# LeoIV/polyaxon

Measured on AMD Instinct MI355X. Metric: HPO trials/hour (whole node) + wall-clock-to-target, ResNet-50 Hyperband sweep, higher is better.
Workload: dtype bf16

## Files before the change

### polyaxon_amd/csrc/bn_kernels.hip

```cpp
#include <hip/hip_runtime.h>

#include "handoff.h"
#include <stdint.h>

#define PLX_API extern "C" __attribute__((visibility("default")))

namespace {

constexpr int kBlock = 256;

struct alignas(16) bf16x8 {
  uint16_t v[8];
};

__device__ __forceinline__ float bf2f(uint16_t b) { return __uint_as_float(((uint32_t)b) << 16); }

__device__ __forceinline__ uint16_t f2bf(float f) {
  return __builtin_bit_cast(uint16_t, (__bf16)f);
}

__device__ __forceinline__ void load8(const bf16x8* p, float* f) {
  const bf16x8 v = *p;
#pragma unroll
  for (int k = 0; k < 8; ++k) f[k] = bf2f(v.v[k]);
}

__device__ __forceinline__ void store8(bf16x8* p, const float* f) {
  bf16x8 v;
#pragma unroll
  for (int k = 0; k < 8; ++k) v.v[k] = f2bf(f[k]);
  *p = v;
}

__global__ __launch_bounds__(kBlock) void bn_stats_kernel(const bf16x8* __restrict__ x, int64_t M, int G, int Gb,
                                                          int64_t rows_per_block, float* __restrict__ psum,
                                                          float* __restrict__ psq) {
  __shared__ float s_sum[kBlock * 8];
  __shared__ float s_sq[kBlock * 8];
  const int tid = threadIdx.x;
  const int cg_local = tid % Gb, rlane = tid / Gb, R = kBlock / Gb;
  const int cg = blockIdx.y * Gb + cg_local;
  const int C = G * 8;
  float shift[8], s[8], q[8];
  load8(x + cg, shift);
#pragma unroll
  for (int k = 0; k < 8; ++k) s[k] = q[k] = 0.f;
  const int64_t r0 = (int64_t)blockIdx.x * rows_per_block;
  int64_t r1 = r0 + rows_per_block;
  if (r1 > M) r1 = M;
#pragma unroll 4
  for (int64_t r = r0 + rlane; r < r1; r += R) {
    float v[8];
    load8(x + r * G + cg, v);
#pragma unroll
    for (int k = 0; k < 8; ++k) {
      const float d = v[k] - shift[k];
      s[k] += d;
      q[k] = fmaf(d, d, q[k]);
    }
  }
#pragma unroll
  for (int k = 0; k < 8; ++k) {
    s_sum[tid * 8 + k] = s[k];
    s_sq[tid * 8 + k] = q[k];
  }
  __syncthreads();
  if (rlane == 0) {
    for (int j = 1; j < R; ++j) {
      const int o = (j * Gb + cg_local) * 8;
#pragma unroll
      for (int k = 0; k < 8; ++k) {
        s[k] += s_sum[o + k];
        q[k] += s_sq[o + k];
      }
    }
    float* ps = psum + (int64_t)blockIdx.x * C + cg * 8;
    float* pq = psq + (int64_t)blockIdx.x * C + cg * 8;
#pragma unroll
    for (int k = 0; k < 8; ++k) {
      ps[k] = s[k];
      pq[k] = q[k];
    }
  }
}

constexpr int kRowsPerSplit = 64;

template <int NT>
__device__ __forceinline__ float l1_rows(const float* __restrict__ src, int b0, int b1, int C, int c, int lane) {
  constexpr int G = NT / 64, U = kRowsPerSplit / G;
  float x[U];
#pragma unroll
  for (int u = 0; u < U; ++u) {
    const int b = b0 + lane + u * G;
    x[u] = b < b1 ? src[(int64_t)b * C + c] : 0.f;
  }
  float a = 0.f;
#pragma unroll
  for (int u = 0; u < U; ++u) a += x[u];
  return a;
}

template <int NT>
__global__ __launch_bounds__(NT) void bn_partial_reduce_kernel(const float* __restrict__ part, int nblk, int C,
                                                               float* __restrict__ out, int S) {
  constexpr int G = NT / 64;
  __shared__ float sh[NT];
  const int c = blockIdx.x * 64 + (threadIdx.x & 63);
  const int lane = threadIdx.x >> 6;
  const int s = blockIdx.y, which = blockIdx.z;
  const int b0 = s * kRowsPerSplit;
  const int b1 = b0 + kRowsPerSplit < nblk ? b0 + kRowsPerSplit : nblk;
  sh[threadIdx.x] = c < C ? l1_rows<NT>(part + (int64_t)which * nblk * C, b0, b1, C, c, lane) : 0.f;
  __syncthreads();
  if (lane == 0 && c < C) {
    float r = 0.f;
#pragma unroll
    for (int g = 0; g < G; ++g) r += sh[threadIdx.x + 64 * g];
    out[((int64_t)which * S + s) * C + c] = r;
  }
}

template <int NT = 256, bool ATOMIC = false>
__device__ __forceinline__ bool fin_sum2(const float* __restrict__ pa, const float* __restrict__ pb, int nblk, int C,
                                         double& A, double& B) {
  constexpr int G = NT / 64;
  __shared__ double sh[2][G][64];
  const int lc = threadIdx.x & 63, sp = threadIdx.x >> 6;
  const int c = blockIdx.x * 64 + lc;
  double a0 = 0.0, b0 = 0.0;
  if (c < C) {
    for (int b = sp; b < nblk; b += 8 * G) {
      float x[8], y[8];
#pragma unroll
      for (int u = 0; u < 8; ++u) {
        const int r = b + u * G;
        if (ATOMIC) {
          x[u] = r < nblk ? __hip_atomic_load(pa + (int64_t)r * C + c, __ATOMIC_RELAXED, __HIP_MEMORY_SCOPE_AGENT) : 0.f;
          y[u] = r < nblk ? __hip_atomic_load(pb + (int64_t)r * C + c, __ATOMIC_RELAXED, __HIP_MEMORY_SCOPE_AGENT) : 0.f;
        } else {
          x[u] = r < nblk ? pa[(int64_t)r * C + c] : 0.f;
          y[u] = r < nblk ? pb[(int64_t)r * C + c] : 0.f;
        }
      }
#pragma unroll
      for (int u = 0; u < 8; ++u) { a0 += x[u]; b0 += y[u]; }
    }
  }
  sh[0][sp][lc] = a0;
  sh[1][sp][lc] = b0;
  __syncthreads();
  if (sp != 0 || c >= C) return false;
  double sa = 0.0, sb = 0.0;
#pragma unroll
  for (int g = 0; g < G; ++g) { sa += sh[0][g][lc]; sb += sh[1][g][lc]; }
  A = sa;
  B = sb;
  return true;
}

struct FwdFin {
  const uint16_t* x_row0;
  int C;
  int64_t M;
  const float* gamma;
  const float* beta;
  float eps, momentum;
  float* running_mean;
  float* running_var;
  float* save_mean;
  float* save_invstd;
  float* scale;
  float* bias;
};

struct BwdFin {
  int C;
  int64_t M;
  const float* gamma;
  const float* mean;
  const float* invstd;
  float* dgamma;
  float* dbeta;
  float* coef;
  int accumulate;
};

template <int NT, bool ATOMIC = false>
__device__ __forceinline__ void fwd_finalize(const float* psum, const float* psq, int nblk, const FwdFin& f) {
  double S, Q;
  if (!fin_sum2<NT, ATOMIC>(psum, psq, nblk, f.C, S, Q)) return;
  const int c = blockIdx.x * 64 + (threadIdx.x & 63);
  const double m = S / (double)f.M;
  double var = Q / (double)f.M - m * m;
  if (var < 0.0) var = 0.0;
  const float mean = (f.x_row0 != nullptr ? bf2f(f.x_row0[c]) : 0.f) + (float)m;
  const float invstd = rsqrtf((float)var + f.eps);
  const float g = f.gamma[c];
  f.save_mean[c] = mean;
  f.save_invstd[c] = invstd;
  f.scale[c] = g * invstd;
  f.bias[c] = f.beta[c] - mean * g * invstd;
  if (f.running_mean != nullptr) {
    const float unbiased = f.M > 1 ? (float)(var * (double)f.M / (double)(f.M - 1)) : (float)var;
    f.running_mean[c] = (1.f - f.momentum) * f.running_mean[c] + f.momentum * mean;
    f.running_var[c] = (1.f - f.momentum) * f.running_var[c] + f.momentum * unbiased;
  }
}

template <int NT, bool ATOMIC = false>
__device__ __forceinline__ void bwd_finalize(const float* pdz, const float* pdzx, int nblk, const BwdFin& f) {
  double A, B;
  if (!fin_sum2<NT, ATOMIC>(pdz, pdzx, nblk, f.C, A, B)) return;
  const int C = f.C;
  const int c = blockIdx.x * 64 + (threadIdx.x & 63);
  const float db = (float)A, dg = (float)B;
  f.dbeta[c] = f.accumulate ? f.dbeta[c] + db : db;
  f.dgamma[c] = f.accumulate ? f.dgamma[c] + dg : dg;
  const float is = f.invstd[c], k1 = f.gamma[c] * is;
  const float k2 = db / (float)f.M, k3 = dg / (float)f.M;
  f.coef[c] = k1;
  f.coef[C + c] = -k1 * k3 * is;
  f.coef[2 * C + c] = -k1 * k2 + k1 * k3 * is * f.mean[c];
}

template <int NT>
__device__ __forceinline__ bool reduce_l2_last(const float* __restrict__ part, int nblk, int C, float* l2, int S,
                                               unsigned* cnt) {
  constexpr int G = NT / 64;
  __shared__ float sh[2][NT];
  __shared__ int s_last;
  const int c = blockIdx.x * 64 + (threadIdx.x & 63);
  const int lane = threadIdx.x >> 6;
  const int s = blockIdx.y;
  const int b0 = s * kRowsPerSplit;
  int b1 = b0 + kRowsPerSplit;
  if (b1 > nblk) b1 = nblk;
  float a0 = 0.f, a1 = 0.f;
  if (c < C) {
    a0 = l1_rows<NT>(part, b0, b1, C, c, lane);
    a1 = l1_rows<NT>(part + (int64_t)nblk * C, b0, b1, C, c, lane);
  }
  sh[0][threadIdx.x] = a0;
  sh[1][threadIdx.x] = a1;
  __syncthreads();
  if (lane == 0 && c < C) {
    const int t = threadIdx.x;
    float r0 = 0.f, r1 = 0.f;
#pragma unroll
    for (int g = 0; g < G; ++g) { r0 += sh[0][t + 64 * g]; r1 += sh[1][t + 64 * g]; }
    __hip_atomic_store(l2 + (int64_t)s * C + c, r0, __ATOMIC_RELAXED, __HIP_MEMORY_SCOPE_AGENT);
    __hip_atomic_store(l2 + ((int64_t)S + s) * C + c, r1, __ATOMIC_RELAXED, __HIP_MEMORY_SCOPE_AGENT);
  }
  asm volatile("s_waitcnt vmcnt(0)" ::: "memory");
  __syncthreads();
  if (threadIdx.x == 0) {
    plx_handoff_release();
    const unsigned old = __hip_atomic_fetch_add(cnt + blockIdx.x, 1u, __ATOMIC_RELAXED, __HIP_MEMORY_SCOPE_AGENT);
    const int last = old == (unsigned)(S - 1);
    if (last) plx_handoff_acquire();
    if (last) __hip_atomic_store(cnt + blockIdx.x, 0u, __ATOMIC_RELAXED, __HIP_MEMORY_SCOPE_AGENT);
    s_last = last;
  }
  __syncthreads();
  return s_last != 0;
}

constexpr int kFinNT = 1024;
template <int NT>
__global__ __launch_bounds__(NT) void bn_fwd_reduce_finalize_kernel(const float* __restrict__ part, int nblk, float* l2,
                                                                    int S, unsigned* cnt, FwdFin f) {
  if (!reduce_l2_last<NT>(part, nblk, f.C, l2, S, cnt)) return;
  fwd_finalize<NT, true>(l2, l2 + (int64_t)S * f.C, S, f);
}

template <int NT>
__global__ __launch_bounds__(NT) void bn_bwd_reduce_finalize_kernel(const float* __restrict__ part, int nblk, float* l2,
                                                                    int S, unsigned* cnt, BwdFin f) {
  if (!reduce_l2_last<NT>(part, nblk, f.C, l2, S, cnt)) return;
  bwd_finalize<NT, true>(l2, l2 + (int64_t)S * f.C, S, f);
}

template <int NT>
__global__ __launch_bounds__(NT) void bn_fwd_finalize_kernel(const float* __restrict__ psum, const float* __restrict__ psq, int nblk,
                                       const uint16_t* __restrict__ x_row0, int C, int64_t M,
                                       const float* __restrict__ gamma, const float* __restrict__ beta, float eps,
                                       float momentum, float* __restrict__ running_mean,
                                       float* __restrict__ running_var, float* __restrict__ save_mean,
                                       float* __restrict__ save_invstd, float* __restrict__ scale,
                                       float* __restrict__ bias) {
  double S, Q;
  if (!fin_sum2<NT>(psum, psq, nblk, C, S, Q)) return;
  const int c = blockIdx.x * 64 + (threadIdx.x & 63);
  const double m = S / (double)M;
  double var = Q / (double)M - m * m;
  if (var < 0.0) var = 0.0;
  const float mean = (x_row0 != nullptr ? bf2f(x_row0[c]) : 0.f) + (float)m;
  const float invstd = rsqrtf((float)var + eps);
  const float g = gamma[c];
  save_mean[c] = mean;
  save_invstd[c] = invstd;
  scale[c] = g * invstd;
  bias[c] = beta[c] - mean * g * invstd;
  if (running_mean != nullptr) {
    const float unbiased = M > 1 ? (float)(var * (double)M / (double)(M - 1)) : (float)var;
    running_mean[c] = (1.f - momentum) * running_mean[c] + momentum * mean;
    running_var[c] = (1.f - momentum) * running_var[c] + momentum * unbiased;
  }
}

template <bool RES, bool RELU>
__global__ __launch_bounds__(kBlock) void bn_apply_kernel(const bf16x8* __restrict__ x, const bf16x8* __restrict__ res,
                                                          bf16x8* __restrict__ y, const float* __restrict__ scale,
                                                          const float* __restrict__ bias, int64_t n_vec, int G,
                                                          uint8_t* __restrict__ mask, const float* __restrict__ rsb) {
  const int64_t stride = (int64_t)gridDim.x * blockDim.x;
  int64_t i = (int64_t)blockIdx.x * blockDim.x + threadIdx.x;
  if (i >= n_vec) return;
  const int cg = (int)(i % G);
  float a[8], b[8], ra[8], rb[8];
#pragma unroll
  for (int k = 0; k < 8; ++k) {
    a[k] = scale[cg * 8 + k];
    b[k] = bias[cg * 8 + k];
    ra[k] = 1.f;
    rb[k] = 0.f;
  }
  if (RES && rsb != nullptr) {
#pragma unroll
    for (int k = 0; k < 8; ++k) {
      ra[k] = rsb[cg * 8 + k];
      rb[k] = rsb[G * 8 + cg * 8 + k];
    }
  }
  for (; i < n_vec; i += stride) {
    const bf16x8 xv = x[i];
    bf16x8 rv;
    if constexpr (RES) rv = res[i];
    float v[8];
#pragma unroll
    for (int k = 0; k < 8; ++k) v[k] = fmaf(bf2f(xv.v[k]), a[k], b[k]);
    if constexpr (RES) {
#pragma unroll
      for (int k = 0; k < 8; ++k) v[k] += fmaf(bf2f(rv.v[k]), ra[k], rb[k]);
    }
    if constexpr (RELU) {
#pragma unroll
      for (int k = 0; k < 8; ++k) v[k] = fmaxf(v[k], 0.f);
    }
    store8(y + i, v);
    if (RELU && mask != nullptr) {
      uint32_t bits = 0;
#pragma unroll
      for (int k = 0; k < 8; ++k) bits |= (uint32_t)(v[k] > 0.f) << k;
      mask[i] = (uint8_t)bits;
    }
  }
}

template <bool RELU>
__global__ __launch_bounds__(kBlock) void bn_bwd_reduce_kernel(const bf16x8* __restrict__ x, const uint8_t* __restrict__ mask,
                                                               const bf16x8* __restrict__ dy, int64_t M, int G, int Gb,
                                                               int64_t rows_per_block, const float* __restrict__ mean,
                                                               const float* __restrict__ invstd, int relu,
                                                               float* __restrict__ pdz, float* __restrict__ pdzx) {
  __shared__ float s_a[kBlock * 8];
  __shared__ float s_b[kBlock * 8];
  const int tid = threadIdx.x;
  const int cg_local = tid % Gb, rlane = tid / Gb, R = kBlock / Gb;
  const int cg = blockIdx.y * Gb + cg_local;
  const int C = G * 8;
  float mu[8], is[8], sa[8], sb[8];
#pragma unroll
  for (int k = 0; k < 8; ++k) {
    mu[k] = mean[cg * 8 + k];
    is[k] = invstd[cg * 8 + k];
    sa[k] = sb[k] = 0.f;
  }
  const int64_t r0 = (int64_t)blockIdx.x * rows_per_block;
  int64_t r1 = r0 + rows_per_block;
  if (r1 > M) r1 = M;
#pragma unroll 4
  for (int64_t r = r0 + rlane; r < r1; r += R) {
    const int64_t off = r * G + cg;
    float xv[8], g[8];
    uint32_t mb = 0xffu;
    if constexpr (RELU) mb = mask[off];
    load8(x + off, xv);
    load8(dy + off, g);
    if constexpr (RELU) {
#pragma unroll
      for (int k = 0; k < 8; ++k) g[k] = (mb >> k) & 1u ? g[k] : 0.f;
    }
#pragma unroll
    for (int k = 0; k < 8; ++k) {
      sa[k] += g[k];
      sb[k] = fmaf(g[k], (xv[k] - mu[k]) * is[k], sb[k]);
    }
  }
#pragma unroll
  for (int k = 0; k < 8; ++k) {
    s_a[tid * 8 + k] = sa[k];
    s_b[tid * 8 + k] = sb[k];
  }
  __syncthreads();
  if (rlane == 0) {
    for (int j = 1; j < R; ++j) {
      const int o = (j * Gb + cg_local) * 8;
#pragma unroll
      for (int k = 0; k < 8; ++k) {
        sa[k] += s_a[o + k];
        sb[k] += s_b[o + k];
      }
    }
    float* pa = pdz + (int64_t)blockIdx.x * C + cg * 8;
    float* pb = pdzx + (int64_t)blockIdx.x * C + cg * 8;
#pragma unroll
    for (int k = 0; k < 8; ++k) {
      pa[k] = sa[k];
      pb[k] = sb[k];
    }
  }
}

template <int NT>
__global__ __launch_bounds__(NT) void bn_bwd_finalize_kernel(const float* __restrict__ pdz, const float* __restrict__ pdzx, int nblk, int C,
                                       int64_t M, const float* __restrict__ gamma, const float* __restrict__ mean,
                                       const float* __restrict__ invstd, float* __restrict__ dgamma,
                                       float* __restrict__ dbeta, float* __restrict__ coef, int accumulate) {
  double A, B;
  if (!fin_sum2<NT>(pdz, pdzx, nblk, C, A, B)) return;
  const int c = blockIdx.x * 64 + (threadIdx.x & 63);
  const float db = (float)A, dg = (float)B;
  dbeta[c] = accumulate ? dbeta[c] + db : db;
  dgamma[c] = accumulate ? dgamma[c] + dg : dg;
  const float is = invstd[c], k1 = gamma[c] * is;
  const float k2 = db / (float)M, k3 = dg / (float)M;
  coef[c] = k1;
  coef[C + c] = -k1 * k3 * is;
  coef[2 * C + c] = -k1 * k2 + k1 * k3 * is * mean[c];
}

struct ResBn {
  const bf16x8* x;
  const uint8_t* mask;
  const float* mean;
  const float* invstd;
  float* part;
};

template <bool RP, bool RELU, bool RMASK = false>
__global__ __launch_bounds__(kBlock) void bn_bwd_dx_kernel(const bf16x8* __restrict__ x, const uint8_t* __restrict__ mask,
                                                           const bf16x8* __restrict__ dy, bf16x8* __restrict__ dx,
                                                           bf16x8* __restrict__ dres, const float* __restrict__ coef,
                                                           int64_t n_vec, int G, int relu, ResBn rb) {
  const int64_t stride = (int64_t)gridDim.x * blockDim.x;
  int64_t i = (int64_t)blockIdx.x * blockDim.x + threadIdx.x;
  if (!RP && i >= n_vec) return;
  const int cg = (int)(i % G);
  const int C = G * 8;
  constexpr bool rp = RP;
  float A[8], B[8], D[8], mu2[8], is2[8], ra[8], rc[8];
#pragma unroll
  for (int k = 0; k < 8; ++k) {
    A[k] = coef[cg * 8 + k];
    B[k] = coef[C + cg * 8 + k];
    D[k] = coef[2 * C + cg * 8 + k];
    ra[k] = rc[k] = 0.f;
    mu2[k] = rp ? rb.mean[cg * 8 + k] : 0.f;
    is2[k] = rp ? rb.invstd[cg * 8 + k] : 0.f;
  }
  for (; i < n_vec; i += stride) {
    float xv[8], g[8];
    uint32_t mb = 0xffu;
    if constexpr (RELU) mb = mask[i];
    load8(x + i, xv);
    load8(dy + i, g);
    if constexpr (RELU) {
#pragma unroll
      for (int k = 0; k < 8; ++k) g[k] = (mb >> k) & 1u ? g[k] : 0.f;
    }
    if (dres != nullptr) store8(dres + i, g);
    if constexpr (rp) {
      float x2[8];
      load8(rb.x + i, x2);
      const uint32_t m2 = RMASK ? rb.mask[i] : 0xffu;
#pragma unroll
      for (int k = 0; k < 8; ++k) {
        const float g2 = (m2 >> k) & 1u ? g[k] : 0.f;
        ra[k] += g2;
        rc[k] = fmaf(g2, (x2[k] - mu2[k]) * is2[k], rc[k]);
      }
    }
    float o[8];
#pragma unroll
    for (int k = 0; k < 8; ++k) o[k] = fmaf(A[k], g[k], fmaf(B[k], xv[k], D[k]));
    store8(dx + i, o);
  }
  if constexpr (rp) {
  __shared__ float red[kBlock * 16];
#pragma unroll
  for (int k = 0; k < 8; ++k) {
    red[threadIdx.x * 16 + k] = ra[k];
    red[threadIdx.x * 16 + 8 + k] = rc[k];
  }
  __syncthreads();
  if ((int)threadIdx.x < G) {
    for (int j = 1; j < kBlock / G; ++j) {
      const float* o = red + (j * G + threadIdx.x) * 16;
#pragma unroll
      for (int k = 0; k < 8; ++k) {
        ra[k] += o[k];
        rc[k] += o[8 + k];
      }
    }
    float* pa = rb.part + (int64_t)blockIdx.x * C + cg * 8;
    float* pc = rb.part + ((int64_t)gridDim.x + blockIdx.x) * C + cg * 8;
#pragma unroll
    for (int k = 0; k < 8; ++k) {
      pa[k] = ra[k];
      pc[k] = rc[k];
    }
  }
  }
}

struct Plan {
  int G, Gb, gy, nblk, S;
  int64_t rows_per_block;
};

inline bool plan_for(int64_t M, int C, Plan* p) {
  if (C <= 0 || (C & 7)) return false;
  const int G = C / 8;
  if (G & (G - 1)) return false;
  p->G = G;
  p->Gb = G < kBlock ? G : kBlock;
  p->gy = G / p->Gb;
  const int R = kBlock / p->Gb;
  const int64_t cap = (2048 + p->gy - 1) / p->gy;
  int64_t want = (M + 16 * R - 1) / (16 * R);
  if (want > cap) want = cap;
  if (want < 1) want = 1;
  int64_t rpb = (M + want - 1) / want;
  rpb = (rpb + R - 1) / R * R;
  p->rows_per_block = rpb;
  p->nblk = (int)((M + rpb - 1) / rpb);
  p->S = (p->nblk + kRowsPerSplit - 1) / kRowsPerSplit;
  return true;
}

inline int apply_grid(int64_t n_vec, int G) {
  int64_t g = (n_vec + kBlock - 1) / kBlock;
  if (g > 4096) g = 4096;
  if (g < 1) g = 1;
  const int64_t mult = G > kBlock ? G / kBlock : 1;
  g = (g + mult - 1) / mult * mult;
  return (int)g;
}

inline void launch_dx(hipStream_t stream, int64_t n_vec, int G, const void* x, const uint8_t* mask, const void* dy,
                      void* dx, void* dres, const float* coef, int relu, const ResBn& rb) {
  const dim3 grid(apply_grid(n_vec, G));
  auto k = rb.part == nullptr ? (relu ? bn_bwd_dx_kernel<false, true> : bn_bwd_dx_kernel<false, false>)
           : rb.mask != nullptr ? (relu ? bn_bwd_dx_kernel<true, true, true> : bn_bwd_dx_kernel<true, false, true>)
                                : (relu ? bn_bwd_dx_kernel<true, true> : bn_bwd_dx_kernel<true, false>);
  hipLaunchKernelGGL(k, grid, dim3(kBlock), 0, stream, (const bf16x8*)x, mask, (const bf16x8*)dy, (bf16x8*)dx,
                     (bf16x8*)dres, coef, n_vec, G, relu, rb);
}

inline void launch_apply(hipStream_t stream, int64_t n_vec, int G, const void* x, const void* res, void* y,
                         const float* scale, const float* bias, int relu, uint8_t* mask, const float* rsb) {
  auto k = res != nullptr ? (relu ? bn_apply_kernel<true, true> : bn_apply_kernel<true, false>)
                          : (relu ? bn_apply_kernel<false, true> : bn_apply_kernel<false, false>);
  hipLaunchKernelGGL(k, dim3(apply_grid(n_vec, G)), dim3(kBlock), 0, stream, (const bf16x8*)x, (const bf16x8*)res,
                     (bf16x8*)y, scale, bias, n_vec, G, mask, rsb);
}

inline void reduce_finalize_fwd(hipStream_t stream, const float* part, int nblk, float* l2, unsigned* cnt,
                                const FwdFin& f) {
  const int C = f.C, S = (nblk + kRowsPerSplit - 1) / kRowsPerSplit;
  if (cnt != nullptr) {
    hipLaunchKernelGGL(bn_fwd_reduce_finalize_kernel<kFinNT>, dim3((C + 63) / 64, S), dim3(kFinNT), 0, stream, part, nblk, l2, S,
                       cnt, f);
    return;
  }
  hipLaunchKernelGGL(bn_partial_reduce_kernel<kFinNT>,
                     dim3((C + 63) / 64, S, 2), dim3(kFinNT), 0, stream, part, nblk, C, l2, S);
  hipLaunchKernelGGL(bn_fwd_finalize_kernel<kFinNT>, dim3((C + 63) / 64),
                     dim3(kFinNT), 0, stream, l2, l2 + (int64_t)S * C, S,
                     f.x_row0, C, f.M, f.gamma, f.beta, f.eps, f.momentum, f.running_mean, f.running_var, f.save_mean,
                     f.save_invstd, f.scale, f.bias);
}

inline void reduce_finalize_bwd(hipStream_t stream, const float* part, int nblk, float* l2, unsigned* cnt,
                                const BwdFin& f) {
  const int C = f.C, S = (nblk + kRowsPerSplit - 1) / kRowsPerSplit;
  if (cnt != nullptr) {
    hipLaunchKernelGGL(bn_bwd_reduce_finalize_kernel<kFinNT>, dim3((C + 63) / 64, S), dim3(kFinNT), 0, stream, part, nblk, l2, S,
                       cnt, f);
    return;
  }
  hipLaunchKernelGGL(bn_partial_reduce_kernel<kFinNT>,
                     dim3((C + 63) / 64, S, 2), dim3(kFinNT), 0, stream, part, nblk, C, l2, S);
  hipLaunchKernelGGL(bn_bwd_finalize_kernel<kFinNT>, dim3((C + 63) / 64),
                     dim3(kFinNT), 0, stream, l2, l2 + (int64_t)S * C, S, C,
                     f.M, f.gamma, f.mean, f.invstd, f.dgamma, f.dbeta, f.coef, f.accumulate);
}

struct alignas(8) u8x8 {
  uint8_t v[8];
};

__global__ __launch_bounds__(256) void stem_apply_pool_kernel(const bf16x8* __restrict__ x,
                                                              const float* __restrict__ sb, bf16x8* __restrict__ y,
                                                              u8x8* __restrict__ idx, int N, int H, int W, int G,
                                                              int OH, int OW) {
  const unsigned j = blockIdx.x * 256u + threadIdx.x;
  if (j >= (unsigned)(OW * G)) return;
  const unsigned g = j % (unsigned)G, ow = j / (unsigned)G;
  const int C = G * 8;
  float a[8], b[8];
#pragma unroll
  for (int k = 0; k < 8; ++k) {
    a[k] = sb[g * 8 + k];
    b[k] = sb[C + g * 8 + k];
  }
  for (int row = blockIdx.y; row < N * OH; row += gridDim.y) {
    const int n = row / OH, oh = row - n * OH;
    float best[8];
    uint8_t arg[8];
#pragma unroll
    for (int k = 0; k < 8; ++k) {
      best[k] = -INFINITY;
      arg[k] = 255;
    }
    uint4 q[9];
    bool ok[9];
#pragma unroll
    for (int kh = 0; kh < 3; ++kh) {
      const int ih = oh * 2 - 1 + kh;
      const int ihc = ih < 0 ? 0 : (ih >= H ? H - 1 : ih);
#pragma unroll
      for (int kw = 0; kw < 3; ++kw) {
        const int iw = (int)ow * 2 - 1 + kw;
        const int iwc = iw < 0 ? 0 : (iw >= W ? W - 1 : iw);
        ok[kh * 3 + kw] = ih >= 0 && ih < H && iw >= 0 && iw < W;
        q[kh * 3 + kw] = *(const uint4*)(x + ((size_t)(n * H + ihc) * W + iwc) * G + g);
      }
    }
#pragma unroll
    for (int t9 = 0; t9 < 9; ++t9) {
      const uint32_t qw[4] = {q[t9].x, q[t9].y, q[t9].z, q[t9].w};
#pragma unroll
      for (int k = 0; k < 8; ++k) {
        const float xk = __uint_as_float((k & 1) ? (qw[k >> 1] & 0xffff0000u) : (qw[k >> 1] << 16));
        const float f = (float)(__bf16)fmaxf(fmaf(xk, a[k], b[k]), 0.f);
        if (ok[t9] && (f > best[k] || arg[k] == 255)) {
          best[k] = f;
          arg[k] = (uint8_t)t9;
        }
      }
    }
    bf16x8 o;
    u8x8 m;
#pragma unroll
    for (int k = 0; k < 8; ++k) {
      o.v[k] = f2bf(best[k]);
      m.v[k] = arg[k];
    }
    const size_t t = (size_t)row * OW * G + j;
    y[t] = o;
    idx[t] = m;
  }
}

__device__ __forceinline__ int stem_cover(int i, int O, int* o, int* k) {
  int n = 0;
  if (i & 1) {
    if ((i + 1) >> 1 < O) { o[n] = (i + 1) >> 1; k[n++] = 0; }
    o[n] = (i - 1) >> 1; k[n++] = 2;
  } else if ((i >> 1) < O) {
    o[n] = i >> 1; k[n++] = 1;
  }
  return n;
}

template <bool DX>
__global__ __launch_bounds__(256) void stem_pool_bn_bwd_kernel(const bf16x8* __restrict__ dy, const u8x8* __restrict__ idx,
                                                               const bf16x8* __restrict__ x, const float* __restrict__ sb,
                                                               const float* __restrict__ mean,
                                                               const float* __restrict__ invstd,
                                                               const float* __restrict__ coef, bf16x8* __restrict__ dx,
                                                               float* __restrict__ part, int N, int H, int W, int G,
                                                               int OH, int OW) {
  const int QH = (H + 1) / 2, QW = (W + 1) / 2;
  const unsigned j0 = blockIdx.x * 256u + threadIdx.x;
  const bool active = j0 < (unsigned)(QW * G);
  const unsigned j = active ? j0 : 0u;
  const unsigned g = j % (unsigned)G;
  const int qb = (int)(j / (unsigned)G);
  const int C = G * 8;
  float a[8], b[8], c1[8], c2[8], c3[8], s1[8], s2[8];
#pragma unroll
  for (int k = 0; k < 8; ++k) {
    a[k] = sb[g * 8 + k];
    b[k] = sb[C + g * 8 + k];
    if constexpr (DX) {
      c1[k] = coef[g * 8 + k];
      c2[k] = coef[C + g * 8 + k];
      c3[k] = coef[2 * C + g * 8 + k];
    } else {
      c1[k] = mean[g * 8 + k];
      c2[k] = invstd[g * 8 + k];
      c3[k] = 0.f;
    }
    s1[k] = s2[k] = 0.f;
  }
  for (int row = blockIdx.y; active && row < N * QH; row += gridDim.y) {
    const int n = row / QH, qa = row - n * QH;
    uint2 am[4];
    uint4 d[4], xq[4];
    bool wv[4], pv[4];
#pragma unroll
    for (int p = 0; p < 2; ++p)
#pragma unroll
      for (int q = 0; q < 2; ++q) {
        const int w4 = p * 2 + q, oh = qa + p, ow = qb + q;
        wv[w4] = oh < OH && ow < OW;
        const size_t off = ((size_t)(n * OH + (oh < OH ? oh : OH - 1)) * OW + (ow < OW ? ow : OW - 1)) * G + g;
        am[w4] = *(const uint2*)(idx + off);
        d[w4] = *(const uint4*)(dy + off);
        if (!wv[w4]) am[w4] = make_uint2(0xffffffffu, 0xffffffffu);
        const int ih = 2 * qa + p, iw = 2 * qb + q;
        pv[w4] = ih < H && iw < W;
        xq[w4] = *(const uint4*)(x + ((size_t)(n * H + (ih < H ? ih : H - 1)) * W + (iw < W ? iw : W - 1)) * G + g);
      }
#pragma unroll
    for (int di = 0; di < 2; ++di)
#pragma unroll
      for (int dj = 0; dj < 2; ++dj) {
        const int e = di * 2 + dj;
        const uint32_t xw[4] = {xq[e].x, xq[e].y, xq[e].z, xq[e].w};
        float o[8];
#pragma unroll
        for (int k = 0; k < 8; ++k) {
          float acc = 0.f;
#pragma unroll
          for (int p = 0; p < 2; ++p)
#pragma unroll
            for (int q = 0; q < 2; ++q) {
              const int kh = di + 1 - 2 * p, kw = dj + 1 - 2 * q;
              if (kh < 0 || kw < 0) continue;
              const int w4 = p * 2 + q;
              const uint32_t ab = (k < 4 ? am[w4].x : am[w4].y) >> (8 * (k & 3)) & 0xffu;
              const uint32_t dw = (k >> 1) == 0 ? d[w4].x : (k >> 1) == 1 ? d[w4].y : (k >> 1) == 2 ? d[w4].z : d[w4].w;
              const float dv = __uint_as_float((k & 1) ? (dw & 0xffff0000u) : (dw << 16));
              acc += ab == (uint32_t)(kh * 3 + kw) ? dv : 0.f;
            }
          const float xf = __uint_as_float((k & 1) ? (xw[k >> 1] & 0xffff0000u) : (xw[k >> 1] << 16));
          const float dz = (pv[e] && fmaf(xf, a[k], b[k]) > 0.f) ? (float)(__bf16)acc : 0.f;
          if constexpr (DX) {
            o[k] = fmaf(c1[k], dz, fmaf(c2[k], xf, c3[k]));
          } else {
            s1[k] += dz;
            s2[k] = fmaf(dz, (xf - c1[k]) * c2[k], s2[k]);
          }
        }
        if constexpr (DX) {
          if (pv[e]) store8(dx + ((size_t)(n * H + 2 * qa + di) * W + 2 * qb + dj) * G + g, o);
        }
      }
  }
  if constexpr (!DX) {
    __shared__ float red[256 * 17];
#pragma unroll
    for (int k = 0; k < 8; ++k) {
      red[threadIdx.x * 17 + k] = s1[k];
      red[threadIdx.x * 17 + 8 + k] = s2[k];
    }
    __syncthreads();
    const int nb = gridDim.x * gridDim.y, blk = blockIdx.y * gridDim.x + blockIdx.x;
    for (int e = threadIdx.x; e < G * 16; e += 256) {
      const int gg = e % G, v = e / G;
      float sum = 0.f;
      for (int r = gg; r < 256; r += G) sum += red[r * 17 + v];
      const int c = gg * 8 + (v & 7);
      part[((int64_t)(v < 8 ? 0 : nb) + blk) * C + c] = sum;
    }
  }
}

constexpr int g_stem_bwd_cap = 4096;

inline dim3 stem_bwd_grid(int N, int H, int W, int G, bool dx) {
  const int rows = N * ((H + 1) / 2), cap = dx ? 65535 : g_stem_bwd_cap;
  return dim3((((W + 1) / 2) * G + 255) / 256, rows < cap ? rows : cap);
}

}

PLX_API int64_t plx_bn_workspace(int64_t M, int C) {
  Plan p;
  if (!plan_for(M, C, &p)) return -1;
  return 2 * (int64_t)(p.nblk + p.S) * C;
}

PLX_API int plx_bn_forward(const void* x, const void* res, void* y, int64_t M, int C, const float* gamma,
                           const float* beta, float eps, float momentum, float* running_mean, float* running_var,
                           float* save_mean, float* save_invstd, float* scale_bias ,
                           float* partials , uint8_t* mask ,
                           int relu, const float* res_sb ,
                           unsigned* counters ,
                           hipStream_t stream) {
  Plan p;
  if (!plan_for(M, C, &p) || M < 1) return 1;
  float* psum = partials;
  float* psq = partials + (int64_t)p.nblk * C;
  hipLaunchKernelGGL(bn_stats_kernel, dim3(p.nblk, p.gy), dim3(kBlock), 0, stream, (const bf16x8*)x, M, p.G, p.Gb,
                     p.rows_per_block, psum, psq);
  float* l2 = partials + 2 * (int64_t)p.nblk * C;
  reduce_finalize_fwd(stream, partials, p.nblk, l2, counters,
                      FwdFin{(const uint16_t*)x, C, M, gamma, beta, eps, momentum, running_mean, running_var,
                             save_mean, save_invstd, scale_bias, scale_bias + C});
  const int64_t n_vec = M * p.G;
  if (y != nullptr)
    launch_apply(stream, n_vec, p.G, x, res, y, scale_bias, scale_bias + C, relu, relu ? mask : nullptr, res_sb);
  return (int)hipGetLastError();
}

PLX_API int64_t plx_bn_l2_workspace(int nblk, int C) {
  return 2 * (int64_t)((nblk + kRowsPerSplit - 1) / kRowsPerSplit) * C;
}

PLX_API int plx_bn_forward_from_partials(const void* x, const void* res, void* y, int64_t M, int C,
                                         const float* gamma, const float* beta, float eps, float momentum,
                                         float* running_mean, float* running_var, float* save_mean,
                                         float* save_invstd, float* scale_bias, const float* partials, int nblk,
                                         float* l2, uint8_t* mask, int relu, const float* res_sb,
                                         unsigned* counters, hipStream_t stream) {
  Plan p;
  if (!plan_for(M, C, &p) || M < 1 || nblk < 1) return 1;
  reduce_finalize_fwd(stream, partials, nblk, l2, counters,
                      FwdFin{nullptr, C, M, gamma, beta, eps, momentum, running_mean, running_var, save_mean,
                             save_invstd, scale_bias, scale_bias + C});
  const int64_t n_vec = M * p.G;
  if (y != nullptr)
    launch_apply(stream, n_vec, p.G, x, res, y, scale_bias, scale_bias + C, relu, relu ? mask : nullptr, res_sb);
  return (int)hipGetLastError();
}

PLX_API int plx_bn_apply(const void* x, const void* res, void* y, int64_t M, int C, const float* scale_bias, int relu,
                         hipStream_t stream) {
  Plan p;
  if (!plan_for(M, C, &p)) return 1;
  const int64_t n_vec = M * p.G;
  launch_apply(stream, n_vec, p.G, x, res, y, scale_bias, scale_bias + C, relu, nullptr, nullptr);
  return (int)hipGetLastError();
}

PLX_API int plx_bn_dx_blocks(int64_t M, int C) {
  Plan p;
  if (!plan_for(M, C, &p)) return -1;
  return apply_grid(M * p.G, p.G);
}

PLX_API int plx_bn_backward(const void* x, const uint8_t* mask, const void* dy, void* dx, void* dres, int64_t M, int C,
                            const float* gamma, const float* save_mean, const float* save_invstd, float* dgamma,
                            float* dbeta, float* coef , float* partials , int relu,
                            int accumulate, const ResBn* resbn , unsigned* counters,
                            hipStream_t stream) {
  Plan p;
  if (!plan_for(M, C, &p) || M < 1 || (relu && mask == nullptr)) return 1;
  if (resbn != nullptr && (dres == nullptr || resbn->part == nullptr)) return 1;
  const ResBn rb = resbn != nullptr ? *resbn : ResBn{};
  float* pa = partials;
  float* pb = partials + (int64_t)p.nblk * C;
  hipLaunchKernelGGL(relu ? bn_bwd_reduce_kernel<true> : bn_bwd_reduce_kernel<false>, dim3(p.nblk, p.gy), dim3(kBlock), 0, stream, (const bf16x8*)x,
                     mask, (const bf16x8*)dy, M, p.G, p.Gb, p.rows_per_block, save_mean, save_invstd,
                     relu, pa, pb);
  float* l2 = partials + 2 * (int64_t)p.nblk * C;
  reduce_finalize_bwd(stream, partials, p.nblk, l2, counters,
                      BwdFin{C, M, gamma, save_mean, save_invstd, dgamma, dbeta, coef, accumulate});
  const int64_t n_vec = M * p.G;
  launch_dx(stream, n_vec, p.G, x, mask, dy, dx, dres, coef, relu, rb);
  return (int)hipGetLastError();
}

PLX_API int plx_bn_backward_from_partials(const void* x, const uint8_t* mask, const void* dy, void* dx, void* dres,
                                          int64_t M, int C, const float* gamma, const float* save_mean,
                                          const float* save_invstd, float* dgamma, float* dbeta, float* coef,
                                          const float* partials, int nblk, float* l2, int relu, int accumulate,
                                          const ResBn* resbn, unsigned* counters, hipStream_t stream) {
  Plan p;
  if (!plan_for(M, C, &p) || M < 1 || nblk < 1 || (relu && mask == nullptr)) return 1;
  if (resbn != nullptr && (dres == nullptr || resbn->part == nullptr)) return 1;
  const ResBn rb = resbn != nullptr ? *resbn : ResBn{};
  reduce_finalize_bwd(stream, partials, nblk, l2, counters,
                      BwdFin{C, M, gamma, save_mean, save_invstd, dgamma, dbeta, coef, accumulate});
  const int64_t n_vec = M * p.G;
  launch_dx(stream, n_vec, p.G, x, mask, dy, dx, dres, coef, relu, rb);
  return (int)hipGetLastError();
}

PLX_API int plx_bn_backward_coef(const void* x, const uint8_t* mask, const void* dy, int64_t M, int C,
                                 const float* gamma, const float* save_mean, const float* save_invstd, float* dgamma,
                                 float* dbeta, float* coef, float* partials, int relu, int accumulate,
                                 unsigned* counters, hipStream_t stream) {
  Plan p;
  if (!plan_for(M, C, &p) || M < 1 || (relu && mask == nullptr)) return 1;
  float* pa = partials;
  float* pb = partials + (int64_t)p.nblk * C;
  hipLaunchKernelGGL(relu ? bn_bwd_reduce_kernel<true> : bn_bwd_reduce_kernel<false>, dim3(p.nblk, p.gy), dim3(kBlock), 0, stream, (const bf16x8*)x,
                     mask, (const bf16x8*)dy, M, p.G, p.Gb, p.rows_per_block, save_mean, save_invstd,
                     relu, pa, pb);
  reduce_finalize_bwd(stream, partials, p.nblk, partials + 2 * (int64_t)p.nblk * C, counters,
                      BwdFin{C, M, gamma, save_mean, save_invstd, dgamma, dbeta, coef, accumulate});
  return (int)hipGetLastError();
}

PLX_API int plx_bn_backward_coef_from_partials(int64_t M, int C, const float* gamma, const float* save_mean,
                                               const float* save_invstd, float* dgamma, float* dbeta, float* coef,
                                               const float* partials, int nblk, float* l2, int accumulate,
                                               unsigned* counters, hipStream_t stream) {
  Plan p;
  if (!plan_for(M, C, &p) || M < 1 || nblk < 1) return 1;
  reduce_finalize_bwd(stream, partials, nblk, l2, counters,
                      BwdFin{C, M, gamma, save_mean, save_invstd, dgamma, dbeta, coef, accumulate});
  return (int)hipGetLastError();
}

PLX_API int plx_stem_bn_pool_forward(const void* x, void* y, void* idx, int N, int H, int W, int C, const float* gamma,
                                     const float* beta, float eps, float momentum, float* running_mean,
                                     float* running_var, float* save_mean, float* save_invstd, float* scale_bias,
                                     float* partials, const float* ext_part, int ext_nblk, unsigned* counters,
                                     hipStream_t stream) {
  const int G = C / 8;
  if (N <= 0 || H <= 0 || W <= 0 || C % 8 || G > 256 || 256 % G) return 1;
  const int rc = ext_part != nullptr
                     ? plx_bn_forward_from_partials(x, nullptr, nullptr, (int64_t)N * H * W, C, gamma, beta, eps,
                                                    momentum, running_mean, running_var, save_mean, save_invstd,
                                                    scale_bias, ext_part, ext_nblk, partials, nullptr, 1, nullptr,
                                                    counters, stream)
                     : plx_bn_forward(x, nullptr, nullptr, (int64_t)N * H * W, C, gamma, beta, eps, momentum,
                                      running_mean, running_var, save_mean, save_invstd, scale_bias, partials, nullptr,
                                      1, nullptr, counters, stream);
  if (rc) return rc;
  const int OH = (H - 1) / 2 + 1, OW = (W - 1) / 2 + 1;
  const int rows = N * OH;
  hipLaunchKernelGGL(stem_apply_pool_kernel, dim3((OW * G + 255) / 256, rows < 65535 ? rows : 65535), dim3(256), 0,
                     stream, (const bf16x8*)x, scale_bias, (bf16x8*)y, (u8x8*)idx, N, H, W, G, OH, OW);
  return (int)hipGetLastError();
}


PLX_API int64_t plx_stem_bn_pool_bwd_workspace(int N, int H, int W, int C) {
  const dim3 g = stem_bwd_grid(N, H, W, C / 8, false);
  const int64_t nblk = (int64_t)g.x * g.y;
  return 2 * (nblk + (nblk + kRowsPerSplit - 1) / kRowsPerSplit) * C;
}

PLX_API int plx_stem_bn_pool_backward(const void* dy, const void* idx, const void* x, void* dx, int N, int H, int W,
                                      int C, const float* gamma, const float* save_mean, const float* save_invstd,
                                      const float* scale_bias, float* dgamma, float* dbeta, float* coef,
                                      float* workspace, int accumulate, unsigned* counters, hipStream_t stream) {
  const int G = C / 8;
  if (N <= 0 || H <= 0 || W <= 0 || C % 8 || G > 256 || 256 % G) return 1;
  const int OH = (H - 1) / 2 + 1, OW = (W - 1) / 2 + 1;
  const dim3 grid = stem_bwd_grid(N, H, W, G, false), grid_dx = stem_bwd_grid(N, H, W, G, true);
  const int nblk = grid.x * grid.y;
  hipLaunchKernelGGL(stem_pool_bn_bwd_kernel<false>, grid, dim3(256), 0, stream, (const bf16x8*)dy, (const u8x8*)idx,
                     (const bf16x8*)x, scale_bias, save_mean, save_invstd, (const float*)nullptr, (bf16x8*)nullptr,
                     workspace, N, H, W, G, OH, OW);
  reduce_finalize_bwd(stream, workspace, nblk, workspace + 2 * (int64_t)nblk * C, counters,
                      BwdFin{C, (int64_t)N * H * W, gamma, save_mean, save_invstd, dgamma, dbeta, coef, accumulate});
  hipLaunchKernelGGL(stem_pool_bn_bwd_kernel<true>, grid_dx, dim3(256), 0, stream, (const bf16x8*)dy, (const u8x8*)idx,
                     (const bf16x8*)x, scale_bias, save_mean, save_invstd, coef, (bf16x8*)dx, (float*)nullptr, N, H,
                     W, G, OH, OW);
  return (int)hipGetLastError();
}
```

### polyaxon_amd/csrc/conv_gemm.hip

```cpp
#include <hip/hip_runtime.h>

#include <stdint.h>

namespace {

typedef __bf16 bf16x8 __attribute__((ext_vector_type(8)));
typedef short s16x4 __attribute__((ext_vector_type(4)));
typedef float f32x4 __attribute__((ext_vector_type(4)));
typedef uint32_t u32x4 __attribute__((ext_vector_type(4)));
typedef __attribute__((address_space(3))) void lds_void;
typedef __attribute__((address_space(1))) const void gbl_void;

constexpr int BK = 64;

struct ConvGeom {
    int H, W;
    int Hr, Wr;
    int C, S, ntaps;
    int Hc, Wc, OS, oph, opw;
    signed char offh[9], offw[9], btap[9];
    int tap_a[9], tap_b[9];
    uint32_t mWr, mHr;
    int nh, nw, hv[3], wv[3];
    uint32_t pat[9];
    int tap_inner;
};

__device__ __forceinline__ int pick9(const int (&v)[9], int t) {
    int r = v[0];
#pragma unroll
    for (int i = 1; i < 9; ++i) r = t == i ? v[i] : r;
    return r;
}

inline uint32_t div_magic(int d) { return d <= 1 ? 0u : (uint32_t)((1ull << 32) / (unsigned)d + 1); }

inline ConvGeom finish_geom(ConvGeom g) {
    g.nh = g.nw = 0;
    for (int i = 0; i < 9; ++i) g.pat[i] = 0;
    for (int t = 0; t < 9; ++t) {
        g.tap_a[t] = t < g.ntaps ? (g.offh[t] * g.W + g.offw[t]) * g.C * 2 : 0;
        g.tap_b[t] = t < g.ntaps ? g.btap[t] * g.C * 2 : 0;
        if (t >= g.ntaps) continue;
        int i = 0, j = 0;
        while (i < g.nh && g.hv[i] != g.offh[t]) ++i;
        if (i == g.nh) g.hv[g.nh++] = g.offh[t];
        while (j < g.nw && g.wv[j] != g.offw[t]) ++j;
        if (j == g.nw) g.wv[g.nw++] = g.offw[t];
        g.pat[i * 3 + j] |= 1u << t;
    }
    g.mWr = div_magic(g.Wr);
    g.mHr = div_magic(g.Hr);
    return g;
}

struct BnBwd {
    const __bf16* x;
    const uint8_t* mask;
    const float* mean;
    const float* invstd;
    float* part;
    int part_ld, blk_off;
    int skip_h, skip_w;
};

struct BnDx {
    const __bf16* x;
    const uint8_t* mask;
    const float* coef;
    __bf16* dy;
};

__device__ __forceinline__ void row_coords(int m, int Hr, int Wr, int& n, int& r, int& c) {
    const int q = m / Wr;
    c = m - q * Wr;
    n = q / Hr;
    r = q - n * Hr;
}

__device__ __forceinline__ void row_coords(int m, const ConvGeom& g, int& n, int& r, int& c) {
    const int q = g.mWr ? (int)__umulhi((uint32_t)m, g.mWr) : m;
    c = m - q * g.Wr;
    n = g.mHr ? (int)__umulhi((uint32_t)q, g.mHr) : q;
    r = q - n * g.Hr;
}

__device__ __forceinline__ size_t out_row(const ConvGeom& g, int m) {
    if (g.OS == 0) return (size_t)m;
    int n, r, c;
    row_coords(m, g.Hr, g.Wr, n, r, c);
    return ((size_t)n * g.Hc + r * g.OS + g.oph) * g.Wc + c * g.OS + g.opw;
}
constexpr int NTHREADS = 256;

template <int STEP>
__device__ __forceinline__ void wait_vm_stages(int stages) {
    if (stages >= 4 && 4 * STEP <= 63) asm volatile("s_waitcnt vmcnt(%0)" ::"n"(4 * STEP < 63 ? 4 * STEP : 63) : "memory");
    else if (stages >= 3) asm volatile("s_waitcnt vmcnt(%0)" ::"n"(3 * STEP) : "memory");
    else if (stages == 2) asm volatile("s_waitcnt vmcnt(%0)" ::"n"(2 * STEP) : "memory");
    else if (stages == 1) asm volatile("s_waitcnt vmcnt(%0)" ::"n"(STEP) : "memory");
    else asm volatile("s_waitcnt vmcnt(0)" ::: "memory");
}

__device__ __forceinline__ int xcd_remap(int bid, int nwg) {
    const int xcd = bid & 7, q = nwg >> 3, r = nwg & 7;
    const int base = xcd < r ? xcd * (q + 1) : r * (q + 1) + (xcd - r) * q;
    return base + (bid >> 3);
}

__device__ __forceinline__ void glds16(const void* g, void* l) {
    __builtin_amdgcn_global_load_lds((gbl_void*)g, (lds_void*)l, 16, 0, 0);
}

constexpr uint32_t OOB = 0x80000000u;

__device__ __forceinline__ __amdgpu_buffer_rsrc_t buf_rsrc(const void* base) {
    return __builtin_amdgcn_make_buffer_rsrc(const_cast<void*>(base), 0, (int)OOB, 0x00020000);
}

__device__ __forceinline__ void blds16(__amdgpu_buffer_rsrc_t r, uint32_t off, void* l) {
    __builtin_amdgcn_raw_ptr_buffer_load_lds(r, (lds_void*)l, 16, off, 0, 0, 0);
}

__device__ __forceinline__ uint32_t pack_bf16x2(float a, float b) {
    return (uint32_t)__builtin_bit_cast(uint16_t, (__bf16)a) | ((uint32_t)__builtin_bit_cast(uint16_t, (__bf16)b) << 16);
}

__device__ __forceinline__ int nt_swz(int row) { return (row >> 1) & 7; }

template <int BM, int BN, int WGM, int WGN, int MODE, int MINB = 2, int NBUF = 2, bool BWD = false, int NTH = NTHREADS,
          bool BNDX = false>
__global__ void __launch_bounds__(NTH, MINB)
gemm_nt_kernel(const __bf16* __restrict__ A, const __bf16* __restrict__ B, __bf16* __restrict__ C,
               int M, int N, int K, int lda, int ldb, int ldc, const __bf16* __restrict__ zero,
               float* __restrict__ stats, ConvGeom geo, const __bf16* __restrict__ D, int ldd, BnBwd bnr,
               const uint8_t* __restrict__ dmask, BnDx bd) {
    constexpr bool CONV = MODE == 1, STEM = MODE == 2;
    static_assert(MODE >= 0 && MODE <= 2, "dense, gather or stem");
    static_assert(!BNDX || (MODE == 0 && NBUF == 2 && BWD && NTH == 256), "BNDX: dense double-buffered data gradient");
    constexpr int NW = NTH / 64;
    static_assert(WGM * WGN == NW, "one wave per wave tile");
    static_assert(NTH == 256 && NBUF >= 1 && NBUF <= 2, "4-wave kernels, one or two K stages");
    constexpr int WTM = BM / WGM, WTN = BN / WGN;
    constexpr int RM = WTM / 16, RN = WTN / 16;
    constexpr int A_BYTES = BM * BK * 2, B_BYTES = BN * BK * 2, STAGE = A_BYTES + B_BYTES;
    extern __shared__ __attribute__((aligned(16))) char smem[];

    const int tid = threadIdx.x, lane = tid & 63;
    const int wave = __builtin_amdgcn_readfirstlane(tid >> 6);
    const int ntn = N / BN, ntm = (M + BM - 1) / BM;
    const int id = xcd_remap(blockIdx.x, ntm * ntn);
    const int tn = id % ntn, tm = id / ntn;
    const int m0 = tm * BM, n0 = tn * BN;
    const int wm = wave / WGN, wn = wave % WGN;

    constexpr int AI = BM / (8 * NW), BI = BN / (8 * NW);
    int a_off[AI];
    uint32_t a_ok[AI];
#pragma unroll
    for (int i = 0; i < AI; ++i) {
        const int row = (i * NW + wave) * 8 + (lane >> 3);
        const int lc = (lane & 7) ^ nt_swz(row);
        const int gm = m0 + row;
        if constexpr (CONV) {
            int n, r, c;
            row_coords(gm, geo, n, r, c);
            const int ih0 = r * geo.S, iw0 = c * geo.S;
            a_off[i] = (((n * geo.H + ih0) * geo.W + iw0) * lda + lc * 8) * 2;
            uint32_t ok = 0;
#pragma unroll
            for (int hi = 0; hi < 3; ++hi) {
                const bool vh = hi < geo.nh && (unsigned)(ih0 + geo.hv[hi]) < (unsigned)geo.H;
#pragma unroll
                for (int wj = 0; wj < 3; ++wj) {
                    const bool vw = wj < geo.nw && (unsigned)(iw0 + geo.wv[wj]) < (unsigned)geo.W;
                    ok |= (vh && vw) ? geo.pat[hi * 3 + wj] : 0u;
                }
            }
            a_ok[i] = gm < M ? ok : 0u;
        } else if constexpr (STEM) {
            int n, r, c;
            row_coords(gm, geo, n, r, c);
            const int ih0 = 2 * r - 3, sc0 = c - 2;
            a_off[i] = ((n * geo.H + ih0) * geo.W + sc0) * 16;
            uint32_t ok = 0;
#pragma unroll
            for (int st = 0; st < 4; ++st) {
                const int t = st * 8 + lc;
                ok |= (t < 28 && (unsigned)(ih0 + (t >> 2)) < (unsigned)geo.H && (unsigned)(sc0 + (t & 3)) < (unsigned)geo.W)
                          ? 1u << st : 0u;
            }
            a_ok[i] = gm < M ? ok : 0u;
        } else {
            a_off[i] = (gm * lda + lc * 8) * 2;
            a_ok[i] = gm < M ? 1u : 0u;
        }
    }
    int b_off[BI];
#pragma unroll
    for (int i = 0; i < BI; ++i) {
        const int row = (i * NW + wave) * 8 + (lane >> 3);
        b_off[i] = ((n0 + row) * ldb + ((lane & 7) ^ nt_swz(row)) * 8) * 2;
    }
    const __amdgpu_buffer_rsrc_t ra = buf_rsrc(A), rb = buf_rsrc(B);

    auto stage_a = [&](int buf, int k0, int t, int c0) {
        char* base = smem + buf * STAGE;
        int a_add = k0 * 2, bit = 0;
        if constexpr (CONV) {
            a_add = pick9(geo.tap_a, t) + c0 * 2;
            bit = t;
        }
        if constexpr (STEM) bit = k0 / BK;
#pragma unroll
        for (int i = 0; i < AI; ++i) {
            if constexpr (STEM) {
                const int t = bit * 8 + ((lane & 7) ^ nt_swz((i * NW + wave) * 8 + (lane >> 3)));
                a_add = ((t >> 2) * geo.W + (t & 3)) * 16;
            }
            const uint32_t off = (a_ok[i] >> bit) & 1u ? (uint32_t)(a_off[i] + a_add) : OOB;
            blds16(ra, off, base + (i * NW + wave) * 1024);
        }
    };
    auto stage_b = [&](int buf, int k0, int t, int c0) {
        char* base = smem + buf * STAGE;
        const int bk0 = CONV ? pick9(geo.tap_b, t) + c0 * 2 : k0 * 2;
#pragma unroll
        for (int i = 0; i < BI; ++i) blds16(rb, (uint32_t)(b_off[i] + bk0), base + A_BYTES + (i * NW + wave) * 1024);
    };
    auto stage = [&](int buf, int k0, int t, int c0) {
        stage_a(buf, k0, t, c0);
        stage_b(buf, k0, t, c0);
    };

    f32x4 acc[RN][RM];
#pragma unroll
    for (int a = 0; a < RN; ++a)
#pragma unroll
        for (int b = 0; b < RM; ++b) acc[a][b] = f32x4{0.f, 0.f, 0.f, 0.f};

    const int fr = lane & 15, fq = lane >> 4;
    const int nk = K / BK;
    const int cdim = CONV ? geo.C : K;
    int st = 0, sc = 0;
    const bool tap_inner = CONV && geo.tap_inner;
    auto advance = [&]() {
        const bool wt = st + 1 == geo.ntaps, wc = sc + BK == cdim;
        const int st_i = wt ? 0 : st + 1, sc_i = wt ? sc + BK : sc;
        const int st_m = wc ? st + 1 : st, sc_m = wc ? 0 : sc + BK;
        st = tap_inner ? st_i : st_m;
        sc = tap_inner ? sc_i : sc_m;
    };
    constexpr int XI = BNDX ? AI : 1;
    uint32_t e_off[XI];
    u32x4 gq[XI], xq[XI], oq[XI];
    uint32_t mq[XI];
    u32x4 cf[6];
    const int lc8 = (((lane & 7) ^ nt_swz(wave * 8 + (lane >> 3))) & 7) * 8;
    const bool dy_owner = tn == 0;
    if constexpr (BNDX) {
#pragma unroll
        for (int i = 0; i < XI; ++i) {
            const int gm = m0 + (i * NW + wave) * 8 + (lane >> 3);
            e_off[i] = gm < M ? (uint32_t)((gm * K + lc8) * 2) : OOB;
        }
    }
    auto load_a = [&](int k0) {
        const __amdgpu_buffer_rsrc_t rx = buf_rsrc(bd.x), rc = buf_rsrc(bd.coef);
#pragma unroll
        for (int i = 0; i < XI; ++i) {
            gq[i] = __builtin_amdgcn_raw_buffer_load_b128(ra, (int)e_off[i], k0 * 2, 0);
            xq[i] = __builtin_amdgcn_raw_buffer_load_b128(rx, (int)e_off[i], k0 * 2, 0);
        }
        if (bd.mask != nullptr) {
            const __amdgpu_buffer_rsrc_t rm = buf_rsrc(bd.mask);
#pragma unroll
            for (int i = 0; i < XI; ++i)
                mq[i] = __builtin_amdgcn_raw_buffer_load_b8(rm, (int)(e_off[i] == OOB ? OOB : e_off[i] >> 4), k0 >> 3, 0);
        } else {
#pragma unroll
            for (int i = 0; i < XI; ++i) mq[i] = 0xffu;
        }
#pragma unroll
        for (int r = 0; r < 3; ++r) {
            cf[2 * r] = __builtin_amdgcn_raw_buffer_load_b128(rc, lc8 * 4, (r * K + k0) * 4, 0);
            cf[2 * r + 1] = __builtin_amdgcn_raw_buffer_load_b128(rc, lc8 * 4 + 16, (r * K + k0) * 4, 0);
        }
    };
    auto xform_a = [&](int buf) {
        char* base = smem + buf * STAGE;
        const float* ca = (const float*)&cf[0];
        const float* cb = (const float*)&cf[2];
        const float* cd = (const float*)&cf[4];
#pragma unroll
        for (int i = 0; i < XI; ++i) {
            const uint32_t* pg = (const uint32_t*)&gq[i];
            const uint32_t* px = (const uint32_t*)&xq[i];
            uint32_t* po = (uint32_t*)&oq[i];
            const uint32_t mb = mq[i];
#pragma unroll
            for (int j = 0; j < 4; ++j) {
                const float g0 = (mb >> (2 * j)) & 1u ? __uint_as_float(pg[j] << 16) : 0.f;
                const float g1 = (mb >> (2 * j + 1)) & 1u ? __uint_as_float(pg[j] & 0xffff0000u) : 0.f;
                const float x0 = __uint_as_float(px[j] << 16), x1 = __uint_as_float(px[j] & 0xffff0000u);
                const float o0 = fmaf(ca[2 * j], g0, fmaf(cb[2 * j], x0, cd[2 * j]));
                const float o1 = fmaf(ca[2 * j + 1], g1, fmaf(cb[2 * j + 1], x1, cd[2 * j + 1]));
                po[j] = pack_bf16x2(o0, o1);
            }
            if (e_off[i] == OOB) oq[i] = u32x4{0u, 0u, 0u, 0u};
            *(u32x4*)(base + (i * NW + wave) * 1024 + lane * 16) = oq[i];
        }
    };
    auto store_dy = [&](int k0) {
        if (!dy_owner) return;
        const __amdgpu_buffer_rsrc_t rd = buf_rsrc(bd.dy);
#pragma unroll
        for (int i = 0; i < XI; ++i) __builtin_amdgcn_raw_buffer_store_b128(oq[i], rd, (int)e_off[i], k0 * 2, 0);
    };
    if constexpr (BNDX) {
        static_assert(!BNDX || NW == 4, "a thread's rows step by 32: one chunk column per thread");
        load_a(0);
        stage_b(0, 0, 0, 0);
        xform_a(0);
        asm volatile("s_waitcnt vmcnt(0)" ::: "memory");
        __syncthreads();
        store_dy(0);
    } else {
        stage(0, 0, 0, 0);
        advance();
        asm volatile("s_waitcnt vmcnt(0)" ::: "memory");
        __syncthreads();
    }
    for (int kt = 0; kt < nk; ++kt) {
        const int cur = NBUF == 2 ? kt & 1 : 0;
        if constexpr (BNDX) {
            if (kt + 1 < nk) {
                load_a((kt + 1) * BK);
                stage_b(cur ^ 1, (kt + 1) * BK, 0, 0);
            }
        }
        if (!BNDX && NBUF == 1 && kt > 0) {
            stage(0, kt * BK, st, sc);
            advance();
            asm volatile("s_waitcnt vmcnt(0)" ::: "memory");
            __syncthreads();
        }
        if (!BNDX && NBUF == 2 && kt + 1 < nk) {
            stage(cur ^ 1, (kt + 1) * BK, st, sc);
            advance();
        }
        const char* As = smem + cur * STAGE;
        const char* Bs = As + A_BYTES;
#pragma unroll
        for (int kk = 0; kk < 2; ++kk) {
            bf16x8 fa[RN], fb[RM];
#pragma unroll
            for (int rn = 0; rn < RN; ++rn) {
                const int row = wn * WTN + rn * 16 + fr;
                const int pc = (kk * 4 + fq) ^ nt_swz(row);
                fa[rn] = *(const bf16x8*)(Bs + row * 128 + pc * 16);
            }
#pragma unroll
            for (int rm = 0; rm < RM; ++rm) {
                const int row = wm * WTM + rm * 16 + fr;
                const int pc = (kk * 4 + fq) ^ nt_swz(row);
                fb[rm] = *(const bf16x8*)(As + row * 128 + pc * 16);
            }
#pragma unroll
            for (int rn = 0; rn < RN; ++rn)
#pragma unroll
                for (int rm = 0; rm < RM; ++rm)
                    acc[rn][rm] = __builtin_amdgcn_mfma_f32_16x16x32_bf16(fa[rn], fb[rm], acc[rn][rm], 0, 0, 0);
        }
        if constexpr (BNDX) {
            if (kt + 1 < nk) xform_a(cur ^ 1);
        }
        if (NBUF == 2) asm volatile("s_waitcnt vmcnt(0)" ::: "memory");
        __syncthreads();
        if constexpr (BNDX) {
            if (kt + 1 < nk) store_dy((kt + 1) * BK);
        }
    }
    constexpr int CROW = BN * 2 + 16;
    constexpr int CHUNKS = BN / 8;
    static_assert(NTH % CHUNKS == 0, "a thread keeps one chunk column over the store loop");
    constexpr int RSTEP = NTH / CHUNKS, ITERS = BM / RSTEP;
    const int rows = min(BM, M - m0);
    const int cc = tid % CHUNKS, r0 = tid / CHUNKS;
    const int ch0 = n0 + cc * 8;
    const bool bnr_on = BWD && bnr.part != nullptr;
    const bool stats_on = !BWD && stats != nullptr;
    const bool d_on = BWD && D != nullptr;
    int orow[ITERS];
#pragma unroll
    for (int it = 0; it < ITERS; ++it) {
        const int gm = min(m0 + r0 + it * RSTEP, M - 1);
        if constexpr (CONV) orow[it] = (int)out_row(geo, gm);
        else orow[it] = gm;
    }
    auto tile_to_lds = [&]() {
#pragma unroll
        for (int rm = 0; rm < RM; ++rm) {
            const int ml = wm * WTM + rm * 16 + fr;
#pragma unroll
            for (int rn = 0; rn < RN; ++rn) {
                const int nl = wn * WTN + rn * 16 + fq * 4;
                const f32x4 v = acc[rn][rm];
                uint2 packed;
                packed.x = pack_bf16x2(v[0], v[1]);
                packed.y = pack_bf16x2(v[2], v[3]);
                *(uint2*)(smem + ml * CROW + nl * 2) = packed;
            }
        }
    };
    constexpr bool LATE = BWD && NBUF == 1;
    if constexpr (LATE) tile_to_lds();
    uint4 dpre[ITERS], xpre[ITERS];
    uint32_t mpre[ITERS], dmpre[ITERS];
    if (d_on) {
#pragma unroll
        for (int it = 0; it < ITERS; ++it) dpre[it] = *(const uint4*)(D + (size_t)orow[it] * ldd + ch0);
        if (dmask != nullptr) {
#pragma unroll
            for (int it = 0; it < ITERS; ++it) dmpre[it] = dmask[((size_t)orow[it] * ldd + ch0) >> 3];
        }
    }
    float sa[8], sb[8], mu[8], is[8];
    float s1[8], s2[8];
#pragma unroll
    for (int k = 0; k < 8; ++k) s1[k] = s2[k] = 0.f;
    if (bnr_on) {
#pragma unroll
        for (int it = 0; it < ITERS; ++it) xpre[it] = *(const uint4*)(bnr.x + (size_t)orow[it] * ldc + ch0);
        if (bnr.mask != nullptr) {
#pragma unroll
            for (int it = 0; it < ITERS; ++it) mpre[it] = bnr.mask[((size_t)orow[it] * ldc + ch0) >> 3];
        } else {
#pragma unroll
            for (int it = 0; it < ITERS; ++it) mpre[it] = 0xffu;
        }
        if (bnr.skip_w > 0) {
#pragma unroll
            for (int it = 0; it < ITERS; ++it) {
                const int gm = m0 + r0 + it * RSTEP, q = gm / bnr.skip_w;
                if (((gm - q * bnr.skip_w) | (q % bnr.skip_h)) % 2 == 0) mpre[it] = 0u;
            }
        }
#pragma unroll
        for (int k = 0; k < 8; ++k) {
            sa[k] = sb[k] = 0.f;
            mu[k] = bnr.mean[ch0 + k];
            is[k] = bnr.invstd[ch0 + k];
        }
    }
    if constexpr (!LATE) tile_to_lds();
    __syncthreads();
#pragma unroll
    for (int it = 0; it < ITERS; ++it) {
        const int r = r0 + it * RSTEP;
        if (r >= rows) break;
        uint4 v = *(const uint4*)(smem + r * CROW + cc * 16);
        if (stats_on) {
            const uint32_t* pv = (const uint32_t*)&v;
#pragma unroll
            for (int j = 0; j < 4; ++j) {
                const float lo = __uint_as_float(pv[j] << 16), hi = __uint_as_float(pv[j] & 0xffff0000u);
                s1[2 * j] += lo;
                s1[2 * j + 1] += hi;
                s2[2 * j] = fmaf(lo, lo, s2[2 * j]);
                s2[2 * j + 1] = fmaf(hi, hi, s2[2 * j + 1]);
            }
        }
        if (d_on) {
            uint32_t* pv = (uint32_t*)&v;
            const uint32_t* pd = (const uint32_t*)&dpre[it];
            const uint32_t db = dmask != nullptr ? dmpre[it] : 0xffu;
#pragma unroll
            for (int j = 0; j < 4; ++j) {
                const float d0 = (db >> (2 * j)) & 1u ? __uint_as_float(pd[j] << 16) : 0.f;
                const float d1 = (db >> (2 * j + 1)) & 1u ? __uint_as_float(pd[j] & 0xffff0000u) : 0.f;
                const float lo = __uint_as_float(pv[j] << 16) + d0;
                const float hi = __uint_as_float(pv[j] & 0xffff0000u) + d1;
                pv[j] = pack_bf16x2(lo, hi);
            }
        }
        *(uint4*)(C + (size_t)orow[it] * ldc + ch0) = v;
        if (bnr_on) {
            const uint32_t mb = mpre[it];
            const uint32_t* pv = (const uint32_t*)&v;
            const uint32_t* px = (const uint32_t*)&xpre[it];
#pragma unroll
            for (int j = 0; j < 4; ++j) {
                const float g0 = (mb >> (2 * j)) & 1u ? __uint_as_float(pv[j] << 16) : 0.f;
                const float g1 = (mb >> (2 * j + 1)) & 1u ? __uint_as_float(pv[j] & 0xffff0000u) : 0.f;
                const float x0 = __uint_as_float(px[j] << 16), x1 = __uint_as_float(px[j] & 0xffff0000u);
                sa[2 * j] += g0;
                sa[2 * j + 1] += g1;
                sb[2 * j] = fmaf(g0, (x0 - mu[2 * j]) * is[2 * j], sb[2 * j]);
                sb[2 * j + 1] = fmaf(g1, (x1 - mu[2 * j + 1]) * is[2 * j + 1], sb[2 * j + 1]);
            }
        }
    }
    auto reduce_store = [&](const float* va, const float* vb, float* dst_a, float* dst_b) {
        float* red = (float*)smem;
        __syncthreads();
#pragma unroll
        for (int k = 0; k < 8; ++k) {
            red[tid * 17 + k] = va[k];
            red[tid * 17 + 8 + k] = vb[k];
        }
        __syncthreads();
        if (tid < CHUNKS * 16) {
            const int c = tid % CHUNKS, v = tid / CHUNKS;
            float sum = 0.f;
#pragma unroll 4
            for (int j = 0; j < RSTEP; ++j) sum += red[(j * CHUNKS + c) * 17 + v];
            if (v < 8) dst_a[c * 8 + v] = sum;
            else dst_b[c * 8 + v - 8] = sum;
        }
        __syncthreads();
    };
    constexpr int SROWS = BN % 128 == 0 ? 128 : 256, SPB = BM / SROWS;
    static_assert(SPB >= 1 && BM % SROWS == 0, "block height must be a multiple of the stats row height");
    const int srow = m0 / SROWS, nsr = (M + SROWS - 1) / SROWS;
    auto zero_rows = [&](float* base_a, float* base_b, int ld) {
        if constexpr (SPB > 1) {
            for (int i = tid; i < (SPB - 1) * BN; i += NTH) {
                const int r = srow + 1 + i / BN, c = i % BN;
                if (r < nsr) {
                    base_a[(size_t)(r - srow) * ld + c] = 0.f;
                    base_b[(size_t)(r - srow) * ld + c] = 0.f;
                }
            }
        }
    };
    if (bnr_on) {
        float* pa = bnr.part + (size_t)(bnr.blk_off + srow) * ldc + n0;
        float* pb = bnr.part + (size_t)(bnr.part_ld + bnr.blk_off + srow) * ldc + n0;
        reduce_store(sa, sb, pa, pb);
        zero_rows(pa, pb, ldc);
    }
    if (stats_on) {
        float* pa = stats + (size_t)srow * N + n0;
        float* pb = stats + (size_t)(nsr + srow) * N + n0;
        reduce_store(s1, s2, pa, pb);
        zero_rows(pa, pb, N);
    }
}

template <int ROWB>
__device__ __forceinline__ int tr_swz(int row) {
    if constexpr (ROWB >= 256) return 2 * ((row & 3) | (((row >> 3) & 1) << 2));
    else return 2 * (((row >> 1) & 1) | (((row >> 3) & 1) << 1));
}

template <int ROWB>
__device__ __forceinline__ s16x4 tr_read(const char* img, int row, int col ) {
    const int lc = col >> 3, half = (col >> 2) & 1;
    const int pc = lc ^ tr_swz<ROWB>(row);
    return __builtin_amdgcn_ds_read_tr16_b64_v4i16(
        (__attribute__((address_space(3))) s16x4*)(img + row * ROWB + pc * 16 + half * 8));
}

__device__ __forceinline__ uint32_t lds_addr(const void* p) {
    return (uint32_t)(uintptr_t)(const __attribute__((address_space(3))) char*)p;
}

__device__ __forceinline__ s16x4 ds_tr(uint32_t addr) {
    s16x4 r;
    asm volatile("ds_read_b64_tr_b16 %0, %1" : "=v"(r) : "v"(addr) : "memory");
    return r;
}

template <int ROWB, int GATHER = 0, int BKR = BK>
__device__ __forceinline__ void stage_rows(char* img, __amdgpu_buffer_rsrc_t rsrc, int ld, int r0, int rend, int c0,
                                           int wave, int lane, const ConvGeom* geo = nullptr, int dh = 0, int dw = 0) {
    constexpr int INSTR = BKR * ROWB / 1024;
    static_assert(INSTR % 4 == 0, "a stage splits evenly over the 4 waves");
#pragma unroll
    for (int i = 0; i < INSTR / 4; ++i) {
        const int off = (i * 4 + wave) * 1024 + lane * 16;
        const int row = off / ROWB, pc = (off % ROWB) >> 4;
        const int lc = pc ^ tr_swz<ROWB>(row);
        const int gr = r0 + row;
        uint32_t boff;
        if constexpr (GATHER == 2) {
            int n, r, c;
            row_coords(gr, *geo, n, r, c);
            const int t = (c0 >> 3) + lc, ih = 2 * r - 3 + (t >> 2), sc = c - 2 + (t & 3);
            const bool ok = gr < rend && t < 28 && (unsigned)ih < (unsigned)geo->H && (unsigned)sc < (unsigned)geo->W;
            boff = ok ? (uint32_t)(((n * geo->H + ih) * geo->W + sc) * 16) : OOB;
        } else if constexpr (GATHER == 1) {
            int n, r, c;
            row_coords(gr, *geo, n, r, c);
            const int ih = r * geo->S + dh, iw = c * geo->S + dw;
            const bool ok = gr < rend && (unsigned)ih < (unsigned)geo->H && (unsigned)iw < (unsigned)geo->W;
            boff = ok ? (uint32_t)(((((n * geo->H + ih) * geo->W + iw) * ld) + c0 + lc * 8) * 2) : OOB;
        } else {
            boff = gr < rend ? (uint32_t)((gr * ld + c0 + lc * 8) * 2) : OOB;
        }
        blds16(rsrc, boff, img + (i * 4 + wave) * 1024);
    }
}


template <int BN1, int BN2, int WG1, int WG2, int CONV, int NST = 2, int BKT = BK>
__global__ void __launch_bounds__(NTHREADS, NST * BKT <= 2 * BK ? 2 : 1)
gemm_tn_kernel(const __bf16* __restrict__ A, const __bf16* __restrict__ B, float* __restrict__ W,
               int M, int N1, int N2, int lda, int ldb, int kchunk, const __bf16* __restrict__ zero,
               ConvGeom geo) {
    constexpr int WT1 = BN1 / WG1, WT2 = BN2 / WG2, R1 = WT1 / 16, R2 = WT2 / 16;
    constexpr int ROWA = BN1 * 2, ROWB_ = BN2 * 2;
    constexpr int A_BYTES = BKT * ROWA, STAGE = BKT * (ROWA + ROWB_);
    constexpr int PER_STAGE = (BKT * ROWA / 1024 + BKT * ROWB_ / 1024) / 4;
    static_assert(BKT == 64 || BKT == 32, "32- or 64-row stages");
    static_assert(NST >= 2 && NST <= 4, "2-4 stages");
    extern __shared__ __attribute__((aligned(16))) char smem[];

    const int tid = threadIdx.x, lane = tid & 63;
    const int wave = __builtin_amdgcn_readfirstlane(tid >> 6);
    const int nt1 = N1 / BN1, nt2 = N2 / BN2, ntiles = nt1 * nt2;
    const int nslices = (M + kchunk - 1) / kchunk;
    const int id = xcd_remap(blockIdx.x, ntiles * nslices);
    const int tile = id % ntiles, slice = id / ntiles;
    const int t1 = tile / nt2, t2 = tile % nt2;
    const int n10 = t1 * BN1, n20 = t2 * BN2;
    const int kbeg = slice * kchunk, kend = min(M, kbeg + kchunk);
    const int w1 = wave / WG2, w2 = wave % WG2;

    f32x4 acc[R1][R2];
#pragma unroll
    for (int a = 0; a < R1; ++a)
#pragma unroll
        for (int b = 0; b < R2; ++b) acc[a][b] = f32x4{0.f, 0.f, 0.f, 0.f};

    const int nk = (kend - kbeg + BKT - 1) / BKT;
    int bc0 = n20, dh = 0, dw = 0;
    if constexpr (CONV == 1) {
        const int t = n20 / geo.C;
        bc0 = n20 - t * geo.C;
        dh = geo.offh[t];
        dw = geo.offw[t];
    }
    const __amdgpu_buffer_rsrc_t ra = buf_rsrc(A), rb = buf_rsrc(B);
    auto stage = [&](int buf, int k0) {
        char* base = smem + buf * STAGE;
        stage_rows<ROWA, 0, BKT>(base, ra, lda, k0, kend, n10, wave, lane);
        stage_rows<ROWB_, CONV, BKT>(base + A_BYTES, rb, ldb, k0, kend, bc0, wave, lane, &geo, dh, dw);
    };
    const int gi = lane & 15, g = lane >> 4, q = gi >> 2, p = gi & 3;
    if constexpr (NST == 2) {
        if (nk > 0) {
            stage(0, kbeg);
            asm volatile("s_waitcnt vmcnt(0)" ::: "memory");
            __syncthreads();
        }
    } else {
        for (int st = 0; st < NST - 1 && st < nk; ++st) stage(st, kbeg + st * BKT);
    }
    for (int kt = 0; kt < nk; ++kt) {
        int cur;
        if constexpr (NST == 2) {
            cur = kt & 1;
            if (kt + 1 < nk) stage(cur ^ 1, kbeg + (kt + 1) * BKT);
        } else {
            const int later = min(NST - 2, nk - 1 - kt);
            wait_vm_stages<PER_STAGE>(later);
            __syncthreads();
            if (kt + NST - 1 < nk) stage((kt + NST - 1) % NST, kbeg + (kt + NST - 1) * BKT);
            cur = kt % NST;
        }
        const char* As = smem + cur * STAGE;
        const char* Bs = As + A_BYTES;
#pragma unroll
        for (int kk = 0; kk < BKT / 32; ++kk) {
            const int kb = kk * 32 + 8 * g + q;
            bf16x8 fa[R1], fb[R2];
#pragma unroll
            for (int r = 0; r < R1; ++r) {
                const int c = w1 * WT1 + r * 16 + 4 * p;
                const s16x4 lo = tr_read<ROWA>(As, kb, c), hi = tr_read<ROWA>(As, kb + 4, c);
                fa[r] = __builtin_bit_cast(bf16x8, __builtin_shufflevector(lo, hi, 0, 1, 2, 3, 4, 5, 6, 7));
            }
#pragma unroll
            for (int r = 0; r < R2; ++r) {
                const int c = w2 * WT2 + r * 16 + 4 * p;
                const s16x4 lo = tr_read<ROWB_>(Bs, kb, c), hi = tr_read<ROWB_>(Bs, kb + 4, c);
                fb[r] = __builtin_bit_cast(bf16x8, __builtin_shufflevector(lo, hi, 0, 1, 2, 3, 4, 5, 6, 7));
            }
#pragma unroll
            for (int a = 0; a < R1; ++a)
#pragma unroll
                for (int b = 0; b < R2; ++b)
                    acc[a][b] = __builtin_amdgcn_mfma_f32_16x16x32_bf16(fa[a], fb[b], acc[a][b], 0, 0, 0);
        }
        if constexpr (NST == 2) {
            asm volatile("s_waitcnt vmcnt(0)" ::: "memory");
            __syncthreads();
        }
    }
    float* slab = W + (size_t)slice * N1 * N2;
#pragma unroll
    for (int a = 0; a < R1; ++a)
#pragma unroll
        for (int b = 0; b < R2; ++b) {
            const int c2 = n20 + w2 * WT2 + b * 16 + gi;
            const int r1 = n10 + w1 * WT1 + a * 16 + 4 * g;
#pragma unroll
            for (int r = 0; r < 4; ++r) slab[(size_t)(r1 + r) * N2 + c2] = acc[a][b][r];
        }
}

__global__ void slab_partial_kernel(const float* __restrict__ W, float* __restrict__ P, long plane, int slices,
                                    int per_group) {
    const long total4 = plane / 4;
    const int s0 = blockIdx.y * per_group, s1 = min(slices, s0 + per_group);
    for (long i = blockIdx.x * (long)blockDim.x + threadIdx.x; i < total4; i += (long)gridDim.x * blockDim.x) {
        float4 acc = make_float4(0.f, 0.f, 0.f, 0.f);
        for (int s = s0; s < s1; ++s) {
            const float4 v = ((const float4*)(W + s * plane))[i];
            acc.x += v.x; acc.y += v.y; acc.z += v.z; acc.w += v.w;
        }
        ((float4*)(P + blockIdx.y * plane))[i] = acc;
    }
}

__global__ void slab_final_kernel(const float* __restrict__ S, float* __restrict__ C, int N1, int N2, int ldc,
                                  int nslabs, int accumulate) {
    const long total4 = (long)N1 * N2 / 4;
    const long plane = (long)N1 * N2;
    for (long i = blockIdx.x * (long)blockDim.x + threadIdx.x; i < total4; i += (long)gridDim.x * blockDim.x) {
        float4 acc = make_float4(0.f, 0.f, 0.f, 0.f);
        for (int s = 0; s < nslabs; ++s) {
            const float4 v = ((const float4*)(S + s * plane))[i];
            acc.x += v.x; acc.y += v.y; acc.z += v.z; acc.w += v.w;
        }
        const long e = i * 4;
        const int r = (int)(e / N2), c = (int)(e % N2);
        float* dst = C + (size_t)r * ldc + c;
        if (accumulate) {
            const float4 o = *(const float4*)dst;
            acc.x += o.x; acc.y += o.y; acc.z += o.z; acc.w += o.w;
        }
        *(float4*)dst = acc;
    }
}

template <int NA, int NB, int KS, int CONV, int BKT, int RING, bool ATOMIC = false>
__global__ void __launch_bounds__(64 * KS * NA * NB, 1)
wgrad_kernel(const __bf16* __restrict__ A, const __bf16* __restrict__ B, float* __restrict__ W, int M, int N1, int N2,
             int lda, int ldb, int kchunk, ConvGeom geo, int ldc) {
    constexpr int GW = NA * NB;
    constexpr int NW = KS * GW;
    constexpr int R2 = RING / KS;
    constexpr int SUB = BKT * 128;
    constexpr int STAGE = (NA + NB) * SUB;
    constexpr int PPS = SUB / 1024;
    static_assert(BKT == 32 || BKT == 64, "32- or 64-row stages");
    static_assert(KS % 2 == 0, "ping-pong pairs the two halves of the wave groups");
    static_assert(RING % KS == 0 && R2 >= 2, "every group owns >= 2 ring slots");
    static_assert(RING * STAGE <= 160 * 1024, "LDS ring exceeds the CU's LDS");
    static_assert((KS - 1) * GW * 16384 <= RING * STAGE, "the wave-group reduction reuses the ring");
    extern __shared__ __attribute__((aligned(16))) char smem[];

    const int lane = threadIdx.x & 63;
    const int wave = __builtin_amdgcn_readfirstlane(threadIdx.x >> 6);
    constexpr int BN1 = 64 * NA, BN2 = 64 * NB;
    const int nt1 = N1 / BN1, nt2 = N2 / BN2, ntiles = nt1 * nt2;
    const int nslices = (M + kchunk - 1) / kchunk;
    const int id = xcd_remap(blockIdx.x, ntiles * nslices);
    const int tile = id % ntiles, slice = id / ntiles;
    const int n10 = (tile / nt2) * BN1, n20 = (tile % nt2) * BN2;
    const int kbeg = slice * kchunk, kend = min(M, kbeg + kchunk);
    const int nk = kend > kbeg ? (kend - kbeg + BKT - 1) / BKT : 0;
    const int grp = wave / GW, wg = wave % GW, w1 = wg / NB, w2 = wg % NB;
    const int nu = nk > grp ? (nk - grp + KS - 1) / KS : 0;
    const int nit = (nk + KS - 1) / KS;
    const bool lag = wave >= NW / 2;

    constexpr int PA = NA * PPS, PB = NB * PPS;
    constexpr int IA = (PA + GW - 1) / GW, IB = (PB + GW - 1) / GW;
    int cnta = 0, cntb = 0, arow[IA], acol[IA], brow[IB], bcol[IB], bdh[IB], bdw[IB];
#pragma unroll
    for (int i = 0; i < IA; ++i) {
        const int pa = wg + i * GW, row = (pa % PPS) * 8 + (lane >> 3);
        cnta += pa < PA ? 1 : 0;
        arow[i] = row;
        acol[i] = n10 + (pa / PPS) * 64 + (((lane & 7) ^ tr_swz<128>(row)) * 8);
    }
#pragma unroll
    for (int i = 0; i < IB; ++i) {
        const int pb = wg + i * GW, row = (pb % PPS) * 8 + (lane >> 3);
        const int col = n20 + (pb / PPS) * 64, lc8 = ((lane & 7) ^ tr_swz<128>(row)) * 8;
        cntb += pb < PB ? 1 : 0;
        brow[i] = row;
        bdh[i] = bdw[i] = 0;
        bcol[i] = col + lc8;
        if constexpr (CONV == 1) {
            const int t = col / geo.C;
            bdh[i] = geo.offh[t];
            bdw[i] = geo.offw[t];
            bcol[i] = col - t * geo.C + lc8;
        }
    }
    cnta = __builtin_amdgcn_readfirstlane(cnta);
    cntb = __builtin_amdgcn_readfirstlane(cntb);
    const int cnt = cnta + cntb;
    const __amdgpu_buffer_rsrc_t ra = buf_rsrc(A), rb = buf_rsrc(B);
    const int gH = geo.H, gW = geo.W, gS = geo.S, gWr = geo.Wr, gHr = geo.Hr;
    const uint32_t gmWr = geo.mWr, gmHr = geo.mHr;
    auto coords = [=](int m, int& n, int& r, int& c) {
        const int qq = gmWr ? (int)__umulhi((uint32_t)m, gmWr) : m;
        c = m - qq * gWr;
        n = gmHr ? (int)__umulhi((uint32_t)qq, gmHr) : qq;
        r = qq - n * gHr;
    };
    char* const gslots = smem + grp * R2 * STAGE;

    auto issue = [&](int u) {
        char* base = gslots + (u % R2) * STAGE;
        const int k0 = kbeg + (grp + KS * u) * BKT;
#pragma unroll
        for (int i = 0; i < IA; ++i) {
            if (i < cnta) {
                const int gr = k0 + arow[i];
                blds16(ra, gr < kend ? (uint32_t)((gr * lda + acol[i]) * 2) : OOB, base + (wg + i * GW) * 1024);
            }
        }
#pragma unroll
        for (int i = 0; i < IB; ++i) {
            if (i < cntb) {
                const int gr = k0 + brow[i];
                uint32_t off;
                if constexpr (CONV == 1) {
                    int n, r, c;
                    coords(gr, n, r, c);
                    const int ih = r * gS + bdh[i], iw = c * gS + bdw[i];
                    const bool ok = gr < kend && (unsigned)ih < (unsigned)gH && (unsigned)iw < (unsigned)gW;
                    off = ok ? (uint32_t)((((n * gH + ih) * gW + iw) * ldb + bcol[i]) * 2) : OOB;
                } else if constexpr (CONV == 2) {
                    int n, r, c;
                    coords(gr, n, r, c);
                    const int t = bcol[i] >> 3, ih = 2 * r - 3 + (t >> 2), sc = c - 2 + (t & 3);
                    const bool ok = gr < kend && t < 28 && (unsigned)ih < (unsigned)gH && (unsigned)sc < (unsigned)gW;
                    off = ok ? (uint32_t)(((n * gH + ih) * gW + sc) * 16) : OOB;
                } else {
                    off = gr < kend ? (uint32_t)((gr * ldb + bcol[i]) * 2) : OOB;
                }
                blds16(rb, off, base + (PA + wg + i * GW) * 1024);
            }
        }
    };
    auto vm_wait = [&](int n) {
        switch (n < 0 ? 0 : n) {
#define PLX_VMW(k) case k: asm volatile("s_waitcnt vmcnt(" #k ")" ::: "memory"); break;
            PLX_VMW(1) PLX_VMW(2) PLX_VMW(3) PLX_VMW(4) PLX_VMW(5) PLX_VMW(6) PLX_VMW(7) PLX_VMW(8)
            PLX_VMW(9) PLX_VMW(10) PLX_VMW(11) PLX_VMW(12) PLX_VMW(13) PLX_VMW(14) PLX_VMW(15) PLX_VMW(16)
            PLX_VMW(17) PLX_VMW(18) PLX_VMW(19) PLX_VMW(20) PLX_VMW(21) PLX_VMW(22) PLX_VMW(23) PLX_VMW(24)
            PLX_VMW(25) PLX_VMW(26) PLX_VMW(27) PLX_VMW(28) PLX_VMW(29) PLX_VMW(30) PLX_VMW(31) PLX_VMW(32)
#undef PLX_VMW
            default:
                if (n > 32) asm volatile("s_waitcnt vmcnt(32)" ::: "memory");
                else asm volatile("s_waitcnt vmcnt(0)" ::: "memory");
        }
    };

    f32x4 acc[4][4];
#pragma unroll
    for (int a = 0; a < 4; ++a)
#pragma unroll
        for (int b = 0; b < 4; ++b) acc[a][b] = f32x4{0.f, 0.f, 0.f, 0.f};
    const int gi = lane & 15, g4 = lane >> 4, q = gi >> 2, pp = gi & 3;
    static_assert(BKT == 32, "the asm fragment path reads one 32-deep k-step per stage");
    uint32_t aoffr[4], boffr[4];
#pragma unroll
    for (int r = 0; r < 4; ++r) {
        const int kb = 8 * g4 + q, col = r * 16 + 4 * pp;
        const int off = kb * 128 + (((col >> 3) ^ tr_swz<128>(kb)) << 4) + ((col >> 2) & 1) * 8;
        aoffr[r] = (uint32_t)(w1 * SUB + off);
        boffr[r] = (uint32_t)((NA + w2) * SUB + off);
    }

    for (int u = 0; u < R2 && u < nu; ++u) issue(u);
    if (lag) __builtin_amdgcn_s_barrier();
    for (int it = 0; it < nit; ++it) {
        vm_wait(cnt * (min(nu, R2 + it) - min(nu, it + 1)));
        __builtin_amdgcn_s_barrier();
        if (it < nu) {
            const uint32_t sa = lds_addr(gslots + (it % R2) * STAGE);
            s16x4 alo[4], ahi[4], blo[4], bhi[4];
            __builtin_amdgcn_s_setprio(1);
#pragma unroll
            for (int r = 0; r < 4; ++r) {
                alo[r] = ds_tr(sa + aoffr[r]);
                ahi[r] = ds_tr(sa + aoffr[r] + 512);
                blo[r] = ds_tr(sa + boffr[r]);
                bhi[r] = ds_tr(sa + boffr[r] + 512);
            }
            asm volatile("s_waitcnt lgkmcnt(0)"
                         : "+v"(alo[0]), "+v"(alo[1]), "+v"(alo[2]), "+v"(alo[3]), "+v"(ahi[0]), "+v"(ahi[1]),
                           "+v"(ahi[2]), "+v"(ahi[3]), "+v"(blo[0]), "+v"(blo[1]), "+v"(blo[2]), "+v"(blo[3]),
                           "+v"(bhi[0]), "+v"(bhi[1]), "+v"(bhi[2]), "+v"(bhi[3]));
            bf16x8 fa[4], fb[4];
#pragma unroll
            for (int r = 0; r < 4; ++r) {
                fa[r] = __builtin_bit_cast(bf16x8, __builtin_shufflevector(alo[r], ahi[r], 0, 1, 2, 3, 4, 5, 6, 7));
                fb[r] = __builtin_bit_cast(bf16x8, __builtin_shufflevector(blo[r], bhi[r], 0, 1, 2, 3, 4, 5, 6, 7));
            }
#pragma unroll
            for (int a = 0; a < 4; ++a)
#pragma unroll
                for (int b = 0; b < 4; ++b)
                    acc[a][b] = __builtin_amdgcn_mfma_f32_16x16x32_bf16(fa[a], fb[b], acc[a][b], 0, 0, 0);
            __builtin_amdgcn_s_setprio(0);
        }
        asm volatile("s_waitcnt lgkmcnt(0)" ::: "memory");
        __builtin_amdgcn_s_barrier();
        if (it + R2 < nu) issue(it + R2);
    }
    if (!lag) __builtin_amdgcn_s_barrier();
    asm volatile("s_waitcnt vmcnt(0) lgkmcnt(0)" ::: "memory");
    __syncthreads();
    float* red = (float*)smem;
    if (grp > 0) {
        float* dst = red + ((grp - 1) * GW + wg) * 4096 + lane;
#pragma unroll
        for (int a = 0; a < 4; ++a)
#pragma unroll
            for (int b = 0; b < 4; ++b)
#pragma unroll
                for (int r = 0; r < 4; ++r) dst[((a * 4 + b) * 4 + r) * 64] = acc[a][b][r];
    }
    __syncthreads();
    if (!ATOMIC && grp > 0) return;
    if (grp == 0) {
#pragma unroll 1
        for (int g = 1; g < KS; ++g) {
            const float* src = red + ((g - 1) * GW + wg) * 4096 + lane;
#pragma unroll
            for (int a = 0; a < 4; ++a)
#pragma unroll
                for (int b = 0; b < 4; ++b)
#pragma unroll
                    for (int r = 0; r < 4; ++r) acc[a][b][r] += src[((a * 4 + b) * 4 + r) * 64];
        }
    }
    if constexpr (ATOMIC) {
        __syncthreads();
        if (grp == 0) {
            float* t = red + wg * 4096;
#pragma unroll
            for (int a = 0; a < 4; ++a)
#pragma unroll
                for (int b = 0; b < 4; ++b)
#pragma unroll
                    for (int r = 0; r < 4; ++r) {
                        const int row = a * 16 + 4 * g4 + r, col = b * 16 + gi;
                        t[row * 64 + (col ^ (((row >> 2) & 3) << 4))] = acc[a][b][r];
                    }
        }
        __syncthreads();
#pragma unroll 4
        for (int j = wave; j < GW * 64; j += NW) {
            const int tw = j >> 6, row = j & 63;
            const float v = red[tw * 4096 + row * 64 + (lane ^ (((row >> 2) & 3) << 4))];
            float* dst = W + (size_t)(n10 + (tw / NB) * 64 + row) * ldc + n20 + (tw % NB) * 64 + lane;
            __hip_atomic_fetch_add(dst, v, __ATOMIC_RELAXED, __HIP_MEMORY_SCOPE_AGENT);
        }
        return;
    }
    float* slab = W + (size_t)slice * N1 * N2;
#pragma unroll
    for (int a = 0; a < 4; ++a)
#pragma unroll
        for (int b = 0; b < 4; ++b) {
            const int c2 = n20 + w2 * 64 + b * 16 + gi;
            const int r1 = n10 + w1 * 64 + a * 16 + 4 * g4;
#pragma unroll
            for (int r = 0; r < 4; ++r) slab[(size_t)(r1 + r) * N2 + c2] = acc[a][b][r];
        }
}

__global__ void weight_prep_kernel(const float* __restrict__ w, __bf16* __restrict__ wb, __bf16* __restrict__ wt,
                                   int cout, int cin) {
    __shared__ float tile[32][33];
    const int c0 = blockIdx.x * 32, o0 = blockIdx.y * 32;
    const int tx = threadIdx.x & 31, ty = threadIdx.x >> 5;
    for (int j = ty; j < 32; j += 8) {
        const int o = o0 + j, c = c0 + tx;
        float v = (o < cout && c < cin) ? w[(size_t)o * cin + c] : 0.f;
        tile[j][tx] = v;
        if (o < cout && c < cin) wb[(size_t)o * cin + c] = (__bf16)v;
    }
    __syncthreads();
    for (int j = ty; j < 32; j += 8) {
        const int c = c0 + j, o = o0 + tx;
        if (o < cout && c < cin) wt[(size_t)c * cout + o] = (__bf16)tile[tx][j];
    }
}

template <typename KernelT>
int set_lds(KernelT k, int bytes) {
    return hipFuncSetAttribute((const void*)k, hipFuncAttributeMaxDynamicSharedMemorySize, bytes) == hipSuccess ? 0
                                                                                                                 : -2;
}

template <int BM, int BN, int WGM, int WGN, int CONV = 0, int NBUF = 2>
int launch_nt(const void* A, const void* B, void* C, int M, int N, int K, int lda, int ldb, int ldc,
              const void* zero, float* stats, hipStream_t s, ConvGeom geo = {}, const void* D = nullptr,
              int ldd = 0, BnBwd bnr = {}, const uint8_t* dmask = nullptr) {
    constexpr int NTH = NTHREADS;
    constexpr int TILE = BM * (BN * 2 + 16), RED = NTH * 17 * 4;
    constexpr int EPI = TILE > RED ? TILE : RED;
    constexpr int KLOOP = NBUF * (BM + BN) * BK * 2;
    constexpr int LDS = KLOOP > EPI ? KLOOP : EPI;
    static_assert(NBUF >= 1 && NBUF <= 2, "one or two K stages");
    static_assert(NBUF == 1 || EPI <= KLOOP, "epilogue staging must fit the k-loop LDS");
    static_assert(LDS <= 160 * 1024, "LDS");
    constexpr int PER_CU = (160 * 1024) / LDS;
    constexpr int CAP = CONV != 0 && BN == 64 ? 3 : 4;
    constexpr int MIN_F = NBUF == 1 ? (PER_CU < CAP ? PER_CU : CAP) : 2, MIN_B = MIN_F;
    auto kf = gemm_nt_kernel<BM, BN, WGM, WGN, CONV, MIN_F, NBUF, false, NTH>;
    auto kb = gemm_nt_kernel<BM, BN, WGM, WGN, CONV, MIN_B, NBUF, true, NTH>;
    static int attr = set_lds(kf, LDS) | set_lds(kb, LDS);
    if (attr) return attr;
    const bool bwd = D != nullptr || bnr.part != nullptr;
    if (bwd && stats != nullptr) return -1;
    auto k = bwd ? kb : kf;
    const int nwg = ((M + BM - 1) / BM) * (N / BN);
    hipLaunchKernelGGL(k, dim3(nwg), dim3(NTH), LDS, s, (const __bf16*)A, (const __bf16*)B, (__bf16*)C, M, N,
                       K, lda, ldb, ldc, (const __bf16*)zero, stats, geo, (const __bf16*)D, ldd, bnr, dmask, BnDx{});
    return hipGetLastError() == hipSuccess ? 0 : -3;
}

template <int BM, int BN, int WGM, int WGN>
int launch_nt_bndx(const void* g, const BnDx& bd, const void* B, void* C, int M, int N, int K, int ldb, int ldc,
                   hipStream_t s, const void* D, int ldd, BnBwd bnr, const uint8_t* dmask) {
    constexpr int TILE = BM * (BN * 2 + 16), RED = NTHREADS * 17 * 4;
    constexpr int LDS = 2 * (BM + BN) * BK * 2;
    static_assert(TILE <= LDS && RED <= LDS && LDS <= 80 * 1024, "epilogue staging fits; 2 blocks per CU");
    auto k = gemm_nt_kernel<BM, BN, WGM, WGN, 0, 2, 2, true, NTHREADS, true>;
    static int attr = set_lds(k, LDS);
    if (attr) return attr;
    const int nwg = ((M + BM - 1) / BM) * (N / BN);
    hipLaunchKernelGGL(k, dim3(nwg), dim3(NTHREADS), LDS, s, (const __bf16*)g, (const __bf16*)B, (__bf16*)C, M, N, K, K,
                       ldb, ldc, (const __bf16*)nullptr, (float*)nullptr, ConvGeom{}, (const __bf16*)D, ldd, bnr, dmask,
                       bd);
    return hipGetLastError() == hipSuccess ? 0 : -3;
}


inline bool nt_single(bool conv, int K, int nwg) { return nwg >= 768 || (!conv && K == BK); }

struct TnPlan { int kchunk, slices, groups, per_group, blocks, bn1, bn2; };

inline void tn_tile(int N1, int N2, int& bn1, int& bn2) {
    bn1 = N1 % 128 == 0 ? 128 : 64;
    bn2 = N2 % 128 == 0 ? 128 : 64;
}

constexpr int g_tn_blocks_per_cu = 0;
constexpr int g_tn_bpc_big = 3, g_tn_bpc_mid = 1;
constexpr long g_tn_slab_bytes = 16l << 20;

inline TnPlan tn_plan(int M, int N1, int N2, int num_cus, int bpc = 0) {
    int bn1, bn2;
    tn_tile(N1, N2, bn1, bn2);
    const int ntiles = (N1 / bn1) * (N2 / bn2);
    const long plane = (long)N1 * N2;
    const int bpc_eff = bpc > 0 ? bpc
                                : (g_tn_blocks_per_cu > 0 ? g_tn_blocks_per_cu
                                                          : (M >= 400000 ? g_tn_bpc_big : M >= 150000 ? g_tn_bpc_mid : 1));
    int slices = (bpc_eff * (num_cus > 0 ? num_cus : 256)) / ntiles;
    const int by_depth = M / (4 * BK);
    const int by_bytes = (int)(g_tn_slab_bytes / (plane * 4));
    if (slices > by_depth) slices = by_depth;
    if (slices > by_bytes) slices = by_bytes;
    if (slices < 1) slices = 1;
    int kchunk = (M + slices - 1) / slices;
    kchunk = ((kchunk + BK - 1) / BK) * BK;
    slices = (M + kchunk - 1) / kchunk;
    const long total4 = plane / 4;
    int blocks = (int)((total4 + 255) / 256);
    if (blocks > 2048) blocks = 2048;
    int groups = 1024 / blocks;
    if (groups > slices / 8) groups = slices / 8;
    if (groups < 1) groups = 1;
    const int per_group = (slices + groups - 1) / groups;
    groups = (slices + per_group - 1) / per_group;
    return {kchunk, slices, groups, per_group, blocks, bn1, bn2};
}

template <int BN1, int BN2, int WG1, int WG2, int CONV, int NST, int BKT = BK>
int launch_tn_st(const void* A, const void* B, float* W, int M, int N1, int N2, int lda, int ldb, const TnPlan& plan,
                 const void* zero, hipStream_t s, const ConvGeom& geo) {
    constexpr int LDS = NST * BKT * (BN1 + BN2) * 2;
    static_assert(LDS <= 160 * 1024, "LDS ring exceeds the CU's LDS");
    auto k = gemm_tn_kernel<BN1, BN2, WG1, WG2, CONV, NST, BKT>;
    static int attr = set_lds(k, LDS);
    if (attr) return attr;
    const int ntiles = (N1 / BN1) * (N2 / BN2);
    hipLaunchKernelGGL(k, dim3(ntiles * plan.slices), dim3(NTHREADS), LDS, s, (const __bf16*)A, (const __bf16*)B, W,
                       M, N1, N2, lda, ldb, plan.kchunk, (const __bf16*)zero, geo);
    return hipGetLastError() == hipSuccess ? 0 : -3;
}

int g_tn_v2 = 1;
int g_tn2_lds_kb = 64;

struct V2Cfg { int na, nb, ks; };

inline V2Cfg v2_cfg(int N1, int N2) {
    if (N1 % 128 == 0 && N2 % 128 == 0) return {2, 2, 2};
    if (N1 % 128 != 0) {
        if (N1 == 64 && N2 % 256 == 0) return {1, 4, 2};
        if (N1 == 64 && N2 % 192 == 0) return {1, 3, 2};
        if (N1 == 64 && N2 % 128 == 0) return {1, 2, 4};
        return {1, 1, 8};
    }
    return N1 % 256 == 0 ? V2Cfg{4, 1, 2} : V2Cfg{2, 1, 4};
}

inline void plan_reducer(TnPlan& p, long plane) {
    const long total4 = plane / 4;
    int blocks = (int)((total4 + 255) / 256);
    if (blocks > 2048) blocks = 2048;
    int groups = 1024 / blocks;
    if (groups > p.slices / 8) groups = p.slices / 8;
    if (groups < 1) groups = 1;
    const int per_group = (p.slices + groups - 1) / groups;
    p.groups = (p.slices + per_group - 1) / per_group;
    p.per_group = per_group;
    p.blocks = blocks;
}

constexpr double kTnCuFlops = 3.2e12, kTnBlockUs = 2.5;
constexpr double g_tn2_slab_bw = 4.5e12;

constexpr int tn2_ring(int na, int nb, int ks, int lds_kb) {
    const int stage = (na + nb) * 32 * 128, r0 = (lds_kb * 1024) / stage, r1 = r0 > 16 ? 16 : r0, r = r1 - r1 % ks;
    return r / ks >= 2 && (ks - 1) * na * nb * 16384 <= r * stage ? r : 0;
}

inline int tn2_ring_kb(const V2Cfg& c) {
    return g_tn2_lds_kb <= 64 && tn2_ring(c.na, c.nb, c.ks, 64) ? 64 : 128;
}

constexpr int g_tn2_bpc = 0;

int g_tn2_stem = 0;

int g_tn2_c64 = 1;
constexpr int kStemV2Bpc = 2;

int g_tn_atomic = 1;

inline TnPlan tn2_plan(int M, int N1, int N2, int num_cus, const V2Cfg& c, int full_bpc = 0) {
    const int bn1 = 64 * c.na, bn2 = 64 * c.nb;
    const int ntiles = (N1 / bn1) * (N2 / bn2);
    const int ncu = num_cus > 0 ? num_cus : 256;
    const int cus = full_bpc > 0     ? ncu * full_bpc
                    : g_tn2_bpc > 2  ? g_tn2_bpc
                    : g_tn2_bpc > 0  ? ncu * g_tn2_bpc
                                     : (ncu * 3) / 4;
    const int step = 32 * c.ks;
    const long plane = (long)N1 * N2;
    const double flops = 2.0 * M * plane;
    int by_depth = M / (4 * step);
    if (by_depth < 1) by_depth = 1;
    if (by_depth > 1024) by_depth = 1024;
    int best = 1;
    double best_t = 1e30;
    for (int s = 1; s <= by_depth; ++s) {
        const long blocks = (long)ntiles * s;
        const long rounds = (blocks + cus - 1) / cus;
        const double t = flops / (kTnCuFlops * cus) * ((double)rounds * cus / blocks) + rounds * kTnBlockUs * 1e-6 +
                         (s > 1 ? (double)(s + 1) * plane * 4 / g_tn2_slab_bw : 0.0);
        if (t < best_t * 0.995) best_t = t, best = s;
    }
    int kchunk = (M + best - 1) / best;
    kchunk = ((kchunk + step - 1) / step) * step;
    TnPlan p{kchunk, (M + kchunk - 1) / kchunk, 1, 1, 0, bn1, bn2};
    plan_reducer(p, plane);
    return p;
}

template <int NA, int NB, int KS, int CONV, int LDSK, bool ATOMIC>
int launch_tn2_k(const void* A, const void* B, float* W, int M, int N1, int N2, int lda, int ldb, const TnPlan& plan,
                 hipStream_t s, const ConvGeom& geo, int ldc) {
    constexpr int BKT = 32, STAGE = (NA + NB) * BKT * 128;
    constexpr int RING = tn2_ring(NA, NB, KS, LDSK);
    static_assert(RING > 0, "ring budget too small for this configuration");
    constexpr int LDS = RING * STAGE;
    static_assert(!ATOMIC || NA * NB * 16384 <= LDS, "the atomic epilogue's tile image exceeds the ring");
    auto k = wgrad_kernel<NA, NB, KS, CONV, BKT, RING, ATOMIC>;
    static int attr = set_lds(k, LDS);
    if (attr) return attr;
    const int ntiles = (N1 / (64 * NA)) * (N2 / (64 * NB));
    hipLaunchKernelGGL(k, dim3(ntiles * plan.slices), dim3(64 * NA * NB * KS), LDS, s, (const __bf16*)A,
                       (const __bf16*)B, W, M, N1, N2, lda, ldb, plan.kchunk, geo, ldc);
    return hipGetLastError() == hipSuccess ? 0 : -3;
}

template <int NA, int NB, int KS, int CONV, bool ATOMIC>
int launch_tn2(const void* A, const void* B, float* W, int M, int N1, int N2, int lda, int ldb, const TnPlan& plan,
               hipStream_t s, const ConvGeom& geo, int ldc) {
    if constexpr (tn2_ring(NA, NB, KS, 64) > 0) {
        if (tn2_ring_kb(V2Cfg{NA, NB, KS}) <= 64)
            return launch_tn2_k<NA, NB, KS, CONV, 64, ATOMIC>(A, B, W, M, N1, N2, lda, ldb, plan, s, geo, ldc);
    }
    return launch_tn2_k<NA, NB, KS, CONV, 128, ATOMIC>(A, B, W, M, N1, N2, lda, ldb, plan, s, geo, ldc);
}

template <int CONV>
int dispatch_tn2(const V2Cfg& c, const void* A, const void* B, float* W, int M, int N1, int N2, int lda, int ldb,
                 const TnPlan& plan, hipStream_t s, const ConvGeom& geo, bool atomic = false, int ldc = 0) {
    if constexpr (CONV == 2) {
        if (c.na == 1 && c.nb == 4 && c.ks == 2)
            return atomic ? launch_tn2<1, 4, 2, 2, true>(A, B, W, M, N1, N2, lda, ldb, plan, s, geo, ldc)
                          : launch_tn2<1, 4, 2, 2, false>(A, B, W, M, N1, N2, lda, ldb, plan, s, geo, ldc);
        return -1;
    } else {
#define PLX_TN2(a, b, k) \
    if (c.na == a && c.nb == b && c.ks == k) \
        return atomic ? launch_tn2<a, b, k, CONV, true>(A, B, W, M, N1, N2, lda, ldb, plan, s, geo, ldc) \
                      : launch_tn2<a, b, k, CONV, false>(A, B, W, M, N1, N2, lda, ldb, plan, s, geo, ldc);
        PLX_TN2(2, 2, 2) PLX_TN2(1, 4, 2) PLX_TN2(1, 3, 2) PLX_TN2(1, 2, 4) PLX_TN2(1, 1, 8) PLX_TN2(4, 1, 2)
        PLX_TN2(2, 1, 4)
#undef PLX_TN2
        return -1;
    }
}

template <int BN1, int BN2, int WG1, int WG2, int CONV = 0>
int launch_tn(const void* A, const void* B, float* W, int M, int N1, int N2, int lda, int ldb, const TnPlan& plan,
              const void* zero, hipStream_t s, ConvGeom geo = {}) {
    return launch_tn_st<BN1, BN2, WG1, WG2, CONV, 2>(A, B, W, M, N1, N2, lda, ldb, plan, zero, s, geo);
}

}

extern "C" {

int plx_gemm_nt_rows_per_block(int N) { return N % 128 == 0 ? 128 : 256; }

int plx_gemm_nt(const void* A, const void* B, void* C, int M, int N, int K, int lda, int ldb, int ldc,
                const void* zero, float* stats, const void* D, int ldd, const uint8_t* dmask, const BnBwd* bnr,
                void* stream) {
    if (M <= 0 || N % 64 || K % BK || lda % 8 || ldb % 8 || ldc % 8 || (D != nullptr && ldd % 8)) return -1;
    if (dmask != nullptr && (D == nullptr || ldd != N)) return -1;
    if (bnr != nullptr && (ldc != N || bnr->part == nullptr)) return -1;
    const BnBwd b = bnr != nullptr ? *bnr : BnBwd{};
    hipStream_t s = (hipStream_t)stream;
    if (N % 128 == 0) {
        const bool one = nt_single(false, K, ((M + 127) / 128) * (N / 128));
        return one ? launch_nt<128, 128, 2, 2, false, 1>(A, B, C, M, N, K, lda, ldb, ldc, zero, stats, s, {}, D, ldd, b,
                                                         dmask)
                   : launch_nt<128, 128, 2, 2>(A, B, C, M, N, K, lda, ldb, ldc, zero, stats, s, {}, D, ldd, b, dmask);
    }
    const bool one = nt_single(false, K, ((M + 255) / 256) * (N / 64));
    return one ? launch_nt<256, 64, 4, 1, false, 1>(A, B, C, M, N, K, lda, ldb, ldc, zero, stats, s, {}, D, ldd, b, dmask)
               : launch_nt<256, 64, 4, 1>(A, B, C, M, N, K, lda, ldb, ldc, zero, stats, s, {}, D, ldd, b, dmask);
}

int plx_gemm_nt_bndx(const void* g, const void* x, const uint8_t* mask, const float* coef, void* dy, const void* Wt,
                     void* C, int M, int N, int K, int ldb, int ldc, const void* D, int ldd, const uint8_t* dmask,
                     const BnBwd* bnr, void* stream) {
    if (M <= 0 || N % 64 || K % BK || ldb % 8 || ldc % 8 || (D != nullptr && ldd % 8)) return -1;
    if (g == nullptr || x == nullptr || coef == nullptr || dy == nullptr || dy == g || dy == x) return -1;
    if ((long)M * K >= (1l << 30)) return -1;
    if (dmask != nullptr && (D == nullptr || ldd != N)) return -1;
    if (bnr != nullptr && (ldc != N || bnr->part == nullptr)) return -1;
    const BnBwd b = bnr != nullptr ? *bnr : BnBwd{};
    const BnDx bd{(const __bf16*)x, mask, coef, (__bf16*)dy};
    hipStream_t s = (hipStream_t)stream;
    if (N % 128 == 0) return launch_nt_bndx<128, 128, 2, 2>(g, bd, Wt, C, M, N, K, ldb, ldc, s, D, ldd, b, dmask);
    return launch_nt_bndx<256, 64, 4, 1>(g, bd, Wt, C, M, N, K, ldb, ldc, s, D, ldd, b, dmask);
}

int plx_tn_plan_slices(int M, int N1, int N2, int num_cus, int v2) {
    if (M <= 0 || N1 % 64 || N2 % 64) return -1;
    return v2 ? tn2_plan(M, N1, N2, num_cus, v2_cfg(N1, N2)).slices : tn_plan(M, N1, N2, num_cus).slices;
}

void plx_set_tn2_c64(int on) { g_tn2_c64 = on ? 1 : 0; }

void plx_set_tn_atomic(int on) { g_tn_atomic = on ? 1 : 0; }

void plx_set_tn2_stem(int mode) { g_tn2_stem = mode < 0 ? 0 : (mode > 2 ? 2 : mode); }

void plx_set_tn_v2(int on, int lds_kb) {
    g_tn_v2 = on < 0 ? 0 : (on > 2 ? 2 : on);
    if (lds_kb > 0) g_tn2_lds_kb = lds_kb <= 64 ? 64 : 128;
}

long plx_gemm_tn_workspace(int M, int N1, int N2, int num_cus) {
    if (M <= 0 || N1 % 64 || N2 % 64) return -1;
    const TnPlan a = tn_plan(M, N1, N2, num_cus);
    long n = a.slices + (a.groups > 1 ? a.groups : 0);
    for (int kb = 64; kb <= 128; kb += 64) {
        const int keep = g_tn2_lds_kb;
        g_tn2_lds_kb = kb;
        const TnPlan c = tn2_plan(M, N1, N2, num_cus, v2_cfg(N1, N2));
        g_tn2_lds_kb = keep;
        const long nc = c.slices + (c.groups > 1 ? c.groups : 0);
        if (nc > n) n = nc;
    }
    return n * N1 * N2;
}

}

namespace {
template <int CONV>
int run_tn(const void* A, const void* B, float* C, float* ws, int M, int N1, int N2, int lda, int ldb, int ldc,
           const void* zero, int num_cus, int accumulate, hipStream_t s, ConvGeom geo, int bpc = 0) {
    const V2Cfg cfg = v2_cfg(N1, N2);
    const bool six = cfg.na == 1 && cfg.nb == 3;
    const bool v2 = CONV == 2 ? g_tn2_stem > 0
                              : (g_tn_v2 == 1 || (g_tn_v2 == 2 && CONV != 0)) && (!six || g_tn2_c64);
    const TnPlan plan = v2 ? tn2_plan(M, N1, N2, num_cus, cfg, CONV == 2 && g_tn2_stem == 1 ? kStemV2Bpc : 0)
                           : tn_plan(M, N1, N2, num_cus, bpc);
    int rc;
    if (v2 && g_tn_atomic) {
        if (!accumulate && hipMemset2DAsync(C, (size_t)ldc * 4, 0, (size_t)N2 * 4, N1, s) != hipSuccess) return -3;
        return dispatch_tn2<CONV>(cfg, A, B, C, M, N1, N2, lda, ldb, plan, s, geo, true, ldc);
    }
    if (v2)
        rc = dispatch_tn2<CONV>(cfg, A, B, ws, M, N1, N2, lda, ldb, plan, s, geo);
    else if (N1 % 128 == 0 && N2 % 128 == 0)
        rc = launch_tn<128, 128, 2, 2, CONV>(A, B, ws, M, N1, N2, lda, ldb, plan, zero, s, geo);
    else if (N1 % 128 == 0)
        rc = launch_tn<128, 64, 4, 1, CONV>(A, B, ws, M, N1, N2, lda, ldb, plan, zero, s, geo);
    else if (N2 % 128 == 0)
        rc = launch_tn<64, 128, 1, 4, CONV>(A, B, ws, M, N1, N2, lda, ldb, plan, zero, s, geo);
    else
        rc = launch_tn<64, 64, 2, 2, CONV>(A, B, ws, M, N1, N2, lda, ldb, plan, zero, s, geo);
    if (rc) return rc;
    const long plane = (long)N1 * N2;
    const float* slabs = ws;
    int nslabs = plan.slices;
    if (plan.groups > 1) {
        float* part = ws + (long)plan.slices * plane;
        hipLaunchKernelGGL(slab_partial_kernel, dim3(plan.blocks, plan.groups), dim3(256), 0, s, ws, part, plane,
                           plan.slices, plan.per_group);
        slabs = part;
        nslabs = plan.groups;
    }
    hipLaunchKernelGGL(slab_final_kernel, dim3(plan.blocks), dim3(256), 0, s, slabs, C, N1, N2, ldc, nslabs, accumulate);
    return hipGetLastError() == hipSuccess ? 0 : -3;
}

__global__ void weight_prepk_kernel(const float* __restrict__ w, long s_co, long s_ci, long s_kh, long s_kw,
                                    __bf16* __restrict__ wf, __bf16* __restrict__ wd, int cout, int cin, int K) {
    const int taps = K * K;
    const long total = (long)cout * cin * taps;
    for (long i = blockIdx.x * (long)blockDim.x + threadIdx.x; i < total; i += (long)gridDim.x * blockDim.x) {
        const int ci = (int)(i % cin);
        const long r = i / cin;
        const int tap = (int)(r % taps), co = (int)(r / taps);
        const __bf16 v = (__bf16)w[co * s_co + ci * s_ci + (tap / K) * s_kh + (tap % K) * s_kw];
        wf[i] = v;
        wd[((long)ci * taps + tap) * cout + co] = v;
    }
}

struct WSeg {
    long src, dst_f, dst_d;
    int cout, cin, taps, tile0;
};

__global__ void __launch_bounds__(256) weight_prep_all_kernel(const float* __restrict__ base, __bf16* __restrict__ wf,
                                                              __bf16* __restrict__ wd, const WSeg* __restrict__ segs,
                                                              int nseg) {
    __shared__ float tile[32][33];
    int lo = 0, hi = nseg - 1;
    while (lo < hi) {
        const int mid = (lo + hi + 1) >> 1;
        if (segs[mid].tile0 <= (int)blockIdx.x) lo = mid;
        else hi = mid - 1;
    }
    const WSeg s = segs[lo];
    int t = blockIdx.x - s.tile0;
    const int nci = (s.cin + 31) >> 5, nco = (s.cout + 31) >> 5;
    const int ci0 = (t % nci) * 32;
    t /= nci;
    const int co0 = (t % nco) * 32, tap = t / nco;
    const int tx = threadIdx.x & 31, ty = threadIdx.x >> 5;
    for (int j = ty; j < 32; j += 8) {
        const int co = co0 + j, ci = ci0 + tx;
        float v = 0.f;
        if (co < s.cout && ci < s.cin) {
            const long e = ((long)co * s.taps + tap) * s.cin + ci;
            v = base[s.src + e];
            wf[s.dst_f + e] = (__bf16)v;
        }
        tile[j][tx] = v;
    }
    __syncthreads();
    for (int j = ty; j < 32; j += 8) {
        const int ci = ci0 + j, co = co0 + tx;
        if (co < s.cout && ci < s.cin) wd[s.dst_d + ((long)ci * s.taps + tap) * s.cout + co] = (__bf16)tile[tx][j];
    }
}
}

extern "C" {

int plx_gemm_tn(const void* A, const void* B, float* C, float* ws, int M, int N1, int N2, int lda, int ldb, int ldc,
                const void* zero, int num_cus, int accumulate, void* stream) {
    if (M <= 0 || N1 % 64 || N2 % 64 || lda % 8 || ldb % 8 || ldc % 4) return -1;
    return run_tn<false>(A, B, C, ws, M, N1, N2, lda, ldb, ldc, zero, num_cus, accumulate, (hipStream_t)stream, {});
}

}

namespace {
inline int out_dim(int H, int K, int S) { return (H + 2 * (K / 2) - K) / S + 1; }

inline ConvGeom fwd_geom(int H, int W, int C, int K, int S) {
    ConvGeom g{};
    g.H = H; g.W = W; g.Hr = out_dim(H, K, S); g.Wr = out_dim(W, K, S);
    g.C = C; g.S = S; g.ntaps = K * K; g.OS = 0;
    for (int t = 0; t < K * K; ++t) {
        g.offh[t] = (signed char)(t / K - K / 2);
        g.offw[t] = (signed char)(t % K - K / 2);
        g.btap[t] = (signed char)t;
    }
    return finish_geom(g);
}

template <int BM_, int BN_, int WGM_, int WGN_, int NBUF_>
int nt_conv(const void* A, const void* B, void* C, int M, int N, const ConvGeom& g, int ldb, int ldc,
            const void* zero, float* stats, hipStream_t s, const void* D, const BnBwd& bnr) {
    return launch_nt<BM_, BN_, WGM_, WGN_, true, NBUF_>(A, B, C, M, N, g.ntaps * g.C, g.C, ldb, ldc, zero, stats, s, g, D,
                                                 D != nullptr ? ldc : 0, bnr);
}

inline int nt_rows_per_block(int N) { return N % 128 == 0 ? 128 : 256; }

int nt_conv_any(const void* A, const void* B, void* C, int M, int N, const ConvGeom& g_in, int ldb, int ldc,
                const void* zero, float* stats, hipStream_t s, const void* D = nullptr, const BnBwd& bnr = {}) {
    ConvGeom g = g_in;
    g.tap_inner = 1;
    const int K = g.ntaps * g.C;
    if (N % 128 == 0)
        return nt_single(true, K, ((M + 127) / 128) * (N / 128))
                   ? nt_conv<128, 128, 2, 2, 1>(A, B, C, M, N, g, ldb, ldc, zero, stats, s, D, bnr)
                   : nt_conv<128, 128, 2, 2, 2>(A, B, C, M, N, g, ldb, ldc, zero, stats, s, D, bnr);
    return nt_single(true, K, ((M + 255) / 256) * (N / 64))
               ? nt_conv<256, 64, 4, 1, 1>(A, B, C, M, N, g, ldb, ldc, zero, stats, s, D, bnr)
               : nt_conv<256, 64, 4, 1, 2>(A, B, C, M, N, g, ldb, ldc, zero, stats, s, D, bnr);
}

template <typename F>
int for_each_dgrad_gemm(int Nb, int H, int W, int Cin, int Cout, int K, int S, F&& f) {
    const int Ho = out_dim(H, K, S), Wo = out_dim(W, K, S), p = K / 2;
    if (S == 1) {
        ConvGeom g = fwd_geom(Ho, Wo, Cout, K, 1);
        g.Hr = H; g.Wr = W;
        for (int t = 0; t < K * K; ++t) {
            g.offh[t] = (signed char)(p - t / K);
            g.offw[t] = (signed char)(p - t % K);
        }
        return f(finish_geom(g), Nb * H * W);
    }
    for (int ph = 0; ph < 2; ++ph)
        for (int pw = 0; pw < 2; ++pw) {
            ConvGeom g{};
            g.H = Ho; g.W = Wo; g.C = Cout; g.S = 1;
            g.Hr = (H - ph + 1) / 2; g.Wr = (W - pw + 1) / 2;
            g.Hc = H; g.Wc = W; g.OS = 2; g.oph = ph; g.opw = pw;
            int nt = 0;
            for (int kh = 0; kh < K; ++kh) {
                if ((ph + p - kh) & 1) continue;
                for (int kw = 0; kw < K; ++kw) {
                    if ((pw + p - kw) & 1) continue;
                    g.offh[nt] = (signed char)((ph + p - kh) / 2);
                    g.offw[nt] = (signed char)((pw + p - kw) / 2);
                    g.btap[nt] = (signed char)(kh * K + kw);
                    ++nt;
                }
            }
            g.ntaps = nt;
            if (nt == 0 || g.Hr <= 0 || g.Wr <= 0) continue;
            const int rc = f(finish_geom(g), Nb * g.Hr * g.Wr);
            if (rc) return rc;
        }
    return 0;
}
}

extern "C" {

int plx_conv_fwd(const void* x, const void* wf, void* y, int Nb, int H, int W, int Cin, int Cout, int K, int S,
                 const void* zero, float* stats, void* stream) {
    if (Nb <= 0 || Cin % 64 || Cout % 64 || (K != 1 && K != 3) || (S != 1 && S != 2)) return -1;
    const ConvGeom g = fwd_geom(H, W, Cin, K, S);
    return nt_conv_any(x, wf, y, Nb * g.Hr * g.Wr, Cout, g, K * K * Cin, Cout, zero, stats, (hipStream_t)stream);
}

int plx_conv_dgrad(const void* dy, const void* wd, void* dx, int Nb, int H, int W, int Cin, int Cout, int K, int S,
                   const void* zero, const void* D, const BnBwd* bnr, void* stream) {
    if (Nb <= 0 || Cin % 64 || Cout % 64 || (K != 1 && K != 3) || (S != 1 && S != 2)) return -1;
    if (bnr != nullptr && (S == 2 && K == 1) && bnr->blk_off == 0) return -1;
    hipStream_t st = (hipStream_t)stream;
    BnBwd b = bnr != nullptr ? *bnr : BnBwd{};
    const int rpb = nt_rows_per_block(Cin);
    return for_each_dgrad_gemm(Nb, H, W, Cin, Cout, K, S, [&](const ConvGeom& g, int M) {
        const int rc = nt_conv_any(dy, wd, dx, M, Cin, g, K * K * Cout, Cin, zero, nullptr, st, D, b);
        b.blk_off += (M + rpb - 1) / rpb;
        return rc;
    });
}

int plx_conv_dgrad_blocks(int Nb, int H, int W, int Cin, int Cout, int K, int S) {
    int total = 0;
    const int rpb = nt_rows_per_block(Cin);
    const int rc = for_each_dgrad_gemm(Nb, H, W, Cin, Cout, K, S, [&](const ConvGeom&, int M) {
        total += (M + rpb - 1) / rpb;
        return 0;
    });
    return rc ? rc : total;
}

long plx_conv_wgrad_workspace(int Nb, int H, int W, int Cin, int Cout, int K, int S, int num_cus) {
    return plx_gemm_tn_workspace(Nb * out_dim(H, K, S) * out_dim(W, K, S), Cout, K * K * Cin, num_cus);
}

int plx_conv_wgrad(const void* dy, const void* x, float* dw, float* ws, int Nb, int H, int W, int Cin, int Cout, int K,
                   int S, const void* zero, int num_cus, int accumulate, void* stream) {
    if (Nb <= 0 || Cin % 64 || Cout % 64 || (K != 1 && K != 3) || (S != 1 && S != 2)) return -1;
    const ConvGeom g = fwd_geom(H, W, Cin, K, S);
    const int M = Nb * g.Hr * g.Wr;
    return run_tn<true>(dy, x, dw, ws, M, Cout, K * K * Cin, Cout, Cin, K * K * Cin, zero, num_cus, accumulate,
                        (hipStream_t)stream, g);
}

int plx_weight_prepk(const float* w, long s_co, long s_ci, long s_kh, long s_kw, void* wf, void* wd, int cout, int cin,
                     int K, void* stream) {
    const long total = (long)cout * cin * K * K;
    int blocks = (int)((total + 255) / 256);
    if (blocks > 4096) blocks = 4096;
    hipLaunchKernelGGL(weight_prepk_kernel, dim3(blocks), dim3(256), 0, (hipStream_t)stream, w, s_co, s_ci, s_kh, s_kw,
                       (__bf16*)wf, (__bf16*)wd, cout, cin, K);
    return hipGetLastError() == hipSuccess ? 0 : -3;
}

int plx_weight_prep_all(const float* base, void* wf, void* wd, const void* segs, int nseg, int total_tiles,
                        void* stream) {
    static_assert(sizeof(WSeg) == 40, "WSeg layout is shared with ops/wcache.py");
    if (nseg <= 0 || total_tiles <= 0) return -1;
    hipLaunchKernelGGL(weight_prep_all_kernel, dim3(total_tiles), dim3(256), 0, (hipStream_t)stream, base,
                       (__bf16*)wf, (__bf16*)wd, (const WSeg*)segs, nseg);
    return hipGetLastError() == hipSuccess ? 0 : -3;
}

__global__ void stem_pack_input_kernel(const uint32_t* __restrict__ x, uint4* __restrict__ xp, long n_sp) {
    for (long i = blockIdx.x * (long)blockDim.x + threadIdx.x; i < n_sp; i += (long)gridDim.x * blockDim.x) {
        const uint32_t d0 = x[3 * i], d1 = x[3 * i + 1], d2 = x[3 * i + 2];
        xp[i] = make_uint4(d0, d1 & 0xffffu, (d1 >> 16) | (d2 << 16), d2 >> 16);
    }
}

__global__ void stem_pack_weight_kernel(const float* __restrict__ w, long s_co, long s_ci, long s_kh, long s_kw,
                                        __bf16* __restrict__ wp, int cout) {
    const int e = blockIdx.x * blockDim.x + threadIdx.x;
    if (e >= cout * 256) return;
    const int co = e >> 8, k = e & 255, t = k >> 3, px = (k >> 2) & 1, ch = k & 3;
    const int kh = t >> 2, kw = 2 * (t & 3) - 1 + px;
    const bool ok = t < 28 && ch < 3 && kw >= 0 && kw < 7;
    wp[e] = (__bf16)(ok ? w[co * s_co + ch * s_ci + kh * s_kh + kw * s_kw] : 0.f);
}

__global__ void stem_unpack_wgrad_kernel(const float* __restrict__ packed, float* __restrict__ dw, long s_co, long s_ci,
                                         long s_kh, long s_kw, int accumulate) {
    const int e = blockIdx.x * blockDim.x + threadIdx.x;
    if (e >= 64 * 147) return;
    const int co = e / 147, r = e % 147, ci = r / 49, kh = (r % 49) / 7, kw = r % 7;
    const int j = (kw + 1) >> 1, px = (kw + 1) & 1;
    const float v = packed[co * 256 + (kh * 4 + j) * 8 + px * 4 + ci];
    float* d = dw + co * s_co + ci * s_ci + kh * s_kh + kw * s_kw;
    *d = accumulate ? *d + v : v;
}

int plx_weight_prep(const float* w, void* wb, void* wt, int cout, int cin, void* stream) {
    dim3 grid((cin + 31) / 32, (cout + 31) / 32);
    hipLaunchKernelGGL(weight_prep_kernel, grid, dim3(256), 0, (hipStream_t)stream, w, (__bf16*)wb, (__bf16*)wt, cout,
                       cin);
    return hipGetLastError() == hipSuccess ? 0 : -3;
}

}

extern "C" {

int plx_stem_pack_input(const void* x, void* xp, int N, int H, int W, void* stream) {
    if (N <= 0 || H <= 0 || W <= 0 || (W & 1)) return -1;
    const long n_sp = (long)N * H * (W / 2);
    long blocks = (n_sp + 255) / 256;
    if (blocks > 8192) blocks = 8192;
    hipLaunchKernelGGL(stem_pack_input_kernel, dim3((int)blocks), dim3(256), 0, (hipStream_t)stream, (const uint32_t*)x,
                       (uint4*)xp, n_sp);
    return hipGetLastError() == hipSuccess ? 0 : -3;
}

int plx_stem_pack_weight(const float* w, long s_co, long s_ci, long s_kh, long s_kw, void* wp, int cout, void* stream) {
    hipLaunchKernelGGL(stem_pack_weight_kernel, dim3((cout * 256 + 255) / 256), dim3(256), 0, (hipStream_t)stream, w,
                       s_co, s_ci, s_kh, s_kw, (__bf16*)wp, cout);
    return hipGetLastError() == hipSuccess ? 0 : -3;
}

constexpr int kStemWgradBpc = 4;

static long stem_slabs(int M, int num_cus) {
    const TnPlan p = tn_plan(M, 64, 256, num_cus, kStemWgradBpc);
    const TnPlan q = tn2_plan(M, 64, 256, num_cus, v2_cfg(64, 256));
    const TnPlan r = tn2_plan(M, 64, 256, num_cus, v2_cfg(64, 256), kStemV2Bpc);
    const long a = p.slices + (p.groups > 1 ? p.groups : 0), b = q.slices + (q.groups > 1 ? q.groups : 0);
    const long c = r.slices + (r.groups > 1 ? r.groups : 0);
    return a > b ? (a > c ? a : c) : (b > c ? b : c);
}

long plx_stem_conv_wgrad_workspace(int N, int H, int W, int num_cus) {
    const int M = N * ((H - 1) / 2 + 1) * ((W - 1) / 2 + 1);
    return stem_slabs(M, num_cus) * 64 * 256 + 64 * 256;
}

int plx_stem_conv_wgrad(const void* dy, const void* xp, float* dw, long s_co, long s_ci, long s_kh, long s_kw,
                        float* ws, int N, int H, int W, const void* zero, int num_cus, int accumulate, void* stream) {
    if (N <= 0 || H <= 0 || W <= 0 || (W & 1)) return -1;
    ConvGeom g{};
    g.H = H;
    g.W = W / 2;
    g.Hr = (H - 1) / 2 + 1;
    g.Wr = (W - 1) / 2 + 1;
    g.mWr = div_magic(g.Wr);
    g.mHr = div_magic(g.Hr);
    const int M = N * g.Hr * g.Wr;
    float* packed = ws + stem_slabs(M, num_cus) * 64 * 256;
    hipStream_t s = (hipStream_t)stream;
    const int rc = run_tn<2>(dy, xp, packed, ws, M, 64, 256, 64, 8, 256, zero, num_cus, 0, s, g, kStemWgradBpc);
    if (rc) return rc;
    hipLaunchKernelGGL(stem_unpack_wgrad_kernel, dim3((64 * 147 + 255) / 256), dim3(256), 0, s, packed, dw, s_co, s_ci,
                       s_kh, s_kw, accumulate);
    return hipGetLastError() == hipSuccess ? 0 : -3;
}

int plx_stem_conv_rows_per_block() { return 256; }

int plx_stem_conv_fwd(const void* xp, const void* wp, void* y, int N, int H, int W, const void* zero, float* stats,
                      void* stream) {
    if (N <= 0 || H <= 0 || W <= 0 || (W & 1)) return -1;
    ConvGeom g{};
    g.H = H;
    g.W = W / 2;
    g.Hr = (H - 1) / 2 + 1;
    g.Wr = (W - 1) / 2 + 1;
    g.mWr = div_magic(g.Wr);
    g.mHr = div_magic(g.Hr);
    const int M = N * g.Hr * g.Wr;
    return nt_single(true, 256, (M + 255) / 256)
               ? launch_nt<256, 64, 4, 1, 2, 1>(xp, wp, y, M, 64, 256, 8, 256, 64, zero, stats, (hipStream_t)stream, g)
               : launch_nt<256, 64, 4, 1, 2, 2>(xp, wp, y, M, 64, 256, 8, 256, 64, zero, stats, (hipStream_t)stream, g);
}

}
```

### polyaxon_amd/models/resnet.py

```python
from __future__ import annotations

from typing import List, Optional, Type

import torch
import torch.nn as nn

from polyaxon_amd.ops.conv1x1 import Conv1x1, GradMailbox
from polyaxon_amd.ops.conv import Conv3x3, ConvKxK
from polyaxon_amd.ops.norm import BatchNormAct
from polyaxon_amd.ops.pool import MaxPool3s2, global_avg_pool
from polyaxon_amd.ops.stem import StemConv, stem_bn_relu_pool


class Bottleneck(nn.Module):
    expansion = 4

    def __init__(self, in_ch: int, width: int, stride: int = 1, downsample: Optional[nn.Module] = None,
                 fused: bool = True, native_conv: bool = True):
        super().__init__()
        out_ch = width * self.expansion
        self.conv1 = Conv1x1(in_ch, width, native=native_conv)
        self.bn1 = BatchNormAct(width, act=True, fused=fused)
        self.conv2 = Conv3x3(width, width, stride, native=native_conv)
        self.bn2 = BatchNormAct(width, act=True, fused=fused)
        self.conv3 = Conv1x1(width, out_ch, native=native_conv)
        self.bn3 = BatchNormAct(out_ch, act=True, fused=fused, residual=True)
        self.downsample = downsample

    def forward(self, x: torch.Tensor) -> torch.Tensor:
        train = self.training and torch.is_grad_enabled() and x.requires_grad
        box = GradMailbox() if train else None
        if self.downsample is None:
            out = self.bn1(self.conv1(x, grad_box=box, bn_link=True))
            out = self.bn2(self.conv2(out, bn_link=True))
            return self.bn3(self.conv3(out, bn_link=True), x, residual_grad_box=box)
        identity = self.downsample(x, grad_box=box)
        out = self.bn1(self.conv1(x, grad_sink=box, bn_link=True))
        out = self.bn2(self.conv2(out, bn_link=True))
        return self.bn3(self.conv3(out, bn_link=True), identity, residual_link=True)




class Downsample(nn.Module):
    def __init__(self, in_ch: int, out_ch: int, stride: int, fused: bool = True, native_conv: bool = True):
        super().__init__()
        self.conv = (Conv1x1(in_ch, out_ch, native=native_conv) if stride == 1
                     else ConvKxK(in_ch, out_ch, 1, stride, native=native_conv))
        self.bn = BatchNormAct(out_ch, act=False, fused=fused)

    def forward(self, x: torch.Tensor, grad_box: Optional[GradMailbox] = None) -> torch.Tensor:
        return self.bn(self.conv(x, grad_box=grad_box, bn_link=True), defer_apply=True)


class ResNet(nn.Module):
    def __init__(self, layers: List[int], num_classes: int = 1000, width: int = 64,
                 zero_init_residual: bool = True, fused: bool = True, native_conv: bool = True):
        super().__init__()
        self.stem = (StemConv(3, width, native=native_conv) if width == 64
                     else nn.Conv2d(3, width, 7, stride=2, padding=3, bias=False))
        self.stem_bn = BatchNormAct(width, act=True, fused=fused)
        self.pool = MaxPool3s2(native=native_conv)
        stages = []
        in_ch = width
        for i, n in enumerate(layers):
            w = width * (2 ** i)
            stride = 1 if i == 0 else 2
            blocks = []
            for j in range(n):
                ds = None
                if j == 0 and (stride != 1 or in_ch != w * Bottleneck.expansion):
                    ds = Downsample(in_ch, w * Bottleneck.expansion, stride, fused=fused, native_conv=native_conv)
                blocks.append(Bottleneck(in_ch, w, stride if j == 0 else 1, ds, fused=fused, native_conv=native_conv))
                in_ch = w * Bottleneck.expansion
            stages.append(nn.Sequential(*blocks))
        self.stages = nn.Sequential(*stages)
        self.fc = nn.Linear(in_ch, num_classes)
        self.zero_init_residual = zero_init_residual
        self.reset_parameters()

    def init_spec(self):
        spec = []
        for name, mod in self.named_modules():
            if isinstance(mod, nn.Conv2d):
                fan_out = mod.out_channels * mod.kernel_size[0] * mod.kernel_size[1]
                spec.append((mod.weight, "normal", (2.0 / fan_out) ** 0.5))
            elif isinstance(mod, BatchNormAct):
                gamma = 0.0 if (self.zero_init_residual and mod.residual) else 1.0
                spec.append((mod.weight, "const", gamma))
                spec.append((mod.bias, "const", 0.0))
            elif isinstance(mod, nn.Linear):
                bound = 1.0 / mod.in_features ** 0.5
                spec.append((mod.weight, "uniform", bound))
                spec.append((mod.bias, "uniform", bound))
        return spec

    @torch.no_grad()
    def reset_parameters(self) -> None:
        for p, kind, scale in self.init_spec():
            if kind == "normal":
                p.normal_(0.0, scale)
            elif kind == "const":
                p.fill_(scale)
            else:
                p.uniform_(-scale, scale)
        for mod in self.modules():
            if isinstance(mod, BatchNormAct):
                mod.reset_running_stats()

    def forward_features(self, x: torch.Tensor) -> torch.Tensor:
        x = self.stem(x)
        x = stem_bn_relu_pool(x, self.stem_bn, self.pool)
        return self.stages(x)

    def forward_head(self, x: torch.Tensor) -> torch.Tensor:
        x = torch.flatten(x.mean((2, 3)), 1) if x.is_contiguous() else global_avg_pool(x)
        return self.fc(x)

    def forward(self, x: torch.Tensor) -> torch.Tensor:
        return self.forward_head(self.forward_features(x))


def resnet50(num_classes: int = 1000, fused: bool = True, **kw) -> ResNet:
    return ResNet([3, 4, 6, 3], num_classes=num_classes, fused=fused, **kw)


def resnet18ish(num_classes: int = 10, fused: bool = True, **kw) -> ResNet:
    return ResNet([1, 1, 1, 1], num_classes=num_classes, width=8, fused=fused, **kw)
```

### polyaxon_amd/ops/_native.py

```python
from __future__ import annotations

import ctypes
import hashlib
import os
import shutil
import subprocess
import threading
from pathlib import Path
from typing import Dict, Iterable, List, Optional

PKG_DIR = Path(__file__).resolve().parent.parent
CSRC = PKG_DIR / "csrc"
OUT = PKG_DIR / "_native"
ARCH = os.environ.get("PLX_OFFLOAD_ARCH", "gfx950")
ROCM = Path(os.environ.get("ROCM_PATH", "/opt/rocm"))

LIBRARIES: Dict[str, dict] = {
    "plx_train": {"sources": ["train_kernels.hip"], "kind": "hip", "link": []},
    "plx_polytune": {"sources": ["polytune_kernels.hip"], "kind": "hip", "link": []},
    "plx_bn": {"sources": ["bn_kernels.hip"], "kind": "hip", "link": []},
    "plx_procmon": {"sources": ["procmon.cpp"], "kind": "cpp", "link": ["-lpthread"]},
    "plx_gp": {"sources": ["gp_kernels.hip", "gp_chol.hip"], "kind": "hip", "link": []},
    "plx_rms": {"sources": ["rmsnorm.hip"], "kind": "hip", "link": []},
    "plx_conv": {"sources": ["conv_gemm.hip"], "kind": "hip", "link": []},
    "plx_pool": {"sources": ["pool_kernels.hip"], "kind": "hip", "link": []},
    "plx_lm": {"sources": ["lm_kernels.hip"], "kind": "hip", "link": []},
    "plx_gemm": {"sources": ["gemm256.hip"], "kind": "hip", "link": []},
    "plx_attn": {"sources": ["attn_kernels.hip"], "kind": "hip", "link": []},
    "plx_rccl": {"sources": ["rccl_comm.cpp"], "kind": "hip_host", "link": ["-lrccl", "-pthread"]},
}

_lock = threading.Lock()
_loaded: Dict[str, ctypes.CDLL] = {}


def _register(name: str, sources: List[str], kind: str, link: Optional[List[str]] = None) -> None:
    LIBRARIES[name] = {"sources": sources, "kind": kind, "link": list(link or [])}


def lib_path(name: str) -> Path:
    return OUT / f"lib{name}.so"


def _digest(sources: Iterable[Path], flags: List[str]) -> str:
    h = hashlib.sha256()
    for s in sources:
        h.update(s.read_bytes())
    for hdr in sorted(CSRC.glob("*.h")):
        h.update(hdr.read_bytes())
    h.update(" ".join(flags).encode())
    return h.hexdigest()[:16]


def _flags(kind: str) -> List[str]:
    common = ["-O3", "-std=c++17", "-shared", "-fPIC", "-Wall", "-Wno-unused-function", f"-I{CSRC}"]
    if kind == "hip":
        fences = ["-DPLX_HANDOFF_FENCES=1"] if os.environ.get("PLX_HANDOFF_FENCES") == "1" else []
        return common + [f"--offload-arch={ARCH}", "-munsafe-fp-atomics"] + fences
    if kind == "hip_host":
        return common + [f"-I{ROCM / 'include'}", "-D__HIP_PLATFORM_AMD__"]
    return common


def build(name: str, force: bool = False, verbose: bool = False) -> Path:
    spec = LIBRARIES[name]
    srcs = [CSRC / s for s in spec["sources"]]
    flags = _flags(spec["kind"])
    out = lib_path(name)
    stamp = out.with_suffix(".so.sha")
    digest = _digest(srcs, flags + spec["link"])
    if not force and out.exists() and stamp.exists() and stamp.read_text().strip() == digest:
        return out
    OUT.mkdir(parents=True, exist_ok=True)
    if spec["kind"] in ("hip", "hip_host"):
        cc = shutil.which("hipcc") or str(ROCM / "bin" / "hipcc")
    else:
        cc = shutil.which("g++") or "g++"
    link = list(spec["link"])
    if spec["kind"] == "hip_host":
        link = [f"-L{ROCM / 'lib'}", f"-Wl,-rpath,{ROCM / 'lib'}"] + link + ["-lamdhip64"]
    tmp = out.with_suffix(f".so.tmp{os.getpid()}")
    cmd = [cc, *flags, *map(str, srcs), "-o", str(tmp), *link]
    if verbose:
        print(" ".join(cmd))
    proc = subprocess.run(cmd, capture_output=True, text=True)
    if proc.returncode != 0:
        raise RuntimeError(f"native build of {name} failed:\n{' '.join(cmd)}\n{proc.stderr[-6000:]}")
    os.replace(tmp, out)
    stamp.write_text(digest)
    return out


def _stale(name: str) -> bool:
    spec = LIBRARIES[name]
    stamp = lib_path(name).with_suffix(".so.sha")
    if not stamp.exists():
        return False
    try:
        digest = _digest([CSRC / s for s in spec["sources"]], _flags(spec["kind"]) + spec["link"])
    except OSError:
        return False
    return stamp.read_text().strip() != digest


def build_all(force: bool = False, verbose: bool = False) -> List[Path]:
    return [build(n, force=force, verbose=verbose) for n in LIBRARIES]


def available(name: str) -> bool:
    return lib_path(name).exists()


_SIZES: Dict[tuple, int] = {}


_COUNTERS: Dict[tuple, object] = {}


def capturing() -> bool:
    import torch

    return torch.cuda.is_available() and torch.cuda.is_current_stream_capturing()


def cached(cache: dict, key, make, ok=None):
    v = cache.get(key)
    if v is not None and (ok is None or ok(v)):
        return v
    v = make()
    if not capturing():
        cache[key] = v
    return v


def counters(device, key: str, n: int = 4096):
    import torch

    return cached(_COUNTERS, (str(device), key), lambda: torch.zeros(n, dtype=torch.int32, device=device))


def current_stream() -> int:
    import torch

    return torch._C._cuda_getCurrentRawStream(torch._C._cuda_getDevice())


def size(libname: str, fn: str, *args: int) -> int:
    key = (fn,) + args
    v = _SIZES.get(key)
    if v is None:
        v = _SIZES[key] = int(getattr(lib(libname), fn)(*args))
    return v


def lib(name: str) -> ctypes.CDLL:
    with _lock:
        if name in _loaded:
            return _loaded[name]
        path = lib_path(name)
        if not path.exists() or os.environ.get("PLX_NATIVE_REBUILD") == "1" or _stale(name):
            build(name, force=os.environ.get("PLX_NATIVE_REBUILD") == "1")
        handle = ctypes.CDLL(str(path), mode=ctypes.RTLD_GLOBAL)
        _declare(name, handle)
        if name == "plx_conv" and os.environ.get("PLX_WGRAD_ATOMIC"):
            handle.plx_set_tn_atomic(int(os.environ["PLX_WGRAD_ATOMIC"]))
        if name == "plx_gemm" and os.environ.get("PLX_GEMM_WAVES"):
            handle.plx_gemm256_set_waves(int(os.environ["PLX_GEMM_WAVES"]))
        _loaded[name] = handle
        return handle


_P = ctypes.c_void_p
_I = ctypes.c_int
_L = ctypes.c_int64
_U64 = ctypes.c_uint64
_F = ctypes.c_float
_D = ctypes.c_double

SIGNATURES: Dict[str, Dict[str, list]] = {
    "plx_train": {
        "plx_sgd_flat": [_P, _P, _P, _L, _L, _P, _P, _P],
        "plx_adamw_flat": [_P, _P, _P, _P, _L, _L, _P, _P, _P],
        "plx_adamw_mixed": [_P, _P, _P, _P, _P, _L, _I, _P, _P, _P],
        "plx_sgd_flat_clip": [_P, _P, _P, _L, _L, _P, _P, _P, _P],
        "plx_adamw_flat_clip": [_P, _P, _P, _P, _L, _L, _P, _P, _P, _P],
        "plx_adamw_mixed_clip": [_P, _P, _P, _P, _P, _L, _I, _P, _P, _P, _P],
        "plx_gradnorm_blocks": [_L],
        "plx_gradnorm_partials": [_P, _I, _L, _P, _P],
        "plx_gradnorm_finalize": [_P, _I, _P, _P, _P],
        "plx_cast_lp": [_P, _P, _L, _P],
        "plx_init_flat": [_P, _P, _P, _P, _I, _P, _P, _U64, _P],
        "plx_zero_flat": [_P, _L, _P],
        "plx_record_metric": [_P, _I, _P, _P, _I, _P],
        "plx_commit_metric": [_P, _P, _I, _I, _P, _I, _P],
        "plx_synth_images": [_P, _P, _I, _I, _I, _P, _I, _I, _F, _U64, _P, _P],
        "plx_set_adamw_grid_cap": [_I],
        "plx_set_adamw_wide": [_I],
    },
    "plx_bn": {
        "plx_bn_workspace": [_L, _I],
        "plx_bn_forward": [_P, _P, _P, _L, _I, _P, _P, _F, _F, _P, _P, _P, _P, _P, _P, _P, _I, _P, _P, _P],
        "plx_bn_apply": [_P, _P, _P, _L, _I, _P, _I, _P],
        "plx_bn_l2_workspace": [_I, _I],
        "plx_bn_forward_from_partials": [_P, _P, _P, _L, _I, _P, _P, _F, _F, _P, _P, _P, _P, _P, _P, _I, _P, _P,
                                         _I, _P, _P, _P],
        "plx_bn_backward": [_P, _P, _P, _P, _P, _L, _I, _P, _P, _P, _P, _P, _P, _P, _I, _I, _P, _P, _P],
        "plx_bn_dx_blocks": [_L, _I],
        "plx_bn_backward_from_partials": [_P, _P, _P, _P, _P, _L, _I, _P, _P, _P, _P, _P, _P, _P, _I, _P, _I, _I, _P,
                                          _P, _P],
        "plx_bn_backward_coef": [_P, _P, _P, _L, _I, _P, _P, _P, _P, _P, _P, _P, _I, _I, _P, _P],
        "plx_bn_backward_coef_from_partials": [_L, _I, _P, _P, _P, _P, _P, _P, _P, _I, _P, _I, _P, _P],
        "plx_stem_bn_pool_forward": [_P, _P, _P, _I, _I, _I, _I, _P, _P, _F, _F, _P, _P, _P, _P, _P, _P, _P, _I, _P,
                                     _P],
        "plx_stem_bn_pool_bwd_workspace": [_I, _I, _I, _I],
        "plx_stem_bn_pool_backward": [_P, _P, _P, _P, _I, _I, _I, _I, _P, _P, _P, _P, _P, _P, _P, _P, _I, _P, _P],
    },
    "plx_procmon": {
        "plx_pm_create": [],
        "plx_pm_destroy": [_P],
        "plx_pm_spawn": [_P, _P, _P, ctypes.c_char_p, ctypes.c_char_p, ctypes.POINTER(_I)],
        "plx_pm_wait": [_P, _I, ctypes.POINTER(_I), ctypes.POINTER(_I)],
        "plx_pm_wake": [_P],
        "plx_pm_signal": [_P, _I, _I, _I],
        "plx_pm_count": [_P],
    },
    "plx_gp": {
        "plx_gp_kmat": [_P, _P, _I, _I, _I, _P, _I, _I, _F, _F, _F, _I, _F, _P, _P, _D, _I, _P],
        "plx_gp_chol": [_P, _I, _I, _P, _P],
        "plx_gp_kmat_batch_f64": [_P, _I, _I, _P, _I, _P, _I, _L, _I, _D, _D, _D, _P, _P, _D, _I, _P],
        "plx_gp_matern_table": [_D, _D, _D, _I, _P, _P, _P],
        "plx_gp_chol_aug_f64": [_P, _I, _I, _I, _L, _I, _P, _P, _P],
        "plx_gp_chol_scratch_doubles": [],
        "plx_gp_lml_f64": [_P, _I, _I, _L, _I, _P, _P, _P],
        "plx_gp_acq_rows": [_P, _I, _I, _P, _F, _I, _F, _F, _F, _P, _P, _P, _P],
        "plx_gp_predict_acq": [_P, _I, _P, _I, _I, _P, _I, _P, _I, _F, _F, _F, _F, _I, _F, _F, _F, _P, _P, _P, _P,
                               _P, _P, _P, _D, _I, _P],
        "plx_gp_ascent": [_P, _P, _I, _P, _P, _P, _I, _I, _P, _P, _I, _F, _F, _F, _F, _I, _F, _F, _F, _I, _P, _P, _D, _I,
                          _P],
    },
    "plx_conv": {
        "plx_gemm_nt": [_P, _P, _P, _I, _I, _I, _I, _I, _I, _P, _P, _P, _I, _P, _P, _P],
        "plx_gemm_nt_bndx": [_P, _P, _P, _P, _P, _P, _P, _I, _I, _I, _I, _I, _P, _I, _P, _P, _P],
        "plx_gemm_nt_rows_per_block": [_I],
        "plx_gemm_tn_workspace": [_I, _I, _I, _I],
        "plx_set_tn_v2": [_I, _I],
        "plx_set_tn2_stem": [_I],
        "plx_set_tn2_c64": [_I],
        "plx_set_tn_atomic": [_I],
        "plx_tn_plan_slices": [_I, _I, _I, _I, _I],
        "plx_gemm_tn": [_P, _P, _P, _P, _I, _I, _I, _I, _I, _I, _P, _I, _I, _P],
        "plx_weight_prep": [_P, _P, _P, _I, _I, _P],
        "plx_weight_prepk": [_P, _L, _L, _L, _L, _P, _P, _I, _I, _I, _P],
        "plx_weight_prep_all": [_P, _P, _P, _P, _I, _I, _P],
        "plx_stem_pack_input": [_P, _P, _I, _I, _I, _P],
        "plx_stem_pack_weight": [_P, _L, _L, _L, _L, _P, _I, _P],
        "plx_stem_conv_rows_per_block": [],
        "plx_stem_conv_fwd": [_P, _P, _P, _I, _I, _I, _P, _P, _P],
        "plx_stem_conv_wgrad_workspace": [_I, _I, _I, _I],
        "plx_stem_conv_wgrad": [_P, _P, _P, _L, _L, _L, _L, _P, _I, _I, _I, _P, _I, _I, _P],
        "plx_conv_fwd": [_P, _P, _P, _I, _I, _I, _I, _I, _I, _I, _P, _P, _P],
        "plx_conv_dgrad": [_P, _P, _P, _I, _I, _I, _I, _I, _I, _I, _P, _P, _P, _P],
        "plx_conv_dgrad_blocks": [_I, _I, _I, _I, _I, _I, _I],
        "plx_conv_wgrad_workspace": [_I, _I, _I, _I, _I, _I, _I, _I],
        "plx_conv_wgrad": [_P, _P, _P, _P, _I, _I, _I, _I, _I, _I, _I, _P, _I, _I, _P],
    },
    "plx_lm": {
        "plx_qkv_rope_fwd": [_P, _P, _P, _P, _P, _P, _L, _I, _I, _I, _I, _I, _P],
        "plx_qkv_rope_bwd": [_P, _P, _P, _P, _P, _P, _L, _I, _I, _I, _I, _I, _P],
        "plx_swiglu_fwd": [_P, _P, _L, _I, _P],
        "plx_swiglu_bwd": [_P, _P, _P, _L, _I, _P],
        "plx_xent_fwd": [_P, _P, _P, _P, _I, _I, _I, _P],
        "plx_xent_bwd": [_P, _P, _P, _P, _P, _I, _I, _I, _P],
        "plx_xent_cls_fwd": [_P, _P, _P, _P, _I, _I, _P],
        "plx_xent_cls_bwd": [_P, _P, _P, _P, _P, _I, _I, _F, _P],
        "plx_colsum_splits": [_L, _I],
        "plx_colsum": [_P, _L, _I, _P, _P, _P, _I, _P],
        "plx_gelu_bwd_colsum": [_P, _P, _P, _L, _I, _P, _P, _P, _I, _P],
    },
    "plx_gemm": {
        "plx_gemm256": [_P, _P, _P, _P, _I, _I, _I, _I, _I, _I, _I, _I, _F, _I, _P],
        "plx_gemm256_bias": [_P, _P, _P, _P, _I, _I, _I, _I, _I, _I, _I, _I, _F, _I, _P, _P],
        "plx_gemm256_ex": [_P, _P, _P, _P, _I, _I, _I, _I, _I, _I, _I, _I, _F, _I, _P, _P, _P],
        "plx_gemm256_exv": [_P, _P, _P, _P, _I, _I, _I, _I, _I, _I, _I, _I, _F, _I, _P, _P, _I, _P],
        "plx_gemm256_splits": [_I, _I, _I],
        "plx_gemm256_set_split_target": [_I],
        "plx_gemm256_set_waves": [_I],
        "plx_gemm256_set_group": [_I],
        "plx_gemm256_tile": [],
        "plx_gemm256_sk_ws": [_I, _I, _I],
        "plx_gemm256_sk_plan": [_I, _I, _I, ctypes.POINTER(_I), ctypes.POINTER(_I)],
        "plx_gemm256_set_sk_force": [_I],
        "plx_gemm256_sk": [_P, _P, _P, _P, _P, _I, _I, _I, _I, _I, _I, _I, _I, _F, _P, _P, _P, _P],
    },
    "plx_attn": {
        "plx_attn_fwd": [_P, _I, _P],
        "plx_attn_bwd": [_P, _I, _P, _P],
        "plx_attn_bwd_workspace": [_I, _I, _I, _I, _I],
        "plx_attn_args_size": [],
        "plx_attn_set_fwd_waves": [_I],
        "plx_attn_set_dq_waves": [_I],
        "plx_attn_set_dkdv_waves": [_I],
    },
    "plx_pool": {
        "plx_maxpool3s2_forward": [_P, _P, _P, _I, _I, _I, _I, _P],
        "plx_gap_forward": [_P, _P, _I, _I, _I, _P],
        "plx_gap_backward": [_P, _P, _I, _I, _I, _P],
        "plx_maxpool3s2_backward": [_P, _P, _P, _I, _I, _I, _I, _P],
    },
    "plx_rms": {
        "plx_rms_forward": [_P, _P, _P, _P, _L, _I, _F, _P],
        "plx_rms_bwd_blocks": [_L],
        "plx_ln_bwd_blocks": [_L, _I],
        "plx_add_ln_forward": [_P, _P, _P, _P, _P, _P, _P, _P, _L, _I, _F, _P],
        "plx_add_rms_forward": [_P, _P, _P, _P, _P, _P, _L, _I, _F, _P],
        "plx_add_rms_backward": [_P, _P, _P, _P, _P, _P, _P, _L, _I, _P],
        "plx_add_ln_backward": [_P, _P, _P, _P, _P, _P, _P, _P, _P, _L, _I, _P],
        "plx_partial_colsum_workspace": [_I, _I, _I],
        "plx_partial_colsum": [_P, _P, _I, _I, _I, _P, _P, _P, _P, _I, _I, _P],
        "plx_rms_backward": [_P, _P, _P, _P, _P, _P, _L, _I, _P],
        "plx_ln_forward": [_P, _P, _P, _P, _P, _P, _L, _I, _F, _P],
        "plx_ln_backward": [_P, _P, _P, _P, _P, _P, _P, _P, _L, _I, _P],
    },
    "plx_rccl": {
        "plx_rccl_unique_id": [ctypes.c_char_p],
        "plx_rccl_init": [ctypes.c_char_p, _I, _I, _I, _L, _L, ctypes.POINTER(_I)],
        "plx_rccl_all_reduce": [_P, _P, _P, _L, _I, _I, _P],
        "plx_rccl_all_gather": [_P, _P, _P, _L, _I, _P],
        "plx_rccl_reduce_scatter": [_P, _P, _P, _L, _I, _I, _P],
        "plx_rccl_broadcast": [_P, _P, _P, _L, _I, _I, _P],
        "plx_rccl_bus_bw": [_P, _P, _L, _I, _P, ctypes.POINTER(_D), ctypes.POINTER(_D)],
        "plx_rccl_destroy": [_P],
        "plx_rccl_status": [_P],
        "plx_rccl_pending": [_P],
        "plx_rccl_set_timeout": [_P, _L],
        "plx_rccl_abort": [_P],
        "plx_rccl_error": [_I],
    },
    "plx_polytune": {
        "plx_topk_brackets": [_P, _P, _I, _I, _I, _I, _P, _P],
        "plx_philox_sample": [_P, _P, _I, _L, _L, ctypes.c_uint64, _P, _P],
        "plx_philox_desc_size": [],
        "plx_early_stop_any": [_P, _I, _I, _P, _P, _P, _I, _P, _P],
    },
}


RESTYPES: Dict[str, object] = {"plx_attn_bwd_workspace": ctypes.c_longlong, "plx_conv_wgrad_workspace": _L, "plx_bn_workspace": _L, "plx_bn_l2_workspace": _L, "plx_partial_colsum_workspace": _L, "plx_stem_bn_pool_bwd_workspace": _L, "plx_gemm_tn_workspace": _L, "plx_gemm256_sk_ws": ctypes.c_longlong, "plx_stem_conv_wgrad_workspace": _L, "plx_pm_create": _P, "plx_pm_destroy": None, "plx_set_tn_v2": None, "plx_set_tn2_stem": None, "plx_set_tn2_c64": None, "plx_set_tn_atomic": None, "plx_set_adamw_grid_cap": None, "plx_set_adamw_wide": None, "plx_attn_set_fwd_waves": None, "plx_attn_set_dq_waves": None, "plx_attn_set_dkdv_waves": None, "plx_gemm256_set_split_target": None,
                               "plx_pm_wake": None, "plx_rccl_init": _P, "plx_rccl_error": ctypes.c_char_p}


def _declare(name: str, handle: ctypes.CDLL) -> None:
    for fn, argtypes in SIGNATURES.get(name, {}).items():
        f = getattr(handle, fn)
        f.argtypes = argtypes
        f.restype = RESTYPES.get(fn, _I)


class ResBnArgs(ctypes.Structure):
    _fields_ = [("x", _P), ("mask", _P), ("mean", _P), ("invstd", _P), ("part", _P)]


class BnBwdArgs(ctypes.Structure):
    _fields_ = [("x", _P), ("mask", _P), ("mean", _P), ("invstd", _P), ("part", _P), ("part_ld", _I),
                ("blk_off", _I), ("skip_h", _I), ("skip_w", _I)]


def check(rc: int, what: str) -> None:
    if rc != 0:
        raise RuntimeError(f"{what} failed with code {rc}")
```

### polyaxon_amd/ops/bn_fused.py

```python
from __future__ import annotations

import ctypes

from typing import Optional

import torch

from polyaxon_amd.ops import _native
from polyaxon_amd.ops.conv1x1 import BnLink
from polyaxon_amd.ops.flat import direct_grad


def _stream() -> int:
    return _native.current_stream()


_COUNTERS = {}


def _counters(dev: torch.device):
    key = (dev.index, torch.cuda.current_stream(dev).cuda_stream)
    return _native.cached(_COUNTERS, key, lambda: torch.zeros(64, dtype=torch.int32, device=dev)).data_ptr()


def _cl(t: torch.Tensor) -> torch.Tensor:
    return t if t.is_contiguous(memory_format=torch.channels_last) else t.contiguous(memory_format=torch.channels_last)


def supported(x: torch.Tensor) -> bool:
    if not x.is_cuda or x.dtype != torch.bfloat16 or x.dim() != 4:
        return False
    c = x.shape[1]
    g = c // 8
    return c % 8 == 0 and g > 0 and (g & (g - 1)) == 0 and x.numel() > 0


class _BNAct(torch.autograd.Function):
    @staticmethod
    def forward(ctx, x, weight, bias, running_mean, running_var, residual, momentum, eps, relu, ext=None, box=None,
                link=None, rlink=None, defer=False, dxsink=None):
        lib = _native.lib("plx_bn")
        ctx.dxsink = dxsink if x.is_contiguous(memory_format=torch.channels_last) else None
        x = _cl(x)
        n, c, h, w = x.shape
        m = n * h * w
        ws = _native.size("plx_bn", "plx_bn_workspace", m, c)
        if ws < 0:
            raise RuntimeError("unsupported channel count for fused BN")
        f32 = dict(dtype=torch.float32, device=x.device)
        defer = bool(defer) and not relu and residual is None and link is not None
        y = None if defer else torch.empty_like(x, memory_format=torch.channels_last)
        yp = y.data_ptr() if y is not None else None
        stats = torch.empty(4 * c, **f32)
        res_sb = None
        if residual is not None:
            rl = getattr(residual, "_plx_bn_link", None)
            if rl is not None and rl.affine is not None and getattr(residual, "_plx_deferred", False):
                res_sb = rl.affine
        res = _cl(residual) if residual is not None else None
        rsp = res_sb.data_ptr() if res_sb is not None else None
        rm = running_mean.data_ptr() if running_mean is not None else None
        rv = running_var.data_ptr() if running_var is not None else None
        mask = torch.empty(m * c // 8, dtype=torch.uint8, device=x.device) if relu else None
        mp = mask.data_ptr() if mask is not None else None
        if ext is not None:
            part, nblk = ext
            l2 = torch.empty(_native.size("plx_bn", "plx_bn_l2_workspace", nblk, c), **f32)
            rc = lib.plx_bn_forward_from_partials(
                x.data_ptr(), res.data_ptr() if res is not None else None, yp, m, c, weight.data_ptr(),
                bias.data_ptr(), float(eps), float(momentum), rm, rv, stats.data_ptr(), stats[c:].data_ptr(),
                stats[2 * c:].data_ptr(), part.data_ptr(), nblk, l2.data_ptr(), mp, int(relu), rsp,
                _counters(x.device), _stream())
            _native.check(rc, "plx_bn_forward_from_partials")
        else:
            partials = torch.empty(ws, **f32)
            rc = lib.plx_bn_forward(
                x.data_ptr(), res.data_ptr() if res is not None else None, yp, m, c,
                weight.data_ptr(), bias.data_ptr(), float(eps), float(momentum), rm, rv,
                stats.data_ptr(), stats[c:].data_ptr(), stats[2 * c:].data_ptr(), partials.data_ptr(), mp, int(relu),
                rsp, _counters(x.device), _stream())
            _native.check(rc, "plx_bn_forward")
        ctx.save_for_backward(x, mask, weight, stats)
        ctx.relu = relu
        ctx.has_res = residual is not None
        ctx.box = box if (box is not None and box.armed and residual is not None) else None
        if ctx.box is not None:
            ctx.box.expect = True
        ctx.ws = ws
        gw, gb = direct_grad(weight), direct_grad(bias)
        ctx.direct = (gw, gb) if (gw is not None and gb is not None) else None
        ctx.link = link
        if link is not None:
            link.x, link.mask, link.mean, link.invstd = x, mask, stats[:c], stats[c:2 * c]
            if defer:
                link.affine = stats[2 * c:]
        ctx.rlink = rlink if (rlink is not None and residual is not None and rlink.x is not None
                              and rlink.x.shape == x.shape and ctx.box is None) else None
        if defer:
            return x.view_as(x)
        return y

    @staticmethod
    def backward(ctx, dy):
        lib = _native.lib("plx_bn")
        x, mask, weight, stats = ctx.saved_tensors
        n, c, h, w = x.shape
        m = n * h * w
        dy = _cl(dy)
        if dy.dtype != torch.bfloat16:
            dy = dy.to(torch.bfloat16)
        f32 = dict(dtype=torch.float32, device=x.device)
        dx = torch.empty_like(x, memory_format=torch.channels_last)
        masked_box = ctx.box is not None and ctx.relu and mask is not None
        dres = (torch.empty_like(x, memory_format=torch.channels_last)
                if ctx.has_res and not masked_box else None)
        if ctx.direct is not None:
            dg_ptr, db_ptr, acc = ctx.direct[0].data_ptr(), ctx.direct[1].data_ptr(), 1
            dgb = None
        else:
            dgb = torch.empty(2 * c, **f32)
            dg_ptr, db_ptr, acc = dgb.data_ptr(), dgb[c:].data_ptr(), 0
        coef = torch.empty(3 * c, **f32)
        part, nblk = ctx.link.take() if ctx.link is not None else (None, 0)
        if ctx.dxsink is not None and dres is None:
            if part is not None:
                l2 = torch.empty(_native.size("plx_bn", "plx_bn_l2_workspace", nblk, c), **f32)
                rc = lib.plx_bn_backward_coef_from_partials(
                    m, c, weight.data_ptr(), stats.data_ptr(), stats[c:].data_ptr(), dg_ptr, db_ptr, coef.data_ptr(),
                    part.data_ptr(), nblk, l2.data_ptr(), acc, _counters(x.device), _stream())
                _native.check(rc, "plx_bn_backward_coef_from_partials")
            else:
                partials = torch.empty(ctx.ws, **f32)
                rc = lib.plx_bn_backward_coef(
                    x.data_ptr(), mask.data_ptr() if mask is not None else None, dy.data_ptr(), m, c,
                    weight.data_ptr(), stats.data_ptr(), stats[c:].data_ptr(), dg_ptr, db_ptr, coef.data_ptr(),
                    partials.data_ptr(), int(ctx.relu), acc, _counters(x.device), _stream())
                _native.check(rc, "plx_bn_backward_coef")
            ctx.dxsink.put(dy, x, mask if ctx.relu else None, coef, dx)
            if ctx.box is not None:
                ctx.box.put_masked(dy, mask)
            dgamma = dgb[:c] if dgb is not None else None
            dbeta = dgb[c:] if dgb is not None else None
            return dx, dgamma, dbeta, None, None, None, None, None, None, None, None, None, None, None, None
        rb = None
        if ctx.rlink is not None and dres is not None:
            rl = ctx.rlink
            nblk2 = _native.size("plx_bn", "plx_bn_dx_blocks", m, c)
            rl.part = torch.empty(2 * nblk2 * c, **f32)
            rl.nblk = nblk2
            rb = _native.ResBnArgs(rl.x.data_ptr(), rl.mask.data_ptr() if rl.mask is not None else None,
                                   rl.mean.data_ptr(), rl.invstd.data_ptr(), rl.part.data_ptr())
        rbp = ctypes.addressof(rb) if rb is not None else None
        if part is not None:
            l2 = torch.empty(_native.size("plx_bn", "plx_bn_l2_workspace", nblk, c), **f32)
            rc = lib.plx_bn_backward_from_partials(
                x.data_ptr(), mask.data_ptr() if mask is not None else None, dy.data_ptr(), dx.data_ptr(),
                dres.data_ptr() if dres is not None else None, m, c, weight.data_ptr(), stats.data_ptr(),
                stats[c:].data_ptr(), dg_ptr, db_ptr, coef.data_ptr(), part.data_ptr(), nblk, l2.data_ptr(),
                int(ctx.relu), acc, rbp, _counters(x.device), _stream())
            _native.check(rc, "plx_bn_backward_from_partials")
        else:
            partials = torch.empty(ctx.ws, **f32)
            rc = lib.plx_bn_backward(
                x.data_ptr(), mask.data_ptr() if mask is not None else None, dy.data_ptr(), dx.data_ptr(),
                dres.data_ptr() if dres is not None else None, m, c, weight.data_ptr(), stats.data_ptr(),
                stats[c:].data_ptr(), dg_ptr, db_ptr, coef.data_ptr(), partials.data_ptr(), int(ctx.relu), acc,
                rbp, _counters(x.device), _stream())
            _native.check(rc, "plx_bn_backward")
        if ctx.box is not None:
            if masked_box:
                ctx.box.put_masked(dy, mask)
            else:
                ctx.box.put(dres)
            dres = None
        dgamma = dgb[:c] if dgb is not None else None
        dbeta = dgb[c:] if dgb is not None else None
        return dx, dgamma, dbeta, None, None, dres, None, None, None, None, None, None, None, None, None


class _Materialize(torch.autograd.Function):

    @staticmethod
    def forward(ctx, t, sb):
        c = t.shape[1]
        return (t.float() * sb[:c].view(1, c, 1, 1) + sb[c:].view(1, c, 1, 1)).to(t.dtype).contiguous(
            memory_format=torch.channels_last)

    @staticmethod
    def backward(ctx, g):
        return g, None


def materialize(t: Optional[torch.Tensor]) -> Optional[torch.Tensor]:
    if t is None or not getattr(t, "_plx_deferred", False):
        return t
    return _Materialize.apply(t, t._plx_bn_link.affine)


def bn_act(x: torch.Tensor, weight: torch.Tensor, bias: torch.Tensor, running_mean: Optional[torch.Tensor],
           running_var: Optional[torch.Tensor], training: bool, momentum: float, eps: float,
           residual: Optional[torch.Tensor], act: bool, ext_stats=None, residual_grad_box=None,
           residual_link: bool = False, defer_apply: bool = False, dx_sink=None) -> torch.Tensor:
    if residual is not None and residual.dtype != x.dtype:
        residual = residual.to(x.dtype)
    if training:
        link = BnLink()
        rlink = getattr(residual, "_plx_bn_link", None) if (residual_link and residual is not None) else None
        defer = bool(defer_apply) and not act and residual is None
        y = _BNAct.apply(x, weight, bias, running_mean, running_var, residual, momentum, eps, act, ext_stats,
                         residual_grad_box, link, rlink, defer, dx_sink)
        y._plx_bn_link = link
        if defer:
            y._plx_deferred = True
        return y
    residual = materialize(residual)
    lib = _native.lib("plx_bn")
    x = _cl(x)
    n, c, h, w = x.shape
    inv = torch.rsqrt(running_var.float() + eps)
    scale = weight.float() * inv
    sb = torch.cat([scale, bias.float() - running_mean.float() * scale]).contiguous()
    y = torch.empty_like(x, memory_format=torch.channels_last)
    res = _cl(residual) if residual is not None else None
    rc = lib.plx_bn_apply(x.data_ptr(), res.data_ptr() if res is not None else None, y.data_ptr(), n * h * w, c,
                          sb.data_ptr(), int(act), _stream())
    _native.check(rc, "plx_bn_apply")
    return y
```

### polyaxon_amd/ops/conv1x1.py

```python
from __future__ import annotations

import ctypes
import os
from typing import Dict

import torch
import torch.nn as nn
import torch.nn.functional as F

from polyaxon_amd.ops import _native, side_stream, wcache
from polyaxon_amd.ops.flat import direct_grad

_ZERO: Dict[int, torch.Tensor] = {}
_CUS: Dict[int, int] = {}

_BN_DX_FUSED = os.environ.get("PLX_BN_DX_FUSED", "1") != "0"


def set_bn_dx_fused(on: bool) -> bool:
    global _BN_DX_FUSED
    prev, _BN_DX_FUSED = _BN_DX_FUSED, bool(on)
    return prev


def _zero_page(dev: torch.device) -> torch.Tensor:
    idx = dev.index if dev.index is not None else torch.cuda.current_device()
    return _native.cached(_ZERO, idx, lambda: torch.zeros(256, dtype=torch.bfloat16, device=dev))


def _num_cus(dev: torch.device) -> int:
    idx = dev.index if dev.index is not None else torch.cuda.current_device()
    if idx not in _CUS:
        _CUS[idx] = torch.cuda.get_device_properties(idx).multi_processor_count
    return _CUS[idx]


def _stream() -> int:
    return _native.current_stream()


def nt_stats_rows(n: int) -> int:
    return _native.size("plx_conv", "plx_gemm_nt_rows_per_block", n)


def gemm_nt(a: torch.Tensor, b: torch.Tensor, out: torch.Tensor = None, stats: torch.Tensor = None,
            add: torch.Tensor = None, bnr: "_native.BnBwdArgs" = None, add_mask: torch.Tensor = None) -> torch.Tensor:
    m, k = a.shape
    n = b.shape[0]
    if out is None:
        out = torch.empty(m, n, dtype=torch.bfloat16, device=a.device)
    assert a.stride(1) == 1 and b.stride(1) == 1 and out.stride(1) == 1 and b.shape[1] == k
    assert a.data_ptr() % 16 == 0 and b.data_ptr() % 16 == 0 and out.data_ptr() % 16 == 0
    if stats is not None:
        nblk = -(-m // nt_stats_rows(n))
        assert stats.dtype == torch.float32 and stats.is_contiguous() and stats.numel() >= 2 * nblk * n
    if add is not None:
        assert add.shape == (m, n) and add.stride(1) == 1 and add.dtype == torch.bfloat16 and add.data_ptr() % 16 == 0
    if add_mask is not None:
        assert add is not None and add.stride(0) == n and add_mask.dtype == torch.uint8 and add_mask.numel() == m * n // 8
    rc = _native.lib("plx_conv").plx_gemm_nt(a.data_ptr(), b.data_ptr(), out.data_ptr(), m, n, k, a.stride(0),
                                             b.stride(0), out.stride(0), _zero_page(a.device).data_ptr(),
                                             stats.data_ptr() if stats is not None else None,
                                             add.data_ptr() if add is not None else None,
                                             add.stride(0) if add is not None else 0,
                                             add_mask.data_ptr() if add_mask is not None else None,
                                             ctypes.addressof(bnr) if bnr is not None else None, _stream())
    _native.check(rc, "plx_gemm_nt")
    return out


def gemm_nt_bndx(g: torch.Tensor, x: torch.Tensor, mask: torch.Tensor, coef: torch.Tensor, dy: torch.Tensor,
                 b: torch.Tensor, out: torch.Tensor = None, add: torch.Tensor = None,
                 bnr: "_native.BnBwdArgs" = None, add_mask: torch.Tensor = None) -> torch.Tensor:
    m, k = g.shape
    n = b.shape[0]
    if out is None:
        out = torch.empty(m, n, dtype=torch.bfloat16, device=g.device)
    for t in (g, x, dy):
        assert t.shape == (m, k) and t.dtype == torch.bfloat16 and t.stride() == (k, 1) and t.data_ptr() % 16 == 0
    assert b.stride(1) == 1 and out.stride(1) == 1 and b.shape[1] == k and b.dtype == torch.bfloat16
    assert b.data_ptr() % 16 == 0 and out.data_ptr() % 16 == 0
    assert coef.dtype == torch.float32 and coef.is_contiguous() and coef.numel() == 3 * k
    if mask is not None:
        assert mask.dtype == torch.uint8 and mask.numel() == m * k // 8
    if add is not None:
        assert add.shape == (m, n) and add.stride(1) == 1 and add.dtype == torch.bfloat16 and add.data_ptr() % 16 == 0
    if add_mask is not None:
        assert add is not None and add.stride(0) == n and add_mask.dtype == torch.uint8 and add_mask.numel() == m * n // 8
    rc = _native.lib("plx_conv").plx_gemm_nt_bndx(g.data_ptr(), x.data_ptr(),
                                                  mask.data_ptr() if mask is not None else None, coef.data_ptr(),
                                                  dy.data_ptr(), b.data_ptr(), out.data_ptr(), m, n, k, b.stride(0),
                                                  out.stride(0), add.data_ptr() if add is not None else None,
                                                  add.stride(0) if add is not None else 0,
                                                  add_mask.data_ptr() if add_mask is not None else None,
                                                  ctypes.addressof(bnr) if bnr is not None else None, _stream())
    _native.check(rc, "plx_gemm_nt_bndx")
    return out


def gemm_tn(a: torch.Tensor, b: torch.Tensor, out: torch.Tensor = None, accumulate: bool = False) -> torch.Tensor:
    m, n1 = a.shape
    n2 = b.shape[1]
    if out is None:
        out = torch.empty(n1, n2, dtype=torch.float32, device=a.device)
        accumulate = False
    assert a.stride(1) == 1 and b.stride(1) == 1 and out.stride(1) == 1 and b.shape[0] == m
    assert a.data_ptr() % 16 == 0 and b.data_ptr() % 16 == 0 and out.data_ptr() % 16 == 0
    lib = _native.lib("plx_conv")
    cus = _num_cus(a.device)
    ws = torch.empty(_native.size("plx_conv", "plx_gemm_tn_workspace", m, n1, n2, cus), dtype=torch.float32,
                     device=a.device)
    rc = lib.plx_gemm_tn(a.data_ptr(), b.data_ptr(), out.data_ptr(), ws.data_ptr(), m, n1, n2, a.stride(0),
                         b.stride(0), out.stride(0), _zero_page(a.device).data_ptr(), cus, int(accumulate),
                         _stream())
    _native.check(rc, "plx_gemm_tn")
    return out


def weight_prep(w: torch.Tensor):
    cout, cin = w.shape[0], w.shape[1]
    wb = torch.empty(cout, cin, dtype=torch.bfloat16, device=w.device)
    wt = torch.empty(cin, cout, dtype=torch.bfloat16, device=w.device)
    w32 = w.reshape(cout, cin)
    if w32.dtype != torch.float32 or not w32.is_contiguous():
        w32 = w32.float().contiguous()
    rc = _native.lib("plx_conv").plx_weight_prep(w32.data_ptr(), wb.data_ptr(), wt.data_ptr(), cout, cin, _stream())
    _native.check(rc, "plx_weight_prep")
    return wb, wt


class GradMailbox:

    __slots__ = ("armed", "grad", "mask", "expect", "s2k1")

    def __init__(self):
        self.armed = False
        self.grad = None
        self.mask = None
        self.expect = False
        self.s2k1 = False

    def put(self, g: torch.Tensor) -> None:
        if self.grad is not None:
            g = self._dense() + g
        self.grad, self.mask = g, None

    def put_masked(self, g: torch.Tensor, mask: torch.Tensor) -> None:
        if self.grad is not None:
            self.put(unpack_relu_mask(g, mask))
            return
        self.grad, self.mask = g, mask

    def _dense(self) -> torch.Tensor:
        return self.grad if self.mask is None else unpack_relu_mask(self.grad, self.mask)

    def take(self):
        g, m = self.grad, self.mask
        self.grad = self.mask = None
        if g is None and self.expect:
            raise RuntimeError("GradMailbox: the deferred gradient did not arrive before its consumer's backward")
        return g, m


def unpack_relu_mask(g: torch.Tensor, mask: torch.Tensor) -> torch.Tensor:
    bits = (mask.view(-1, 1) >> torch.arange(8, device=mask.device, dtype=torch.uint8)) & 1
    n, c, h, w = g.shape
    keep = bits.view(n, h, w, c).permute(0, 3, 1, 2).to(g.dtype)
    return (g * keep).contiguous(memory_format=torch.channels_last)


class DxSink:

    __slots__ = ("payload",)

    def __init__(self):
        self.payload = None

    def put(self, g: torch.Tensor, x: torch.Tensor, mask, coef: torch.Tensor, dx: torch.Tensor) -> None:
        self.payload = (g, x, mask, coef, dx)

    def take(self):
        p, self.payload = self.payload, None
        return p


def dx_sink_for(x: torch.Tensor, weight: torch.Tensor):
    if not _BN_DX_FUSED or not (torch.is_grad_enabled() and x.requires_grad):
        return None
    cout, cin = weight.shape[0], weight.shape[1]
    return DxSink() if (cout >= 2 * cin and cin <= 128) else None


class BnLink:

    __slots__ = ("x", "mask", "mean", "invstd", "part", "nblk", "_args", "affine", "split")

    def __init__(self, x=None, mask=None, mean=None, invstd=None):
        self.x, self.mask, self.mean, self.invstd = x, mask, mean, invstd
        self.affine = None
        self.part = None
        self.nblk = 0
        self._args = None
        self.split = 0

    def _args_for(self, nblk_total: int, blk_off: int) -> "_native.BnBwdArgs":
        return _native.BnBwdArgs(self.x.data_ptr(), self.mask.data_ptr() if self.mask is not None else None,
                                 self.mean.data_ptr(), self.invstd.data_ptr(), self.part.data_ptr(), nblk_total,
                                 blk_off)

    def request(self, nblk: int) -> "_native.BnBwdArgs":
        c = self.x.shape[1]
        self.part = torch.empty(2 * nblk * c, dtype=torch.float32, device=self.x.device)
        self.nblk, self.split = nblk, 0
        self._args = self._args_for(nblk, 0)
        return self._args

    def request_split(self, nblk1: int, nblk2: int) -> "_native.BnBwdArgs":
        n, c, h, w = self.x.shape
        self.part = torch.empty(2 * (nblk1 + nblk2) * c, dtype=torch.float32, device=self.x.device)
        self.nblk, self.split = nblk1 + nblk2, nblk1
        a = self._args_for(nblk1 + nblk2, 0)
        a.skip_h, a.skip_w = h, w
        self._args = a
        return a

    def request_rest(self) -> "_native.BnBwdArgs":
        a = self._args_for(self.nblk, self.split)
        self.split = 0
        self._args = a
        return a

    def take(self):
        part, nblk = self.part, self.nblk
        if self.split:
            part, nblk = None, 0
        self.part, self._args, self.split = None, None, 0
        return part, nblk


def _rows(t: torch.Tensor) -> torch.Tensor:
    n, c, h, w = t.shape
    return t.permute(0, 2, 3, 1).reshape(n * h * w, c)


def bn_link_of(x: torch.Tensor, want: bool):
    link = getattr(x, "_plx_bn_link", None) if want else None
    return link if (link is not None and link.x is not None and link.x.shape == x.shape) else None


class _Conv1x1(torch.autograd.Function):
    @staticmethod
    def forward(ctx, x, weight, stats, box, sink, link, dxsink=None):
        x = x.to(torch.bfloat16).contiguous(memory_format=torch.channels_last)
        ctx.box = box
        ctx.dxsink = dxsink
        ctx.sink = sink if (sink is not None and sink.armed) else None
        if ctx.sink is not None:
            ctx.sink.expect = True
        ctx.link = link if (sink is None or sink.armed) else None
        ctx.wgrad = direct_grad(weight)
        n, cin, h, w = x.shape
        cout = weight.shape[0]
        wb, wt = wcache.lookup(weight) or weight_prep(weight)
        y = torch.empty((n, cout, h, w), dtype=torch.bfloat16, device=x.device, memory_format=torch.channels_last)
        gemm_nt(_rows(x), wb, _rows(y), stats)
        ctx.save_for_backward(x, wt)
        ctx.wshape = weight.shape
        ctx.wdtype = weight.dtype
        return y

    @staticmethod
    def backward(ctx, dy):
        x, wt = ctx.saved_tensors
        n, cin, h, w = x.shape
        fused = ctx.dxsink.take() if ctx.dxsink is not None else None
        if fused is not None and (dy.data_ptr() != fused[4].data_ptr() or dy.shape != fused[4].shape
                                  or dy.dtype != torch.bfloat16 or not ctx.needs_input_grad[0]):
            raise RuntimeError("DxSink: the BatchNorm's deferred input gradient was replaced before the convolution's "
                               "backward could fill it")
        dy = dy.to(torch.bfloat16).contiguous(memory_format=torch.channels_last)
        dx = dw = None
        extra, extra_mask = ctx.box.take() if ctx.box is not None else (None, None)
        if ctx.needs_input_grad[0]:
            dx = torch.empty_like(x, memory_format=torch.channels_last)
            if extra is not None and (extra.dtype != torch.bfloat16
                                      or not extra.is_contiguous(memory_format=torch.channels_last)):
                if extra_mask is not None:
                    extra, extra_mask = unpack_relu_mask(extra, extra_mask), None
                extra = extra.to(torch.bfloat16).contiguous(memory_format=torch.channels_last)
            bnr = None
            rows = nt_stats_rows(cin)
            if ctx.link is not None and ctx.sink is None and (ctx.box is None or extra is not None):
                bnr = ctx.link.request(-(-(n * h * w) // rows))
            elif ctx.link is not None and ctx.sink is not None and ctx.sink.s2k1 and extra is None:
                bnr = ctx.link.request_split(-(-(n * h * w) // rows), -(-(n * ((h + 1) // 2) * ((w + 1) // 2)) // rows))
            if fused is not None:
                g, bx, bmask, coef, _ = fused
                gemm_nt_bndx(_rows(g), _rows(bx), bmask, coef, _rows(dy), wt, _rows(dx),
                             add=_rows(extra) if extra is not None else None, bnr=bnr, add_mask=extra_mask)
            else:
                gemm_nt(_rows(dy), wt, _rows(dx), add=_rows(extra) if extra is not None else None, bnr=bnr,
                        add_mask=extra_mask)
            if ctx.sink is not None:
                ctx.sink.put(dx)
                dx = None
        if ctx.needs_input_grad[1]:
            cout = ctx.wshape[0]
            if ctx.wgrad is not None:
                slot = ctx.wgrad.as_strided((cout, cin), (cin, 1))
                side_stream.run(lambda: gemm_tn(_rows(dy), _rows(x), out=slot, accumulate=True), (dy, x), x.device)
            else:
                dw = gemm_tn(_rows(dy), _rows(x)).view(ctx.wshape).to(ctx.wdtype)
        return dx, dw, None, None, None, None, None


def _bf16_context(x: torch.Tensor) -> bool:
    if x.dtype == torch.bfloat16:
        return True
    return torch.is_autocast_enabled("cuda") and torch.get_autocast_dtype("cuda") == torch.bfloat16


def supported(x: torch.Tensor, conv: nn.Conv2d) -> bool:
    return (x.is_cuda and x.dim() == 4 and _bf16_context(x) and conv.kernel_size == (1, 1) and conv.stride == (1, 1)
            and conv.padding == (0, 0) and conv.groups == 1 and conv.bias is None
            and conv.in_channels % 64 == 0 and conv.out_channels % 64 == 0 and x.numel() > 0)


def conv1x1(x: torch.Tensor, weight: torch.Tensor, with_stats: bool = False,
            grad_box: "GradMailbox" = None, grad_sink: "GradMailbox" = None, bn_link: bool = False) -> torch.Tensor:
    stats = None
    if with_stats:
        n, _, h, w = x.shape
        m, cout = n * h * w, weight.shape[0]
        nblk = -(-m // nt_stats_rows(cout))
        stats = torch.empty(2 * nblk * cout, dtype=torch.float32, device=x.device)
    if grad_box is not None:
        grad_box.armed = True
    dxsink = dx_sink_for(x, weight)
    y = _Conv1x1.apply(x, weight, stats, grad_box, grad_sink, bn_link_of(x, bn_link), dxsink)
    if stats is not None:
        y._plx_channel_stats = (stats, nblk)
    if dxsink is not None:
        y._plx_dx_sink = dxsink
    return y


class Conv1x1(nn.Conv2d):

    def __init__(self, in_ch: int, out_ch: int, stride: int = 1, native: bool = True, bn_stats: bool = True):
        super().__init__(in_ch, out_ch, 1, stride=stride, bias=False)
        self.native = native
        self.bn_stats = bn_stats

    def forward(self, x: torch.Tensor, grad_box: GradMailbox = None, grad_sink: GradMailbox = None,
                bn_link: bool = False) -> torch.Tensor:
        if self.native and supported(x, self):
            return conv1x1(x, self.weight, with_stats=self.bn_stats and self.training, grad_box=grad_box,
                           grad_sink=grad_sink, bn_link=bn_link)
        return F.conv2d(x, self.weight, None, self.stride)
```

### polyaxon_amd/ops/norm.py

```python
from __future__ import annotations

from typing import Optional

import torch
import torch.nn as nn
import torch.nn.functional as F


def bn_act_reference(x: torch.Tensor, weight: torch.Tensor, bias: torch.Tensor,
                     running_mean: Optional[torch.Tensor], running_var: Optional[torch.Tensor],
                     training: bool, momentum: float, eps: float, residual: Optional[torch.Tensor],
                     act: bool) -> torch.Tensor:
    y = F.batch_norm(x, running_mean, running_var, weight, bias, training, momentum, eps)
    if residual is not None:
        y = y + residual
    if act:
        y = F.relu(y)
    return y


class BatchNormAct(nn.Module):
    def __init__(self, num_features: int, act: bool = True, residual: bool = False, fused: bool = True,
                 eps: float = 1e-5, momentum: float = 0.1):
        super().__init__()
        self.num_features = num_features
        self.act = act
        self.residual = residual
        self.fused = fused
        self.eps = eps
        self.momentum = momentum
        self.weight = nn.Parameter(torch.ones(num_features))
        self.bias = nn.Parameter(torch.zeros(num_features))
        self.register_buffer("running_mean", torch.zeros(num_features))
        self.register_buffer("running_var", torch.ones(num_features))

    def reset_running_stats(self) -> None:
        with torch.no_grad():
            self.running_mean.zero_()
            self.running_var.fill_(1.0)

    def forward(self, x: torch.Tensor, identity: Optional[torch.Tensor] = None, residual_grad_box=None,
                residual_link: bool = False, defer_apply: bool = False) -> torch.Tensor:
        if self.residual and identity is None:
            raise ValueError("BatchNormAct(residual=True) needs the identity tensor")
        if self.fused and x.is_cuda:
            from polyaxon_amd.ops import bn_fused
            if bn_fused.supported(x):
                ext = getattr(x, "_plx_channel_stats", None)
                return bn_fused.bn_act(x, self.weight, self.bias, self.running_mean, self.running_var,
                                       self.training, self.momentum, self.eps, identity, self.act, ext,
                                       residual_grad_box, residual_link, defer_apply,
                                       getattr(x, "_plx_dx_sink", None))
        if identity is not None and identity.is_cuda:
            from polyaxon_amd.ops.bn_fused import materialize
            identity = materialize(identity)
        return bn_act_reference(x, self.weight, self.bias, self.running_mean, self.running_var,
                                self.training, self.momentum, self.eps, identity, self.act)

    def extra_repr(self) -> str:
        return f"{self.num_features}, act={self.act}, residual={self.residual}, fused={self.fused}"
```

Measured before the change: 12580.

## Fuse residual BN apply+ReLU of bottleneck output into next block's conv1x1 GEMM prologue

The final BN+residual+ReLU of a bottleneck block can now be deferred. The next block's first 1x1 conv GEMM then computes the normalized activation while staging its A operand. That same pass writes the materialized output and the ReLU mask from the tn==0 tiles, which removes one standalone elementwise apply pass per eligible block. The cost is a more complex GEMM prologue with extra loads (residual, scale/bias) per K step, plus a pending-state mechanism with a fallback fill kernel for consumers that cannot fuse.

```diff
diff --git a/polyaxon_amd/csrc/bn_kernels.hip b/polyaxon_amd/csrc/bn_kernels.hip
--- a/polyaxon_amd/csrc/bn_kernels.hip
+++ b/polyaxon_amd/csrc/bn_kernels.hip
@@ -859,6 +859,14 @@
   return (int)hipGetLastError();
 }
 
+PLX_API int plx_bn_apply_res_relu(const void* x, const void* res, void* y, int64_t M, int C, const float* scale_bias,
+                                  uint8_t* mask, const float* res_sb, hipStream_t stream) {
+  Plan p;
+  if (!plan_for(M, C, &p) || M < 1 || res == nullptr || mask == nullptr) return 1;
+  launch_apply(stream, M * p.G, p.G, x, res, y, scale_bias, scale_bias + C, 1, mask, res_sb);
+  return (int)hipGetLastError();
+}
+
 PLX_API int plx_bn_dx_blocks(int64_t M, int C) {
   Plan p;
   if (!plan_for(M, C, &p)) return -1;
diff --git a/polyaxon_amd/csrc/conv_gemm.hip b/polyaxon_amd/csrc/conv_gemm.hip
--- a/polyaxon_amd/csrc/conv_gemm.hip
+++ b/polyaxon_amd/csrc/conv_gemm.hip
@@ -71,6 +71,14 @@
     __bf16* dy;
 };
 
+struct BnApply {
+    const __bf16* res;
+    const float* sb;
+    const float* rsb;
+    __bf16* out;
+    uint8_t* mask;
+};
+
 __device__ __forceinline__ void row_coords(int m, int Hr, int Wr, int& n, int& r, int& c) {
     const int q = m / Wr;
     c = m - q * Wr;
@@ -129,13 +137,16 @@
 __device__ __forceinline__ int nt_swz(int row) { return (row >> 1) & 7; }
 
 template <int BM, int BN, int WGM, int WGN, int MODE, int MINB = 2, int NBUF = 2, bool BWD = false, int NTH = NTHREADS,
-          bool BNDX = false>
+          bool BNDX = false, int BNAP = 0>
 __global__ void __launch_bounds__(NTH, MINB)
 gemm_nt_kernel(const __bf16* __restrict__ A, const __bf16* __restrict__ B, __bf16* __restrict__ C,
                int M, int N, int K, int lda, int ldb, int ldc, const __bf16* __restrict__ zero,
                float* __restrict__ stats, ConvGeom geo, const __bf16* __restrict__ D, int ldd, BnBwd bnr,
-               const uint8_t* __restrict__ dmask, BnDx bd) {
+               const uint8_t* __restrict__ dmask, BnDx bd, BnApply ba) {
     constexpr bool CONV = MODE == 1, STEM = MODE == 2;
+    constexpr bool PROD = BNDX || BNAP != 0;
+    static_assert(BNAP >= 0 && BNAP <= 2 && !(BNDX && BNAP != 0), "one producer mode");
+    static_assert(BNAP == 0 || (MODE == 0 && NBUF == 2 && !BWD && NTH == 256), "BNAP: dense double-buffered forward");
     static_assert(MODE >= 0 && MODE <= 2, "dense, gather or stem");
     static_assert(!BNDX || (MODE == 0 && NBUF == 2 && BWD && NTH == 256), "BNDX: dense double-buffered data gradient");
     constexpr int NW = NTH / 64;
@@ -251,14 +262,14 @@
         st = tap_inner ? st_i : st_m;
         sc = tap_inner ? sc_i : sc_m;
     };
-    constexpr int XI = BNDX ? AI : 1;
+    constexpr int XI = PROD ? AI : 1;
     uint32_t e_off[XI];
     u32x4 gq[XI], xq[XI], oq[XI];
     uint32_t mq[XI];
-    u32x4 cf[6];
+    u32x4 cf[BNAP == 2 ? 8 : 6];
     const int lc8 = (((lane & 7) ^ nt_swz(wave * 8 + (lane >> 3))) & 7) * 8;
     const bool dy_owner = tn == 0;
-    if constexpr (BNDX) {
+    if constexpr (PROD) {
 #pragma unroll
         for (int i = 0; i < XI; ++i) {
             const int gm = m0 + (i * NW + wave) * 8 + (lane >> 3);
@@ -316,6 +327,76 @@
         const __amdgpu_buffer_rsrc_t rd = buf_rsrc(bd.dy);
 #pragma unroll
         for (int i = 0; i < XI; ++i) __builtin_amdgcn_raw_buffer_store_b128(oq[i], rd, (int)e_off[i], k0 * 2, 0);
+    };
+    auto load_ap = [&](int k0) {
+        if constexpr (BNAP != 0) {
+            const __amdgpu_buffer_rsrc_t rr = buf_rsrc(ba.res), rc = buf_rsrc(ba.sb);
+#pragma unroll
+            for (int i = 0; i < XI; ++i) {
+                gq[i] = __builtin_amdgcn_raw_buffer_load_b128(ra, (int)e_off[i], k0 * 2, 0);
+                xq[i] = __builtin_amdgcn_raw_buffer_load_b128(rr, (int)e_off[i], k0 * 2, 0);
+            }
+#pragma unroll
+            for (int r = 0; r < 2; ++r) {
+                cf[2 * r] = __builtin_amdgcn_raw_buffer_load_b128(rc, lc8 * 4, (r * K + k0) * 4, 0);
+                cf[2 * r + 1] = __builtin_amdgcn_raw_buffer_load_b128(rc, lc8 * 4 + 16, (r * K + k0) * 4, 0);
+            }
+            if constexpr (BNAP == 2) {
+                const __amdgpu_buffer_rsrc_t rs = buf_rsrc(ba.rsb);
+#pragma unroll
+                for (int r = 0; r < 2; ++r) {
+                    cf[4 + 2 * r] = __builtin_amdgcn_raw_buffer_load_b128(rs, lc8 * 4, (r * K + k0) * 4, 0);
+                    cf[5 + 2 * r] = __builtin_amdgcn_raw_buffer_load_b128(rs, lc8 * 4 + 16, (r * K + k0) * 4, 0);
+                }
+            }
+        }
+    };
+    auto xform_ap = [&](int buf) {
+        if constexpr (BNAP != 0) {
+            char* base = smem + buf * STAGE;
+            const float* ca = (const float*)&cf[0];
+            const float* cb = (const float*)&cf[2];
+            const float* cra = (const float*)&cf[BNAP == 2 ? 4 : 0];
+            const float* crb = (const float*)&cf[BNAP == 2 ? 6 : 0];
+#pragma unroll
+            for (int i = 0; i < XI; ++i) {
+                const uint32_t* px = (const uint32_t*)&gq[i];
+                const uint32_t* pr = (const uint32_t*)&xq[i];
+                uint32_t* po = (uint32_t*)&oq[i];
+                uint32_t bits = 0;
+#pragma unroll
+                for (int j = 0; j < 4; ++j) {
+                    const float x0 = __uint_as_float(px[j] << 16), x1 = __uint_as_float(px[j] & 0xffff0000u);
+                    const float r0 = __uint_as_float(pr[j] << 16), r1 = __uint_as_float(pr[j] & 0xffff0000u);
+                    const float ra0 = BNAP == 2 ? cra[2 * j] : 1.f, ra1 = BNAP == 2 ? cra[2 * j + 1] : 1.f;
+                    const float rb0 = BNAP == 2 ? crb[2 * j] : 0.f, rb1 = BNAP == 2 ? crb[2 * j + 1] : 0.f;
+                    float v0 = fmaf(x0, ca[2 * j], cb[2 * j]), v1 = fmaf(x1, ca[2 * j + 1], cb[2 * j + 1]);
+                    v0 += fmaf(r0, ra0, rb0);
+                    v1 += fmaf(r1, ra1, rb1);
+                    v0 = fmaxf(v0, 0.f);
+                    v1 = fmaxf(v1, 0.f);
+                    bits |= (uint32_t)(v0 > 0.f) << (2 * j) | (uint32_t)(v1 > 0.f) << (2 * j + 1);
+                    po[j] = pack_bf16x2(v0, v1);
+                }
+                mq[i >> 2] = (i & 3) == 0 ? bits : mq[i >> 2] | bits << (8 * (i & 3));
+                if (e_off[i] == OOB) oq[i] = u32x4{0u, 0u, 0u, 0u};
+                *(u32x4*)(base + (i * NW + wave) * 1024 + lane * 16) = oq[i];
+            }
+        }
+    };
+    auto store_ap = [&](int k0) {
+        if constexpr (BNAP != 0) {
+            if (!dy_owner) return;
+            const __amdgpu_buffer_rsrc_t ro = buf_rsrc(ba.out);
+            const __amdgpu_buffer_rsrc_t rm =
+                __builtin_amdgcn_make_buffer_rsrc(ba.mask, 0, (int)(OOB >> 4), 0x00020000);
+#pragma unroll
+            for (int i = 0; i < XI; ++i) {
+                __builtin_amdgcn_raw_buffer_store_b128(oq[i], ro, (int)e_off[i], k0 * 2, 0);
+                __builtin_amdgcn_raw_buffer_store_b8((uint8_t)(mq[i >> 2] >> (8 * (i & 3))), rm,
+                                                     (int)((e_off[i] + (uint32_t)(k0 * 2)) >> 4), 0, 0);
+            }
+        }
     };
     if constexpr (BNDX) {
         static_assert(!BNDX || NW == 4, "a thread's rows step by 32: one chunk column per thread");
@@ -325,6 +406,14 @@
         asm volatile("s_waitcnt vmcnt(0)" ::: "memory");
         __syncthreads();
         store_dy(0);
+    } else if constexpr (BNAP != 0) {
+        static_assert(BNAP == 0 || NW == 4, "a thread's rows step by 32: one chunk column per thread");
+        load_ap(0);
+        stage_b(0, 0, 0, 0);
+        xform_ap(0);
+        asm volatile("s_waitcnt vmcnt(0)" ::: "memory");
+        __syncthreads();
+        store_ap(0);
     } else {
         stage(0, 0, 0, 0);
         advance();
@@ -339,13 +428,19 @@
                 stage_b(cur ^ 1, (kt + 1) * BK, 0, 0);
             }
         }
-        if (!BNDX && NBUF == 1 && kt > 0) {
+        if constexpr (BNAP != 0) {
+            if (kt + 1 < nk) {
+                load_ap((kt + 1) * BK);
+                stage_b(cur ^ 1, (kt + 1) * BK, 0, 0);
+            }
+        }
+        if (!PROD && NBUF == 1 && kt > 0) {
             stage(0, kt * BK, st, sc);
             advance();
             asm volatile("s_waitcnt vmcnt(0)" ::: "memory");
             __syncthreads();
         }
-        if (!BNDX && NBUF == 2 && kt + 1 < nk) {
+        if (!PROD && NBUF == 2 && kt + 1 < nk) {
             stage(cur ^ 1, (kt + 1) * BK, st, sc);
             advance();
         }
@@ -375,10 +470,16 @@
         if constexpr (BNDX) {
             if (kt + 1 < nk) xform_a(cur ^ 1);
         }
+        if constexpr (BNAP != 0) {
+            if (kt + 1 < nk) xform_ap(cur ^ 1);
+        }
         if (NBUF == 2) asm volatile("s_waitcnt vmcnt(0)" ::: "memory");
         __syncthreads();
         if constexpr (BNDX) {
             if (kt + 1 < nk) store_dy((kt + 1) * BK);
+        }
+        if constexpr (BNAP != 0) {
+            if (kt + 1 < nk) store_ap((kt + 1) * BK);
         }
     }
     constexpr int CROW = BN * 2 + 16;
@@ -1029,7 +1130,7 @@
     auto k = bwd ? kb : kf;
     const int nwg = ((M + BM - 1) / BM) * (N / BN);
     hipLaunchKernelGGL(k, dim3(nwg), dim3(NTH), LDS, s, (const __bf16*)A, (const __bf16*)B, (__bf16*)C, M, N,
-                       K, lda, ldb, ldc, (const __bf16*)zero, stats, geo, (const __bf16*)D, ldd, bnr, dmask, BnDx{});
+                       K, lda, ldb, ldc, (const __bf16*)zero, stats, geo, (const __bf16*)D, ldd, bnr, dmask, BnDx{}, BnApply{});
     return hipGetLastError() == hipSuccess ? 0 : -3;
 }
 
@@ -1045,7 +1146,23 @@
     const int nwg = ((M + BM - 1) / BM) * (N / BN);
     hipLaunchKernelGGL(k, dim3(nwg), dim3(NTHREADS), LDS, s, (const __bf16*)g, (const __bf16*)B, (__bf16*)C, M, N, K, K,
                        ldb, ldc, (const __bf16*)nullptr, (float*)nullptr, ConvGeom{}, (const __bf16*)D, ldd, bnr, dmask,
-                       bd);
+                       bd, BnApply{});
+    return hipGetLastError() == hipSuccess ? 0 : -3;
+}
+
+template <int BM, int BN, int WGM, int WGN, int BNAP>
+int launch_nt_bnapply(const void* x, const BnApply& ba, const void* B, void* C, int M, int N, int K, int ldb, int ldc,
+                      float* stats, hipStream_t s) {
+    constexpr int TILE = BM * (BN * 2 + 16), RED = NTHREADS * 17 * 4;
+    constexpr int LDS = 2 * (BM + BN) * BK * 2;
+    static_assert(TILE <= LDS && RED <= LDS && LDS <= 80 * 1024, "epilogue staging fits; 2 blocks per CU");
+    auto k = gemm_nt_kernel<BM, BN, WGM, WGN, 0, 2, 2, false, NTHREADS, false, BNAP>;
+    static int attr = set_lds(k, LDS);
+    if (attr) return attr;
+    const int nwg = ((M + BM - 1) / BM) * (N / BN);
+    hipLaunchKernelGGL(k, dim3(nwg), dim3(NTHREADS), LDS, s, (const __bf16*)x, (const __bf16*)B, (__bf16*)C, M, N, K, K,
+                       ldb, ldc, (const __bf16*)nullptr, stats, ConvGeom{}, (const __bf16*)nullptr, 0, BnBwd{},
+                       (const uint8_t*)nullptr, BnDx{}, ba);
     return hipGetLastError() == hipSuccess ? 0 : -3;
 }
 
@@ -1278,6 +1395,21 @@
     return launch_nt_bndx<256, 64, 4, 1>(g, bd, Wt, C, M, N, K, ldb, ldc, s, D, ldd, b, dmask);
 }
 
+int plx_gemm_nt_bnapply(const void* x, const void* res, const float* sb, const float* rsb, void* out, uint8_t* mask,
+                        const void* W, void* C, int M, int N, int K, int ldb, int ldc, float* stats, void* stream) {
+    if (M <= 0 || N % 64 || K % BK || ldb % 8 || ldc % 8) return -1;
+    if (x == nullptr || res == nullptr || sb == nullptr || out == nullptr || mask == nullptr || out == x || out == res)
+        return -1;
+    if ((long)M * K >= (1l << 30)) return -1;
+    const BnApply ba{(const __bf16*)res, sb, rsb, (__bf16*)out, mask};
+    hipStream_t s = (hipStream_t)stream;
+    if (N % 128 == 0)
+        return rsb != nullptr ? launch_nt_bnapply<128, 128, 2, 2, 2>(x, ba, W, C, M, N, K, ldb, ldc, stats, s)
+                              : launch_nt_bnapply<128, 128, 2, 2, 1>(x, ba, W, C, M, N, K, ldb, ldc, stats, s);
+    return rsb != nullptr ? launch_nt_bnapply<256, 64, 4, 1, 2>(x, ba, W, C, M, N, K, ldb, ldc, stats, s)
+                          : launch_nt_bnapply<256, 64, 4, 1, 1>(x, ba, W, C, M, N, K, ldb, ldc, stats, s);
+}
+
 int plx_tn_plan_slices(int M, int N1, int N2, int num_cus, int v2) {
     if (M <= 0 || N1 % 64 || N2 % 64) return -1;
     return v2 ? tn2_plan(M, N1, N2, num_cus, v2_cfg(N1, N2)).slices : tn_plan(M, N1, N2, num_cus).slices;
diff --git a/polyaxon_amd/models/resnet.py b/polyaxon_amd/models/resnet.py
--- a/polyaxon_amd/models/resnet.py
+++ b/polyaxon_amd/models/resnet.py
@@ -5,6 +5,7 @@
 import torch
 import torch.nn as nn
 
+from polyaxon_amd.ops import conv1x1 as _c1
 from polyaxon_amd.ops.conv1x1 import Conv1x1, GradMailbox
 from polyaxon_amd.ops.conv import Conv3x3, ConvKxK
 from polyaxon_amd.ops.norm import BatchNormAct
@@ -27,19 +28,30 @@
         self.bn3 = BatchNormAct(out_ch, act=True, fused=fused, residual=True)
         self.downsample = downsample
 
-    def forward(self, x: torch.Tensor) -> torch.Tensor:
+    def forward(self, x: torch.Tensor, defer_out: bool = False) -> torch.Tensor:
         train = self.training and torch.is_grad_enabled() and x.requires_grad
         box = GradMailbox() if train else None
         if self.downsample is None:
             out = self.bn1(self.conv1(x, grad_box=box, bn_link=True))
             out = self.bn2(self.conv2(out, bn_link=True))
-            return self.bn3(self.conv3(out, bn_link=True), x, residual_grad_box=box)
+            return self.bn3(self.conv3(out, bn_link=True), x, residual_grad_box=box, defer_res_relu=defer_out)
         identity = self.downsample(x, grad_box=box)
         out = self.bn1(self.conv1(x, grad_sink=box, bn_link=True))
         out = self.bn2(self.conv2(out, bn_link=True))
-        return self.bn3(self.conv3(out, bn_link=True), identity, residual_link=True)
+        return self.bn3(self.conv3(out, bn_link=True), identity, residual_link=True, defer_res_relu=defer_out)
+
+    def takes_pending(self, x: torch.Tensor) -> bool:
+        c = self.conv1
+        return (self.downsample is None and self.training and c.native and _c1.supported(x, c)
+                and _c1.bn_apply_sink_ok(c.in_channels, c.out_channels))
 
 
+def run_blocks(blocks, x: torch.Tensor) -> torch.Tensor:
+    blocks = list(blocks)
+    for i, blk in enumerate(blocks):
+        nxt = blocks[i + 1] if i + 1 < len(blocks) else None
+        x = blk(x, defer_out=blk.training and nxt is not None and nxt.takes_pending(x))
+    return x
 
 
 class Downsample(nn.Module):
@@ -111,7 +123,9 @@
     def forward_features(self, x: torch.Tensor) -> torch.Tensor:
         x = self.stem(x)
         x = stem_bn_relu_pool(x, self.stem_bn, self.pool)
-        return self.stages(x)
+        for stage in self.stages:
+            x = run_blocks(stage, x)
+        return x
 
     def forward_head(self, x: torch.Tensor) -> torch.Tensor:
         x = torch.flatten(x.mean((2, 3)), 1) if x.is_contiguous() else global_avg_pool(x)
diff --git a/polyaxon_amd/ops/_native.py b/polyaxon_amd/ops/_native.py
--- a/polyaxon_amd/ops/_native.py
+++ b/polyaxon_amd/ops/_native.py
@@ -201,6 +201,7 @@
         "plx_bn_workspace": [_L, _I],
         "plx_bn_forward": [_P, _P, _P, _L, _I, _P, _P, _F, _F, _P, _P, _P, _P, _P, _P, _P, _I, _P, _P, _P],
         "plx_bn_apply": [_P, _P, _P, _L, _I, _P, _I, _P],
+        "plx_bn_apply_res_relu": [_P, _P, _P, _L, _I, _P, _P, _P, _P],
         "plx_bn_l2_workspace": [_I, _I],
         "plx_bn_forward_from_partials": [_P, _P, _P, _L, _I, _P, _P, _F, _F, _P, _P, _P, _P, _P, _P, _I, _P, _P,
                                          _I, _P, _P, _P],
@@ -241,6 +242,7 @@
     "plx_conv": {
         "plx_gemm_nt": [_P, _P, _P, _I, _I, _I, _I, _I, _I, _P, _P, _P, _I, _P, _P, _P],
         "plx_gemm_nt_bndx": [_P, _P, _P, _P, _P, _P, _P, _I, _I, _I, _I, _I, _P, _I, _P, _P, _P],
+        "plx_gemm_nt_bnapply": [_P, _P, _P, _P, _P, _P, _P, _P, _I, _I, _I, _I, _I, _P, _P],
         "plx_gemm_nt_rows_per_block": [_I],
         "plx_gemm_tn_workspace": [_I, _I, _I, _I],
         "plx_set_tn_v2": [_I, _I],
diff --git a/polyaxon_amd/ops/bn_fused.py b/polyaxon_amd/ops/bn_fused.py
--- a/polyaxon_amd/ops/bn_fused.py
+++ b/polyaxon_amd/ops/bn_fused.py
@@ -7,7 +7,7 @@
 import torch
 
 from polyaxon_amd.ops import _native
-from polyaxon_amd.ops.conv1x1 import BnLink
+from polyaxon_amd.ops.conv1x1 import BnLink, PendingApply, fill_pending
 from polyaxon_amd.ops.flat import direct_grad
 
 
@@ -38,7 +38,7 @@
 class _BNAct(torch.autograd.Function):
     @staticmethod
     def forward(ctx, x, weight, bias, running_mean, running_var, residual, momentum, eps, relu, ext=None, box=None,
-                link=None, rlink=None, defer=False, dxsink=None):
+                link=None, rlink=None, defer=False, dxsink=None, pend=None):
         lib = _native.lib("plx_bn")
         ctx.dxsink = dxsink if x.is_contiguous(memory_format=torch.channels_last) else None
         x = _cl(x)
@@ -50,7 +50,8 @@
         f32 = dict(dtype=torch.float32, device=x.device)
         defer = bool(defer) and not relu and residual is None and link is not None
         y = None if defer else torch.empty_like(x, memory_format=torch.channels_last)
-        yp = y.data_ptr() if y is not None else None
+        holder, pend = pend, pend is not None and relu and residual is not None and not defer
+        yp = y.data_ptr() if (y is not None and not pend) else None
         stats = torch.empty(4 * c, **f32)
         res_sb = None
         if residual is not None:
@@ -81,6 +82,9 @@
                 rsp, _counters(x.device), _stream())
             _native.check(rc, "plx_bn_forward")
         ctx.save_for_backward(x, mask, weight, stats)
+        ctx.pending = PendingApply(x, res, stats[2 * c:], res_sb, mask, y) if pend else None
+        if pend:
+            holder.append(ctx.pending)
         ctx.relu = relu
         ctx.has_res = residual is not None
         ctx.box = box if (box is not None and box.armed and residual is not None) else None
@@ -104,6 +108,8 @@
     def backward(ctx, dy):
         lib = _native.lib("plx_bn")
         x, mask, weight, stats = ctx.saved_tensors
+        if ctx.pending is not None:
+            ctx.pending.check_done()
         n, c, h, w = x.shape
         m = n * h * w
         dy = _cl(dy)
@@ -141,7 +147,7 @@
                 ctx.box.put_masked(dy, mask)
             dgamma = dgb[:c] if dgb is not None else None
             dbeta = dgb[c:] if dgb is not None else None
-            return dx, dgamma, dbeta, None, None, None, None, None, None, None, None, None, None, None, None
+            return dx, dgamma, dbeta, None, None, None, None, None, None, None, None, None, None, None, None, None
         rb = None
         if ctx.rlink is not None and dres is not None:
             rl = ctx.rlink
@@ -175,7 +181,7 @@
             dres = None
         dgamma = dgb[:c] if dgb is not None else None
         dbeta = dgb[c:] if dgb is not None else None
-        return dx, dgamma, dbeta, None, None, dres, None, None, None, None, None, None, None, None, None
+        return dx, dgamma, dbeta, None, None, dres, None, None, None, None, None, None, None, None, None, None
 
 
 class _Materialize(torch.autograd.Function):
@@ -192,7 +198,10 @@
 
 
 def materialize(t: Optional[torch.Tensor]) -> Optional[torch.Tensor]:
-    if t is None or not getattr(t, "_plx_deferred", False):
+    if t is None:
+        return t
+    fill_pending(t)
+    if not getattr(t, "_plx_deferred", False):
         return t
     return _Materialize.apply(t, t._plx_bn_link.affine)
 
@@ -200,18 +209,23 @@
 def bn_act(x: torch.Tensor, weight: torch.Tensor, bias: torch.Tensor, running_mean: Optional[torch.Tensor],
            running_var: Optional[torch.Tensor], training: bool, momentum: float, eps: float,
            residual: Optional[torch.Tensor], act: bool, ext_stats=None, residual_grad_box=None,
-           residual_link: bool = False, defer_apply: bool = False, dx_sink=None) -> torch.Tensor:
+           residual_link: bool = False, defer_apply: bool = False, dx_sink=None,
+           defer_res_relu: bool = False) -> torch.Tensor:
+    fill_pending(residual)
     if residual is not None and residual.dtype != x.dtype:
         residual = residual.to(x.dtype)
     if training:
         link = BnLink()
         rlink = getattr(residual, "_plx_bn_link", None) if (residual_link and residual is not None) else None
         defer = bool(defer_apply) and not act and residual is None
+        pend = [] if (defer_res_relu and act and residual is not None) else None
         y = _BNAct.apply(x, weight, bias, running_mean, running_var, residual, momentum, eps, act, ext_stats,
-                         residual_grad_box, link, rlink, defer, dx_sink)
+                         residual_grad_box, link, rlink, defer, dx_sink, pend)
         y._plx_bn_link = link
         if defer:
             y._plx_deferred = True
+        if pend:
+            y._plx_pending = pend[0]
         return y
     residual = materialize(residual)
     lib = _native.lib("plx_bn")
diff --git a/polyaxon_amd/ops/conv1x1.py b/polyaxon_amd/ops/conv1x1.py
--- a/polyaxon_amd/ops/conv1x1.py
+++ b/polyaxon_amd/ops/conv1x1.py
@@ -21,6 +21,19 @@
     global _BN_DX_FUSED
     prev, _BN_DX_FUSED = _BN_DX_FUSED, bool(on)
     return prev
+
+
+_BN_APPLY_FUSED = os.environ.get("PLX_BN_APPLY_FUSED", "1") != "0"
+
+
+def set_bn_apply_fused(on: bool) -> bool:
+    global _BN_APPLY_FUSED
+    prev, _BN_APPLY_FUSED = _BN_APPLY_FUSED, bool(on)
+    return prev
+
+
+def bn_apply_fused() -> bool:
+    return _BN_APPLY_FUSED
 
 
 def _zero_page(dev: torch.device) -> torch.Tensor:
@@ -98,6 +111,33 @@
     return out
 
 
+def gemm_nt_bnapply(x: torch.Tensor, res: torch.Tensor, sb: torch.Tensor, rsb, out_a: torch.Tensor, mask: torch.Tensor,
+                    b: torch.Tensor, out: torch.Tensor = None, stats: torch.Tensor = None) -> torch.Tensor:
+    m, k = x.shape
+    n = b.shape[0]
+    if out is None:
+        out = torch.empty(m, n, dtype=torch.bfloat16, device=x.device)
+    for t in (x, res, out_a):
+        assert t.shape == (m, k) and t.dtype == torch.bfloat16 and t.stride() == (k, 1) and t.data_ptr() % 16 == 0
+    assert b.stride(1) == 1 and out.stride(1) == 1 and b.shape[1] == k and b.dtype == torch.bfloat16
+    assert b.data_ptr() % 16 == 0 and out.data_ptr() % 16 == 0
+    assert mask.dtype == torch.uint8 and mask.is_contiguous() and mask.numel() >= m * k // 8
+    for c in (sb, rsb):
+        assert c is None or (c.dtype == torch.float32 and c.is_contiguous() and c.numel() == 2 * k
+                             and c.data_ptr() % 16 == 0)
+    assert sb is not None
+    if stats is not None:
+        nblk = -(-m // nt_stats_rows(n))
+        assert stats.dtype == torch.float32 and stats.is_contiguous() and stats.numel() >= 2 * nblk * n
+    rc = _native.lib("plx_conv").plx_gemm_nt_bnapply(x.data_ptr(), res.data_ptr(), sb.data_ptr(),
+                                                     rsb.data_ptr() if rsb is not None else None, out_a.data_ptr(),
+                                                     mask.data_ptr(), b.data_ptr(), out.data_ptr(), m, n, k,
+                                                     b.stride(0), out.stride(0),
+                                                     stats.data_ptr() if stats is not None else None, _stream())
+    _native.check(rc, "plx_gemm_nt_bnapply")
+    return out
+
+
 def gemm_tn(a: torch.Tensor, b: torch.Tensor, out: torch.Tensor = None, accumulate: bool = False) -> torch.Tensor:
     m, n1 = a.shape
     n2 = b.shape[1]
@@ -191,6 +231,56 @@
     return DxSink() if (cout >= 2 * cin and cin <= 128) else None
 
 
+class PendingApply:
+
+    __slots__ = ("x", "res", "sb", "rsb", "mask", "out", "state")
+
+    def __init__(self, x, res, sb, rsb, mask, out):
+        self.x, self.res, self.sb, self.rsb, self.mask, self.out = x, res, sb, rsb, mask, out
+        self.state = "pending"
+
+    @property
+    def pending(self) -> bool:
+        return self.state == "pending"
+
+    def take(self) -> "PendingApply":
+        if self.state != "pending":
+            raise RuntimeError("PendingApply: the deferred BatchNorm output was already " + self.state
+                               + "; a second consumer cannot take it")
+        self.state = "taken"
+        return self
+
+    def fill(self) -> None:
+        if self.state != "pending":
+            return
+        n, c, h, w = self.x.shape
+        rc = _native.lib("plx_bn").plx_bn_apply_res_relu(
+            self.x.data_ptr(), self.res.data_ptr(), self.out.data_ptr(), n * h * w, c, self.sb.data_ptr(),
+            self.mask.data_ptr(), self.rsb.data_ptr() if self.rsb is not None else None, _stream())
+        _native.check(rc, "plx_bn_apply_res_relu")
+        self.state = "filled"
+        self.release()
+
+    def release(self) -> None:
+        self.x = self.res = self.sb = self.rsb = self.mask = self.out = None
+
+    def check_done(self) -> None:
+        if self.state == "pending":
+            raise RuntimeError("PendingApply: the BatchNorm's deferred output (and its ReLU mask) was never filled: "
+                               "no consumer took it and nothing materialised it before the backward")
+
+
+def fill_pending(t):
+    p = getattr(t, "_plx_pending", None) if t is not None else None
+    if p is not None:
+        p.fill()
+    return t
+
+
+def bn_apply_sink_ok(cin: int, cout: int) -> bool:
+    return _BN_APPLY_FUSED and cin >= 2 * cout and cout <= 128
+
+
 class BnLink:
 
     __slots__ = ("x", "mask", "mean", "invstd", "part", "nblk", "_args", "affine", "split")
@@ -250,7 +340,11 @@
 
 class _Conv1x1(torch.autograd.Function):
     @staticmethod
-    def forward(ctx, x, weight, stats, box, sink, link, dxsink=None):
+    def forward(ctx, x, weight, stats, box, sink, link, dxsink=None, pend=None):
+        if pend is not None and (x.data_ptr() != pend.out.data_ptr() or x.shape != pend.out.shape
+                                 or x.dtype != torch.bfloat16
+                                 or not x.is_contiguous(memory_format=torch.channels_last)):
+            raise RuntimeError("PendingApply: the convolution's input is not the deferred BatchNorm output")
         x = x.to(torch.bfloat16).contiguous(memory_format=torch.channels_last)
         ctx.box = box
         ctx.dxsink = dxsink
@@ -263,7 +357,11 @@
         cout = weight.shape[0]
         wb, wt = wcache.lookup(weight) or weight_prep(weight)
         y = torch.empty((n, cout, h, w), dtype=torch.bfloat16, device=x.device, memory_format=torch.channels_last)
-        gemm_nt(_rows(x), wb, _rows(y), stats)
+        if pend is not None:
+            gemm_nt_bnapply(_rows(pend.x), _rows(pend.res), pend.sb, pend.rsb, _rows(x), pend.mask, wb, _rows(y), stats)
+            pend.release()
+        else:
+            gemm_nt(_rows(x), wb, _rows(y), stats)
         ctx.save_for_backward(x, wt)
         ctx.wshape = weight.shape
         ctx.wdtype = weight.dtype
@@ -311,7 +409,7 @@
                 side_stream.run(lambda: gemm_tn(_rows(dy), _rows(x), out=slot, accumulate=True), (dy, x), x.device)
             else:
                 dw = gemm_tn(_rows(dy), _rows(x)).view(ctx.wshape).to(ctx.wdtype)
-        return dx, dw, None, None, None, None, None
+        return dx, dw, None, None, None, None, None, None
 
 
 def _bf16_context(x: torch.Tensor) -> bool:
@@ -337,7 +435,17 @@
     if grad_box is not None:
         grad_box.armed = True
     dxsink = dx_sink_for(x, weight)
-    y = _Conv1x1.apply(x, weight, stats, grad_box, grad_sink, bn_link_of(x, bn_link), dxsink)
+    pend = getattr(x, "_plx_pending", None)
+    if pend is not None and pend.pending:
+        n, cin, h, w = x.shape
+        if bn_apply_sink_ok(cin, weight.shape[0]) and n * h * w * cin < (1 << 30):
+            pend = pend.take()
+        else:
+            pend.fill()
+            pend = None
+    else:
+        pend = None
+    y = _Conv1x1.apply(x, weight, stats, grad_box, grad_sink, bn_link_of(x, bn_link), dxsink, pend)
     if stats is not None:
         y._plx_channel_stats = (stats, nblk)
     if dxsink is not None:
@@ -357,4 +465,4 @@
         if self.native and supported(x, self):
             return conv1x1(x, self.weight, with_stats=self.bn_stats and self.training, grad_box=grad_box,
                            grad_sink=grad_sink, bn_link=bn_link)
-        return F.conv2d(x, self.weight, None, self.stride)
+        return F.conv2d(fill_pending(x), self.weight, None, self.stride)
diff --git a/polyaxon_amd/ops/norm.py b/polyaxon_amd/ops/norm.py
--- a/polyaxon_amd/ops/norm.py
+++ b/polyaxon_amd/ops/norm.py
@@ -40,7 +40,7 @@
             self.running_var.fill_(1.0)
 
     def forward(self, x: torch.Tensor, identity: Optional[torch.Tensor] = None, residual_grad_box=None,
-                residual_link: bool = False, defer_apply: bool = False) -> torch.Tensor:
+                residual_link: bool = False, defer_apply: bool = False, defer_res_relu: bool = False) -> torch.Tensor:
         if self.residual and identity is None:
             raise ValueError("BatchNormAct(residual=True) needs the identity tensor")
         if self.fused and x.is_cuda:
@@ -50,7 +50,8 @@
                 return bn_fused.bn_act(x, self.weight, self.bias, self.running_mean, self.running_var,
                                        self.training, self.momentum, self.eps, identity, self.act, ext,
                                        residual_grad_box, residual_link, defer_apply,
-                                       getattr(x, "_plx_dx_sink", None))
+                                       getattr(x, "_plx_dx_sink", None),
+                                       defer_res_relu)
         if identity is not None and identity.is_cuda:
             from polyaxon_amd.ops.bn_fused import materialize
             identity = materialize(identity)
```

Result: faster. 12760, median of 6 (+1.4%).
